# mosure/bevy_gaussian_splatting

Hardware: AMD Instinct MI355X
Metric: frames/sec @1080p, 1M-splat 3DGS (sort + rasterize every frame) (higher is better)
Workload: dtype f32; 1 GPU; 1000000-splat 3DGS f32 planar cloud (seed 2, reference random_gaussians_3d distributions), 1920x1080, SH degree 3, CloudSettings::default(), examples/headless.rs camera incl. its Msaa (Bevy's default Sample4: 4 samples per pixel, resolved frame); one camera per GPU; sample_count=4, parallelism=views1, sort=radix32, frames_in_flight=8, lanes=8, streams=4

## Files before the change

### bevy_gaussian_splatting_amd/_native.py

```python
from __future__ import annotations

import ctypes
import os
from ctypes import POINTER, c_char_p, c_float, c_int
from typing import Optional

from . import _build_id, _loader
from .camera import BgsView
from .settings import BgsSettings

SPEC = _build_id.LIBBGS
LIB_PATH = SPEC.path

BGS_OK = 0
BGS_EINVAL = -1
BGS_ENOMEM = -2
BGS_EHIP = -3
BGS_ECAPACITY = -4
BGS_EINTERNAL = -5

STAGE_NAMES = ("keygen", "depth_sort", "project", "tile_sort", "ranges", "raster")

COMM_ID_BYTES = 128
ABI_VERSION = (0 << 16) | 4


class BgsSortEntry(ctypes.Structure):
    _fields_ = [("key", ctypes.c_uint32), ("index", ctypes.c_uint32)]


class BgsStats(ctypes.Structure):
    _fields_ = [
        ("stage_ms", ctypes.c_float * 6),
        ("total_ms", ctypes.c_float),
        ("splat_count", ctypes.c_uint32),
        ("visible_count", ctypes.c_uint32),
        ("draw_count", ctypes.c_uint32),
        ("sort_path", ctypes.c_uint32),
        ("instance_count", ctypes.c_uint64),
        ("instance_capacity", ctypes.c_uint64),
        ("tiles_x", ctypes.c_uint32),
        ("tiles_y", ctypes.c_uint32),
        ("depth_passes", ctypes.c_uint32),
        ("tile_passes", ctypes.c_uint32),
        ("algorithmic_bytes", ctypes.c_uint64),
        ("regrow_count", ctypes.c_uint32),
        ("binning_mode", ctypes.c_uint32),
        ("frames_averaged", ctypes.c_uint32),
        ("list_capacity", ctypes.c_uint32),
        ("list_entries_allocated", ctypes.c_uint64),
        ("strip_tiles", ctypes.c_uint32),
        ("tile_saturation", ctypes.c_uint32),
    ]


class BgsFrameRecordsInfo(ctypes.Structure):

    _fields_ = [("draw_count", ctypes.c_uint32), ("record_stride", ctypes.c_uint32), ("has_rects", ctypes.c_uint32),
                ("visible_count", ctypes.c_uint32), ("color_max_bits", ctypes.c_uint32)]


vp, u32, u64 = ctypes.c_void_p, ctypes.c_uint32, ctypes.c_uint64
fp, up, u64p, vpp = POINTER(c_float), POINTER(u32), POINTER(u64), POINTER(vp)
view_p, settings_p, entry_p = POINTER(BgsView), POINTER(BgsSettings), POINTER(BgsSortEntry)

PROTOTYPES = (
    ("bgs_create", c_int, (c_int, vpp)),
    ("bgs_destroy", None, (vp,)),
    ("bgs_last_error", c_char_p, (vp,)),
    ("bgs_version", u32, ()),
    ("bgs_abi_check", c_int, (u32, u32, u32, u32)),
    ("bgs_build_id", c_char_p, ()),
    ("bgs_settings_default", None, (settings_p,)),
    ("bgs_view_perspective", None, (fp, c_float, c_float, u32, u32, view_p)),
    ("bgs_cloud_upload_f32", c_int, (vp, u32, fp, fp, fp, fp, vpp)),
    ("bgs_cloud_upload_f16", c_int, (vp, u32, fp, up, up, vpp)),
    ("bgs_cloud_upload_cov3d_f32", c_int, (vp, u32, fp, fp, fp, vpp)),
    ("bgs_cloud_free", None, (vp, vp)),
    ("bgs_cloud_len", u32, (vp,)),
    ("bgs_cloud_apply_particle_behaviors", c_int, (vp, vp, vp, u32, c_float)),
    ("bgs_sort", c_int, (vp, vp, view_p, settings_p, entry_p)),
    ("bgs_render", c_int, (vp, vp, view_p, settings_p, fp)),
    ("bgs_framebuffer_device_ptr", c_int, (vp, vpp, u64p)),
    ("bgs_set_output_srgb8", c_int, (vp, c_int)),
    ("bgs_framebuffer_srgb8_device_ptr", c_int, (vp, vpp, u64p)),
    ("bgs_set_output_rgba16f", c_int, (vp, c_int)),
    ("bgs_framebuffer_rgba16f_device_ptr", c_int, (vp, vpp, u64p)),
    ("bgs_set_packed_only", c_int, (vp, c_int)),
    ("bgs_set_srgb8_target", c_int, (vp, vp)),
    ("bgs_download", c_int, (vp, vp, vp, u64)),
    ("bgs_device_alloc", c_int, (vp, u64, vpp)),
    ("bgs_device_free", c_int, (vp, vp)),
    ("bgs_upload", c_int, (vp, vp, vp, u64)),
    ("bgs_set_pipeline_depth", c_int, (vp, u32)),
    ("bgs_pipeline_pop", c_int, (vp, vpp, vpp)),
    ("bgs_frames_in_flight", c_int, (vp, up)),
    ("bgs_sorted_entries_device_ptr", c_int, (vp, vpp, up)),
    ("bgs_synchronize", c_int, (vp,)),
    ("bgs_set_async", c_int, (vp, c_int)),
    ("bgs_stream", c_int, (vp, vpp)),
    ("bgs_set_binning", c_int, (vp, u32)),
    ("bgs_reset_adaptive_state", c_int, (vp,)),
    ("bgs_set_profiling", c_int, (vp, c_int)),
    ("bgs_set_profiling_stride", c_int, (vp, u32)),
    ("bgs_get_stats", c_int, (vp, POINTER(BgsStats))),
    ("bgs_set_pipeline_streams", c_int, (vp, u32)),
    ("bgs_set_graphs", c_int, (vp, c_int)),
    ("bgs_comm_unique_id", c_int, (c_char_p,)),
    ("bgs_comm_create", c_int, (vp, c_char_p, u32, u32, vpp)),
    ("bgs_comm_gather", c_int, (vp, vp, u32, vp, u64, vp, u64p)),
    ("bgs_comm_gather_after", c_int, (vp, vp, u32, vp, u64, vp, vp, u64p)),
    ("bgs_comm_wait", c_int, (vp, vp, u64)),
    ("bgs_comm_stream", c_int, (vp, vp, vpp)),
    ("bgs_comm_destroy", None, (vp, vp)),
    ("bgs_set_debug_flags", c_int, (vp, u32)),
    ("bgs_adaptive_counters", c_int, (vp, u64p)),
    ("bgs_learning_counters", c_int, (vp, u64p, u64p)),
    ("bgs_radix_sort_pairs", c_int, (vp, entry_p, u32, u32)),
    ("bgs_hbm_probe", c_int, (vp, u64, u32, fp, fp)),
    ("bgs_selftest_ln_f32", c_int, (vp, u32, u32, fp, u64p)),
    ("bgs_set_queue_holders", c_int, (c_int,)),
    ("bgs_set_tile_trace", c_int, (vp, vp)),
    ("bgs_graph_counters", c_int, (vp, u64p, u64p)),
    ("bgs_tile_order_counters", c_int, (vp, u64p, u64p, u64p)),
    ("bgs_selftest_tile_order", c_int, (vp, vp, u32, u32, vp, vp)),
    ("bgs_selftest_pack", c_int, (vp, u32, vp, u32, vp)),
    ("bgs_debug_frame_records", c_int, (vp, vp, u64, up, u32, POINTER(BgsFrameRecordsInfo))),
)
EXPORTED_SYMBOLS = tuple(name for name, _, _ in PROTOTYPES)


class BgsError(RuntimeError):
    def __init__(self, status: int, message: str):
        super().__init__(f"libbgs error {status}: {message}")
        self.status = status


_lib: Optional[ctypes.CDLL] = None


def ensure_current() -> str:
    return _loader.ensure_current(SPEC, LIB_PATH)


def build_id() -> str:
    return load().bgs_build_id().decode()


def load() -> ctypes.CDLL:
    global _lib
    if _lib is not None:
        return _lib
    override = os.environ.get("BGS_LIB_OVERRIDE")
    if override:
        import sys
        print(f"bevy_gaussian_splatting_amd: BGS_LIB_OVERRIDE={override} — NOT the library of this tree "
              f"(build id {_build_id.library_build_id(override)})", file=sys.stderr)
        lib = ctypes.CDLL(override, mode=SPEC.dlopen_mode)
        _loader.declare(lib, PROTOTYPES)
    else:
        want = ensure_current()
        lib = ctypes.CDLL(LIB_PATH, mode=SPEC.dlopen_mode)
        _loader.declare(lib, PROTOTYPES)
        if lib.bgs_build_id().decode() != want:
            raise ImportError(f"{LIB_PATH}: bgs_build_id() disagrees with the id in the file's bytes")
    rc = lib.bgs_abi_check(ABI_VERSION, ctypes.sizeof(BgsView), ctypes.sizeof(BgsSettings), ctypes.sizeof(BgsStats))
    if rc != BGS_OK:
        raise ImportError("libbgs.so refuses this binding: " + (lib.bgs_last_error(None) or b"").decode("utf-8", "replace"))
    _lib = lib
    return lib


def check(lib: ctypes.CDLL, ctx, status: int) -> None:
    if status != BGS_OK:
        msg = lib.bgs_last_error(ctx)
        raise BgsError(status, msg.decode("utf-8", "replace") if msg else "")
```

### bevy_gaussian_splatting_amd/csrc/bgs_api.hip

```cpp
#include "bgs_context.h"
#include "build_id.inc"

static const char g_build_id[] = "BGS_BUILD_ID=" BGS_BUILD_ID;

namespace {
void mat4_mul(const float* a, const float* b, float* out) {
    for (int c = 0; c < 4; ++c)
        for (int r = 0; r < 4; ++r) {
            float acc = 0.0f;
            for (int k = 0; k < 4; ++k) acc += a[4 * k + r] * b[4 * c + k];
            out[4 * c + r] = acc;
        }
}

bool mat4_inverse(const float* m, float* out) {
    double a[4][8];
    for (int r = 0; r < 4; ++r)
        for (int c = 0; c < 4; ++c) {
            a[r][c] = m[4 * c + r];
            a[r][4 + c] = r == c ? 1.0 : 0.0;
        }
    for (int i = 0; i < 4; ++i) {
        int piv = i;
        for (int r = i + 1; r < 4; ++r)
            if (std::fabs(a[r][i]) > std::fabs(a[piv][i])) piv = r;
        if (a[piv][i] == 0.0) return false;
        if (piv != i)
            for (int c = 0; c < 8; ++c) std::swap(a[i][c], a[piv][c]);
        const double d = a[i][i];
        for (int c = 0; c < 8; ++c) a[i][c] /= d;
        for (int r = 0; r < 4; ++r)
            if (r != i) {
                const double f = a[r][i];
                for (int c = 0; c < 8; ++c) a[r][c] -= f * a[i][c];
            }
    }
    for (int r = 0; r < 4; ++r)
        for (int c = 0; c < 4; ++c) out[4 * c + r] = (float)a[r][4 + c];
    return true;
}

}


extern "C" {

uint32_t bgs_version(void) { return (BGS_VERSION_MAJOR << 16) | BGS_VERSION_MINOR; }

const char* bgs_build_id(void) { return g_build_id + 13; }

const char* bgs_last_error(const bgs_ctx* ctx) { return ctx ? ctx->error.c_str() : g_error.c_str(); }

int bgs_create(int hip_device, bgs_ctx** out) {
    if (!out) return fail(nullptr, BGS_EINVAL, "out is NULL");
    *out = nullptr;
    int count = 0;
    hipError_t e = hipGetDeviceCount(&count);
    if (e != hipSuccess || count <= 0)
        return fail(nullptr, BGS_EHIP, std::string("no usable HIP device (there is no CPU fallback): ") +
                                           hipGetErrorString(e));
    if (hip_device < 0 || hip_device >= count) return fail(nullptr, BGS_EINVAL, "hip_device out of range");
    bgs_ctx* ctx = new (std::nothrow) bgs_ctx();
    if (!ctx) return fail(nullptr, BGS_ENOMEM, "out of host memory");
    ctx->device = hip_device;
    auto bail = [&](const std::string& msg) {
        bgs_destroy(ctx);
        return fail(nullptr, BGS_EHIP, msg);
    };
    if ((e = hipSetDevice(hip_device)) != hipSuccess) return bail(std::string("hipSetDevice: ") + hipGetErrorString(e));
    hipDeviceProp_t prop;
    if ((e = hipGetDeviceProperties(&prop, hip_device)) != hipSuccess)
        return bail(std::string("hipGetDeviceProperties: ") + hipGetErrorString(e));
    ctx->num_cus = prop.multiProcessorCount > 0 ? prop.multiProcessorCount : 256;
    if (lane_create(ctx, ctx->lanes[0]) != BGS_OK) return bail(ctx->error);
    *out = ctx;
    return BGS_OK;
}

void bgs_destroy(bgs_ctx* ctx) {
    if (!ctx) return;
    (void)hipSetDevice(ctx->device);
    for (auto& L : ctx->lanes) lane_destroy(L);
    for (auto st : ctx->streams) if (st) (void)hipStreamDestroy(st);
    if (ctx->step_done) (void)hipEventDestroy(ctx->step_done);
    delete ctx;
}

void bgs_settings_default(bgs_settings* out) {
    if (!out) return;
    std::memset(out, 0, sizeof *out);
    for (int i = 0; i < 4; ++i) out->transform[5 * i] = 1.0f;
    out->global_opacity = 1.0f;
    out->global_scale = 1.0f;
    out->gaussian_mode = BGS_GAUSSIAN_3D;
    out->aabb = 0;
    out->opacity_adaptive_radius = 1;
    out->color_space = BGS_COLOR_SRGB;
    out->radix_depth_bits = 32;
    out->sh_degree = 3;
    out->sort_mode = BGS_SORT_RADIX;
    out->rasterize_mode = BGS_RASTERIZE_COLOR;
    out->num_classes = 1;
    for (int i = 0; i < 3; ++i) out->position_max[i] = 1.0f;
    out->position_min[3] = out->position_max[3] = 1.0f;
}

void bgs_view_perspective(const float world_from_view[16], float fov_y_radians, float near_plane,
                          uint32_t width, uint32_t height, bgs_view* out) {
    if (!out || !world_from_view) return;
    std::memset(out, 0, sizeof *out);
    std::memcpy(out->world_from_view, world_from_view, 16 * sizeof(float));
    if (!mat4_inverse(world_from_view, out->view_from_world))
        for (int i = 0; i < 4; ++i) out->view_from_world[5 * i] = 1.0f;
    const float f = 1.0f / std::tan(0.5f * fov_y_radians);
    const float aspect = (float)width / (float)height;
    out->clip_from_view[0] = f / aspect;
    out->clip_from_view[5] = f;
    out->clip_from_view[11] = -1.0f;
    out->clip_from_view[14] = near_plane;
    mat4_mul(out->clip_from_view, out->view_from_world, out->clip_from_world);
    out->viewport[0] = 0.0f;
    out->viewport[1] = 0.0f;
    out->viewport[2] = (float)width;
    out->viewport[3] = (float)height;
    out->clear_color[3] = 1.0f;
    out->sample_count = 4;
    std::memcpy(out->previous_clip_from_world, out->clip_from_world, sizeof out->clip_from_world);
    out->delta_time = 1.0f / 60.0f;
}

static int upload_plane(bgs_ctx* ctx, const void* host, size_t bytes, DeviceBuffer<uint8_t>& dev) {
    if (!dev.reserve(bytes, 16)) return fail(ctx, BGS_ENOMEM, "hipMalloc(cloud plane) failed");
    if (bytes && hipMemcpy(dev.ptr, host, bytes, hipMemcpyHostToDevice) != hipSuccess)
        return fail(ctx, BGS_EHIP, "hipMemcpy(cloud plane) failed");
    return BGS_OK;
}

static int upload_and_pack(bgs_ctx* ctx, uint32_t format, uint32_t n, const void* pv, const void* const planes[3],
                           const uint32_t v4[3], uint32_t stride_v4, bgs_cloud** out) {
    if (!ctx) return fail(nullptr, BGS_EINVAL, "ctx is NULL");
    if (!out) return fail(ctx, BGS_EINVAL, "out is NULL");
    *out = nullptr;
    if (n > MAX_SPLATS) return fail(ctx, BGS_EINVAL, "too many splats");
    bool missing = !pv;
    for (int k = 0; k < 3; ++k) missing = missing || (v4[k] && !planes[k]);
    if (n && missing) return fail(ctx, BGS_EINVAL, "NULL plane pointer");
    if (hipSetDevice(ctx->device) != hipSuccess) return fail(ctx, BGS_EHIP, "hipSetDevice failed");
    bgs_cloud* c = new (std::nothrow) bgs_cloud();
    if (!c) return fail(ctx, BGS_ENOMEM, "out of host memory");
    DeviceBuffer<uint8_t> tmp[3];
    int rc = upload_plane(ctx, pv, (size_t)n * 16, c->positions);
    for (int k = 0; rc == BGS_OK && k < 3; ++k)
        if (v4[k]) rc = upload_plane(ctx, planes[k], (size_t)n * 16 * v4[k], tmp[k]);
    if (rc == BGS_OK && !c->packed.reserve((size_t)n * 16 * stride_v4, 256))
        rc = fail(ctx, BGS_ENOMEM, "hipMalloc(packed cloud records) failed");
    if (rc == BGS_OK) {
        hipStream_t st = ctx->lanes[0].stream;
        launch_pack_cloud(st, (const uint4*)c->positions.ptr, (const uint4*)tmp[0].ptr, v4[0], (const uint4*)tmp[1].ptr, v4[1],
                          (const uint4*)tmp[2].ptr, v4[2], (uint4*)c->packed.ptr, stride_v4, n);
        if (hipGetLastError() != hipSuccess || hipStreamSynchronize(st) != hipSuccess) {
            (void)hipGetLastError();
            rc = fail(ctx, BGS_EHIP, "packing the cloud on the device failed");
        }
    }
    if (rc != BGS_OK) { bgs_cloud_free(ctx, c); return rc; }
    c->bytes = (size_t)n * 16 + (size_t)n * 16 * stride_v4;
    c->ptrs.position_visibility = (const float4*)c->positions.ptr;
    c->ptrs.packed = (const uint4*)c->packed.ptr;
    c->ptrs.packed_v4 = stride_v4;
    c->ptrs.n = n;
    c->ptrs.format = format;
    *out = c;
    return BGS_OK;
}

int bgs_cloud_upload_f32(bgs_ctx* ctx, uint32_t n, const float* pv, const float* sh, const float* rot,
                         const float* so, bgs_cloud** out) {
    const void* const planes[3] = {rot, so, sh};
    const uint32_t v4[3] = {1u, 1u, 12u};
    return upload_and_pack(ctx, CLOUD_F32, n, pv, planes, v4, 16u, out);
}

int bgs_cloud_upload_f16(bgs_ctx* ctx, uint32_t n, const float* pv, const uint32_t* sh_h2,
                         const uint32_t* rso, bgs_cloud** out) {
    const void* const planes[3] = {rso, sh_h2, nullptr};
    const uint32_t v4[3] = {1u, 6u, 0u};
    return upload_and_pack(ctx, CLOUD_F16, n, pv, planes, v4, 8u, out);
}

int bgs_cloud_upload_cov3d_f32(bgs_ctx* ctx, uint32_t n, const float* pv, const float* sh, const float* cov3d_opacity,
                               bgs_cloud** out) {
    const void* const planes[3] = {cov3d_opacity, nullptr, sh};
    const uint32_t v4[3] = {2u, 0u, 12u};
    return upload_and_pack(ctx, CLOUD_COV3D, n, pv, planes, v4, 16u, out);
}

void bgs_cloud_free(bgs_ctx* ctx, bgs_cloud* cloud) {
    if (!cloud) return;
    if (ctx) {
        (void)hipSetDevice(ctx->device);
        (void)finish_all(ctx);
        for (auto& L : ctx->lanes) {
            if (L.stream) (void)hipStreamSynchronize(L.stream);
            if (L.in.cloud == cloud) L.in.cloud = nullptr;
        }
        for (auto& sl : ctx->split_slots)
            if (sl.cloud == cloud) sl.epoch = 0;
    }
    delete cloud;
}

uint32_t bgs_cloud_len(const bgs_cloud* cloud) { return cloud ? cloud->ptrs.n : 0; }

int bgs_cloud_apply_particle_behaviors(bgs_ctx* ctx, bgs_cloud* cloud, void* behaviors_device_ptr, uint32_t count, float delta_time) {
    if (!ctx) return fail(nullptr, BGS_EINVAL, "ctx is NULL");
    if (!cloud) return fail(ctx, BGS_EINVAL, "cloud is NULL");
    if (!std::isfinite(delta_time)) return fail(ctx, BGS_EINVAL, "delta_time is not finite");
    if (count == 0) return BGS_OK;
    if (!behaviors_device_ptr) return fail(ctx, BGS_EINVAL, "behaviors_device_ptr is NULL with count > 0");
    if ((uintptr_t)behaviors_device_ptr % 16u) return fail(ctx, BGS_EINVAL, "behaviors_device_ptr is not 16-byte aligned");
    return apply_particle_step(ctx, cloud, behaviors_device_ptr, count, delta_time);
}

int bgs_sort(bgs_ctx* ctx, const bgs_cloud* cloud, const bgs_view* view, const bgs_settings* settings,
             bgs_sort_entry* host_out) {
    int rc = run(ctx, cloud, view, settings, false);
    if (rc != BGS_OK) return rc;
    Lane& L = ctx->lanes[0];
    if (host_out && L.last_sorted_n)
        HIP_TRY(ctx, hipMemcpy(host_out, L.last_sorted, (size_t)L.last_sorted_n * sizeof(uint2), hipMemcpyDeviceToHost));
    return BGS_OK;
}

int bgs_render(bgs_ctx* ctx, const bgs_cloud* cloud, const bgs_view* view, const bgs_settings* settings,
               float* rgba_host_out) {
    int rc = run(ctx, cloud, view, settings, true);
    if (rc != BGS_OK) return rc;
    if (rgba_host_out) {
        Lane& L = ctx->lanes[ctx->recent];
        if (L.pending && (rc = finish_lane(ctx, L)) != BGS_OK) return rc;
        if (!L.fb_valid) return fail(ctx, BGS_EINVAL, "the frame wrote its packed image only (bgs_set_packed_only): no f32 target to copy");
        HIP_TRY(ctx, hipMemcpy(rgba_host_out, L.fb.ptr, (size_t)L.fb_w * L.fb_h * sizeof(float4), hipMemcpyDeviceToHost));
    }
    return BGS_OK;
}

int bgs_framebuffer_device_ptr(bgs_ctx* ctx, void** dptr, uint64_t* bytes) {
    if (!ctx || !dptr) return fail(ctx, BGS_EINVAL, "NULL argument");
    Lane& L = ctx->lanes[ctx->recent];
    if (L.pending) {
        int rc = finish_lane(ctx, L);
        if (rc != BGS_OK) return rc;
    }
    if (!L.fb.ptr) return fail(ctx, BGS_EINVAL, "no frame has been rendered yet");
    if (!L.fb_valid) return fail(ctx, BGS_EINVAL, "the last frame wrote its packed image only (bgs_set_packed_only)");
    *dptr = L.fb.ptr;
    if (bytes) *bytes = (uint64_t)L.fb_w * L.fb_h * sizeof(float4);
    return BGS_OK;
}

int bgs_framebuffer_srgb8_device_ptr(bgs_ctx* ctx, void** dptr, uint64_t* bytes) {
    if (!ctx || !dptr) return fail(ctx, BGS_EINVAL, "NULL argument");
    Lane& L = ctx->lanes[ctx->recent];
    if (L.pending) {
        int rc = finish_lane(ctx, L);
        if (rc != BGS_OK) return rc;
    }
    if (!L.fb8_out || !L.fb8_valid || L.fb8_is_f16)
        return fail(ctx, BGS_EINVAL, "no Rgba8UnormSrgb frame: call bgs_set_output_srgb8(ctx, 1) before rendering");
    *dptr = L.fb8_out;
    if (bytes) *bytes = (uint64_t)L.fb_w * L.fb_h * 4u;
    return BGS_OK;
}

int bgs_pipeline_pop(bgs_ctx* ctx, void** rgba_f32, void** rgba8) {
    if (!ctx) return fail(nullptr, BGS_EINVAL, "ctx is NULL");
    if (hipSetDevice(ctx->device) != hipSuccess) return fail(ctx, BGS_EHIP, "hipSetDevice failed");
    int best = -1;
    for (int i = 0; i < MAX_LANES; ++i)
        if ((ctx->lanes[i].pending || ctx->lanes[i].ready) && (best < 0 || ctx->lanes[i].seq < ctx->lanes[best].seq)) best = i;
    if (best < 0) return fail(ctx, BGS_EINVAL, "no frame in flight");
    Lane& L = ctx->lanes[best];
    int rc = finish_lane(ctx, L);
    if (rc != BGS_OK) return rc;
    if (rgba_f32) *rgba_f32 = L.fb_valid ? L.fb.ptr : nullptr;
    if (rgba8) *rgba8 = L.fb8_valid ? L.fb8_out : nullptr;
    return BGS_OK;
}

int bgs_frames_in_flight(bgs_ctx* ctx, uint32_t* count) {
    if (!ctx || !count) return fail(ctx, BGS_EINVAL, "NULL argument");
    uint32_t c = 0;
    for (auto& L : ctx->lanes) c += (L.pending || L.ready) ? 1u : 0u;
    *count = c;
    return BGS_OK;
}

int bgs_sorted_entries_device_ptr(bgs_ctx* ctx, void** dptr, uint32_t* n) {
    if (!ctx || !dptr) return fail(ctx, BGS_EINVAL, "NULL argument");
    Lane& L = ctx->lanes[ctx->recent];
    if (L.pending) {
        int rc = finish_lane(ctx, L);
        if (rc != BGS_OK) return rc;
    }
    if (!L.last_sorted) return fail(ctx, BGS_EINVAL, "no sort has been run yet");
    *dptr = (void*)L.last_sorted;
    if (n) *n = L.last_sorted_n;
    return BGS_OK;
}

int bgs_synchronize(bgs_ctx* ctx) {
    if (!ctx) return fail(nullptr, BGS_EINVAL, "ctx is NULL");
    if (hipSetDevice(ctx->device) != hipSuccess) return fail(ctx, BGS_EHIP, "hipSetDevice failed");
    int rc = finish_all(ctx);
    if (rc != BGS_OK) return rc;
    for (auto& L : ctx->lanes)
        if (L.stream) HIP_TRY(ctx, hipStreamSynchronize(L.stream));
    return BGS_OK;
}

int bgs_set_async(bgs_ctx* ctx, int enabled) {
    if (!ctx) return fail(nullptr, BGS_EINVAL, "ctx is NULL");
    if (!enabled) {
        int rc = finish_all(ctx);
        if (rc != BGS_OK) return rc;
    }
    ctx->async_frames = enabled != 0;
    return BGS_OK;
}

int bgs_set_pipeline_depth(bgs_ctx* ctx, uint32_t lanes) {
    if (!ctx) return fail(nullptr, BGS_EINVAL, "ctx is NULL");
    if (lanes < 1 || lanes > (uint32_t)MAX_LANES) return fail(ctx, BGS_EINVAL, "pipeline depth must be 1..8");
    if (hipSetDevice(ctx->device) != hipSuccess) return fail(ctx, BGS_EHIP, "hipSetDevice failed");
    int rc = finish_all(ctx);
    if (rc != BGS_OK) return rc;
    ctx->depth = (int)lanes;
    ctx->next = 0;
    ctx->recent = 0;
    for (uint32_t i = 0; i < lanes; ++i)
        if ((rc = lane_create(ctx, ctx->lanes[i])) != BGS_OK) return rc;
    return assign_streams(ctx);
}

int bgs_set_pipeline_streams(bgs_ctx* ctx, uint32_t streams) {
    if (!ctx) return fail(nullptr, BGS_EINVAL, "ctx is NULL");
    if (streams > (uint32_t)MAX_LANES) return fail(ctx, BGS_EINVAL, "pipeline streams must be 0..8");
    if (hipSetDevice(ctx->device) != hipSuccess) return fail(ctx, BGS_EHIP, "hipSetDevice failed");
    int rc = finish_all(ctx);
    if (rc != BGS_OK) return rc;
    for (auto st : ctx->streams)
        if (st) HIP_TRY(ctx, hipStreamSynchronize(st));
    ctx->num_streams = (int)streams;
    return assign_streams(ctx);
}

int bgs_set_srgb8_target(bgs_ctx* ctx, void* device_ptr) {
    if (!ctx) return fail(nullptr, BGS_EINVAL, "ctx is NULL");
    ctx->next_srgb8_target = (uint32_t*)device_ptr;
    return BGS_OK;
}

int bgs_download(bgs_ctx* ctx, const void* device_ptr, void* host_out, uint64_t bytes) {
    if (!ctx || !device_ptr || !host_out) return fail(ctx, BGS_EINVAL, "NULL argument");
    if (hipSetDevice(ctx->device) != hipSuccess) return fail(ctx, BGS_EHIP, "hipSetDevice failed");
    if (bytes) HIP_TRY(ctx, hipMemcpy(host_out, device_ptr, (size_t)bytes, hipMemcpyDeviceToHost));
    return BGS_OK;
}

int bgs_device_alloc(bgs_ctx* ctx, uint64_t bytes, void** device_ptr_out) {
    if (!ctx || !device_ptr_out) return fail(ctx, BGS_EINVAL, "NULL argument");
    *device_ptr_out = nullptr;
    if (hipSetDevice(ctx->device) != hipSuccess) return fail(ctx, BGS_EHIP, "hipSetDevice failed");
    DeviceBuffer<uint8_t> buf;
    if (!buf.reserve((size_t)bytes, 16)) return fail(ctx, BGS_ENOMEM, "hipMalloc(" + std::to_string(bytes) + " bytes) failed");
    *device_ptr_out = buf.release();
    return BGS_OK;
}

int bgs_device_free(bgs_ctx* ctx, void* device_ptr) {
    if (!ctx) return fail(nullptr, BGS_EINVAL, "ctx is NULL");
    if (!device_ptr) return BGS_OK;
    if (hipSetDevice(ctx->device) != hipSuccess) return fail(ctx, BGS_EHIP, "hipSetDevice failed");
    int rc = finish_all(ctx);
    if (rc != BGS_OK) return rc;
    HIP_TRY(ctx, hipFree(device_ptr));
    return BGS_OK;
}

int bgs_upload(bgs_ctx* ctx, void* device_ptr, const void* host_in, uint64_t bytes) {
    if (!ctx || !device_ptr || !host_in) return fail(ctx, BGS_EINVAL, "NULL argument");
    if (hipSetDevice(ctx->device) != hipSuccess) return fail(ctx, BGS_EHIP, "hipSetDevice failed");
    if (bytes) HIP_TRY(ctx, hipMemcpy(device_ptr, host_in, (size_t)bytes, hipMemcpyHostToDevice));
    return BGS_OK;
}

int bgs_set_output_srgb8(bgs_ctx* ctx, int enabled) {
    if (!ctx) return fail(nullptr, BGS_EINVAL, "ctx is NULL");
    ctx->output_srgb8 = enabled != 0;
    if (enabled) ctx->output_rgba16f = false;
    return BGS_OK;
}

int bgs_set_output_rgba16f(bgs_ctx* ctx, int enabled) {
    if (!ctx) return fail(nullptr, BGS_EINVAL, "ctx is NULL");
    ctx->output_rgba16f = enabled != 0;
    if (enabled) ctx->output_srgb8 = false;
    return BGS_OK;
}

int bgs_set_packed_only(bgs_ctx* ctx, int enabled) {
    if (!ctx) return fail(nullptr, BGS_EINVAL, "ctx is NULL");
    ctx->packed_only = enabled != 0;
    return BGS_OK;
}

int bgs_framebuffer_rgba16f_device_ptr(bgs_ctx* ctx, void** dptr, uint64_t* bytes) {
    if (!ctx || !dptr) return fail(ctx, BGS_EINVAL, "NULL argument");
    Lane& L = ctx->lanes[ctx->recent];
    if (L.pending) {
        int rc = finish_lane(ctx, L);
        if (rc != BGS_OK) return rc;
    }
    if (!L.fb8_out || !L.fb8_valid || !L.fb8_is_f16)
        return fail(ctx, BGS_EINVAL, "no Rgba16Float frame: call bgs_set_output_rgba16f(ctx, 1) before rendering");
    *dptr = L.fb8_out;
    if (bytes) *bytes = (uint64_t)L.fb_w * L.fb_h * 8u;
    return BGS_OK;
}

int bgs_stream(bgs_ctx* ctx, void** hip_stream) {
    if (!ctx || !hip_stream) return fail(ctx, BGS_EINVAL, "NULL argument");
    *hip_stream = (void*)ctx->lanes[ctx->recent].stream;
    return BGS_OK;
}

int bgs_set_profiling(bgs_ctx* ctx, int enabled) {
    if (!ctx) return fail(nullptr, BGS_EINVAL, "ctx is NULL");
    if (enabled < 0 || enabled > 2) return fail(ctx, BGS_EINVAL, "profiling level must be 0, 1 or 2");
    ctx->profiling = enabled;
    return BGS_OK;
}

int bgs_set_profiling_stride(bgs_ctx* ctx, uint32_t every_nth_frame) {
    if (!ctx) return fail(nullptr, BGS_EINVAL, "ctx is NULL");
    if (every_nth_frame == 0) return fail(ctx, BGS_EINVAL, "stride must be >= 1");
    ctx->profiling_stride = every_nth_frame;
    ctx->frame_counter = 0;
    return BGS_OK;
}

int bgs_set_binning(bgs_ctx* ctx, uint32_t mode) {
    if (!ctx) return fail(nullptr, BGS_EINVAL, "ctx is NULL");
    if (mode > BINNING_SORT) return fail(ctx, BGS_EINVAL, "binning mode must be 0 (scan) or 1 (sort)");
    int rc = finish_all(ctx);
    if (rc != BGS_OK) return rc;
    ctx->binning = mode;
    return BGS_OK;
}

int bgs_set_debug_flags(bgs_ctx* ctx, uint32_t flags) {
    if (!ctx) return fail(nullptr, BGS_EINVAL, "ctx is NULL");
    ctx->debug_flags = flags;
    return BGS_OK;
}

int bgs_adaptive_counters(bgs_ctx* ctx, uint64_t out[8]) {
    if (!ctx || !out) return fail(ctx, BGS_EINVAL, "NULL argument");
    out[0] = ctx->bucket_frames;
    out[1] = ctx->onesweep_frames;
    out[2] = ctx->reruns_sort;
    out[3] = ctx->reruns_lists;
    out[4] = ctx->reruns_instances;
    out[5] = ctx->level_changes;
// ... 88 lines not shown
```

### bevy_gaussian_splatting_amd/csrc/bgs_context.h

```cpp
#pragma once
#include <hip/hip_runtime.h>

#include <dlfcn.h>

#include <algorithm>
#include <chrono>
#include <cmath>
#include <cstdio>
#include <cstdlib>
#include <cstring>
#include <mutex>
#include <new>
#include <string>
#include <unordered_map>
#include <vector>

#include "../../include/bgs.h"
#include "../../include/bgs_diag.h"
#include "bgs_device.h"
#include "device_buffer.h"
#include "frame_params.h"
#include "kernels.h"

using namespace bgs;

namespace bgs_host {

struct DeviceMem {
    static void* alloc(size_t bytes) {
        void* p = nullptr;
        if (hipMalloc(&p, bytes) == hipSuccess) return p;
        (void)hipGetLastError();
        return nullptr;
    }
    static void free(void* p) { (void)hipFree(p); }
};
struct PinnedMem {
    static void* alloc(size_t bytes) {
        void* p = nullptr;
        if (hipHostMalloc(&p, bytes, hipHostMallocDefault) == hipSuccess) return p;
        (void)hipGetLastError();
        return nullptr;
    }
    static void free(void* p) { (void)hipHostFree(p); }
};
template <class T> using DeviceBuffer = Buffer<T, DeviceMem>;
template <class T> using PinnedBuffer = Buffer<T, PinnedMem>;

}

struct bgs_cloud {
    CloudPtrs ptrs{};
    bgs_host::DeviceBuffer<uint8_t> positions, packed;
    uint64_t bytes = 0;
};

namespace bgs_host {

extern thread_local std::string g_error;

constexpr uint64_t MIN_INSTANCE_CAPACITY = 1ull << 22;
constexpr uint64_t MAX_INSTANCE_CAPACITY = 1ull << 30;
constexpr uint32_t MAX_SPLATS = (1u << 30) - 1u;
constexpr int EV_COUNT = BGS_STAGE_COUNT + 1;
constexpr int EV_RING = 64;
constexpr int MAX_LANES = 8;

struct GraphKey {
    const void* cloud[6];
    const void* bufs[11];
    uint32_t n, format, places, sort_mode, gaussian_mode, aabb, any_mode, srgb8, debug_flags;
    int32_t width, height;
    int32_t sort_blocks, bin_blocks, keygen_blocks;
    uint32_t sup_edge;
    ScratchLayout scratch;
    uint32_t coarse_cap, sort_path;
    const void* keygen_func;
    uint32_t keygen_threads;
    uint32_t wide_bin;
    uint32_t raster_variant;
    uint32_t split_sub;
};
struct FrameGraph {
    hipGraph_t graph = nullptr;
    hipGraphExec_t exec = nullptr;
    hipGraphNode_t keygen_node = nullptr;
    GraphKey key{};
};

struct FrameInputs {
    const bgs_cloud* cloud = nullptr;
    bgs_view view{};
    bgs_settings settings{};
    bool render = false, allow_graph = false;
    uint32_t* srgb8_target = nullptr;
    bool output_srgb8 = false, output_rgba16f = false, packed_only = false;
    uint32_t debug_flags = 0;
    uint64_t kind = 0;
    bool force_passes = false;
};

struct FramePlan {
    FrameParams fp{};
    bool render = false, scan = false, surfel = false, culled_tail = true;
    uint32_t n = 0, places = 0, rec_bytes = 0, cloud_format = 0;
    bool bucket = false, wide = false, kept = false;
    uint32_t bucket_sub = 1, split_sub_out = 1;
    int split_slot = -1;
    uint64_t split_epoch = 0;
    uint32_t edges[4] = {6, 8, 16, 32}, level = 1, sup_edge = 8, num_st = 0;
    bool large = false, wide_bin = false, want_srgb8 = false;
    int sort_blocks = 0, bin_blocks = 0, binning_blocks = 0;
    uint32_t out_format = 0, ntiles = 0;
    bool raster_cleans = false;
    RasterInst raster{};
    bool heavy = false, cost = false, ordered = false, refresh = false, graph_ok = false;
    uint64_t sat_kind = 0;
};

struct Lane {
    hipStream_t stream = nullptr;
    hipEvent_t done = nullptr;
    DeviceBuffer<FrameParams> d_fp;
    FrameGraph graph[2];

    DeviceBuffer<uint8_t> scratch;
    ScratchLayout layout;
    uint32_t ctl_parity = 0;
    bool scratch_clean = false;

    DeviceBuffer<uint2> entries[2], culled;
    DeviceBuffer<uint8_t> records;
    DeviceBuffer<uint32_t> rects;
    DeviceBuffer<uint2> inst[2];
    DeviceBuffer<uint32_t> coarse;
    DeviceBuffer<uint2> bucket_slots;
    DeviceBuffer<uint32_t> d_split_keys;
    PinnedBuffer<uint32_t> h_split_keys;
    DeviceBuffer<uint8_t> heavy[2];
    uint32_t heavy_parity = 0;
    const uint8_t* heavy_done = nullptr;
    uint32_t heavy_done_grid = 0;
    bool ready = false;
    DeviceBuffer<uint16_t> cost[2], order;
    uint32_t cost_parity = 0;
    const uint16_t* cost_done = nullptr;
    uint32_t cost_done_grid = 0;
    uint32_t order_grid = 0xFFFFFFFFu, order_age = 0;
    DeviceBuffer<float4> fb;
    DeviceBuffer<uint32_t> fb8;
    uint32_t* fb8_out = nullptr;
    uint32_t fb_w = 0, fb_h = 0;
    bool fb8_valid = false, fb8_is_f16 = false;
    bool fb_valid = true;

    PinnedBuffer<Control> h_ctl;
    Control* h_ctl_dev = nullptr;
    hipEvent_t ev_ring[EV_RING][EV_COUNT] = {};
    uint8_t ev_kind[EV_RING] = {};
    uint32_t ev_head = 0;
    uint32_t frames_timed = 0;

    bool pending = false;
    FrameInputs in;
    FramePlan plan;
    uint32_t pending_coarse_cap = 0;
    uint64_t cost_done_kind = 0;
    uint64_t order_kind = 0;
    uint64_t seq = 0;

    const uint2* last_sorted = nullptr;
    uint32_t last_sorted_n = 0;
    const Control* last_ctl = nullptr;

    bgs_stats result{};
    bool has_result = false;
    uint8_t result_kind = 0;
};

}
using namespace bgs_host;

struct bgs_ctx {
    int device = 0;
    int num_cus = 256;
    std::string error;

    Lane lanes[MAX_LANES];
    hipStream_t streams[MAX_LANES] = {};
    int num_streams = 4;
    int depth = 1;
    int next = 0;
    int recent = 0;
    uint64_t seq = 0;
    hipEvent_t step_done = nullptr;

    uint32_t binning = BINNING_SCAN;
    uint32_t debug_flags = 0;
    int profiling = 2;
    uint32_t profiling_stride = 1;
    uint32_t frame_counter = 0;
    bool async_frames = false;
    bool output_srgb8 = false;
    bool output_rgba16f = false;
    bool packed_only = false;
    uint32_t* next_srgb8_target = nullptr;

    uint32_t draw_hint = 0;
    bool draw_hint_valid = false;
    uint32_t draw_shrink_votes = 0;
    uint32_t sup_level = 1;
    struct SplitterSlot {
        SplitterKeys table{};
        const bgs_cloud* cloud = nullptr;
        uint32_t n = 0;
        uint32_t sort_mode = 0;
        float transform[16] = {};
        float pos[3] = {}, fwd[3] = {};
        float clip_from_view[16] = {};
        float viewport_wh[2] = {};
        float reach = 0.0f;
        uint64_t epoch = 0;
        uint64_t last_used = 0;
    };
    static constexpr int SPLITTER_SLOTS = 16;
    SplitterSlot split_slots[SPLITTER_SLOTS];
    uint64_t split_epoch = 0;
    uint64_t split_failed_epoch = 0;
    uint32_t bucket_block = 0;
    uint32_t bucket_fail_streak = 0;
    uint32_t list_shrink_votes = 0;
    uint64_t bucket_frames = 0, onesweep_frames = 0;
    uint64_t reruns_sort = 0, reruns_lists = 0, reruns_instances = 0, level_changes = 0;
    uint32_t coarse_cap_hint = 0;
    struct KindState { uint32_t sup_level = 1; bool midround = false; };
    std::unordered_map<uint64_t, KindState> kinds;
    static constexpr uint32_t LEARN_MAX = 3;
    static constexpr double MIDROUND_ON = 0.30, MIDROUND_OFF = 0.15;
    uint64_t cur_kind = 0;
    std::unordered_map<uint64_t, uint32_t> learning;
    uint64_t early_frames = 0;
    uint4* tile_trace = nullptr;
    bool use_graphs = false;
    uint64_t graph_captures = 0, graph_replays = 0;
    uint64_t cost_frames = 0, ordered_frames = 0, order_refreshes = 0;

    bool have_stats = false;
    bgs_stats stats{};
    uint32_t regrow_count = 0;
};

namespace bgs_host {
int fail(bgs_ctx* ctx, int status, const std::string& msg);
int assign_streams(bgs_ctx* ctx);
int lane_create(bgs_ctx* ctx, Lane& L);
void lane_destroy(Lane& L);
int finish_lane(bgs_ctx* ctx, Lane& L);
int finish_all(bgs_ctx* ctx);
int collect_stats(bgs_ctx* ctx);
int ensure_scratch(bgs_ctx* ctx, Lane& L, uint32_t n, uint64_t inst_cap);
int enqueue_frame(bgs_ctx* ctx, Lane& L, const FrameInputs& in);
int ensure_entries(bgs_ctx* ctx, Lane& L, uint32_t n);
int run(bgs_ctx* ctx, const bgs_cloud* cloud, const bgs_view* view, const bgs_settings* s, bool render);
int apply_particle_step(bgs_ctx* ctx, bgs_cloud* cloud, void* behaviors, uint32_t count, float dt);
extern int g_queue_holders_mode;
extern std::mutex g_queue_holders_mutex;
}

#define HIP_TRY(ctx, expr)                                                                  \
    do {                                                                                    \
        hipError_t e_ = (expr);                                                             \
        if (e_ != hipSuccess)                                                               \
            return fail(ctx, BGS_EHIP, std::string(#expr) + ": " + hipGetErrorString(e_));  \
    } while (0)
```

### bevy_gaussian_splatting_amd/csrc/bgs_frame.hip

```cpp
#include "bgs_context.h"

thread_local std::string bgs_host::g_error;

namespace bgs_host {


constexpr int MAX_DEVICES = 64;
hipStream_t g_queue_holders[MAX_DEVICES][3] = {};
int g_queue_holders_mode = -1;
std::mutex g_queue_holders_mutex;

int fail(bgs_ctx* ctx, int status, const std::string& msg) {
    if (ctx) ctx->error = msg;
    g_error = msg;
    return status;
}


int assign_streams(bgs_ctx* ctx) {
    const int S = ctx->num_streams > 0 ? std::min(ctx->num_streams, ctx->depth) : ctx->depth;
    for (int i = 0; i < MAX_LANES; ++i) {
        Lane& L = ctx->lanes[i];
        if (!L.done) continue;
        const int si = i < ctx->depth ? i % S : i;
// ... 114 lines not shown

bool cost_holds(const Lane& L, uint32_t tiles) { return L.cost[0].holds(tile_cost_bytes(tiles) / 2u); }

int ensure_cost(bgs_ctx* ctx, Lane& L, uint32_t tiles) {
    if (cost_holds(L, tiles)) return BGS_OK;
    L.cost_done = nullptr;
    L.order_grid = 0xFFFFFFFFu;
    L.order.reset();
    bool ok = reserve_group(tile_cost_bytes(tiles) / 2u, L.cost[0], L.cost[1]) < 0;
    for (auto& c : L.cost)
        if (ok && hipMemset(c.ptr, 0, tile_cost_bytes(tiles)) != hipSuccess) { (void)hipGetLastError(); ok = false; }
    if (!ok) {
        for (auto& c : L.cost) c.reset();
        return fail(ctx, BGS_ENOMEM, "hipMalloc(tile cost feedback) failed");
    }
    if (!L.order.reserve(tile_order_bytes(tiles) / 2u)) {
        for (auto& c : L.cost) c.reset();
        return fail(ctx, BGS_ENOMEM, "hipMalloc(tile order) failed");
    }
    return BGS_OK;
}

int ensure_framebuffer(bgs_ctx* ctx, Lane& L, uint32_t w, uint32_t h, bool want8) {
    const size_t px = (size_t)w * h;
    if (!L.fb.reserve(px)) return fail(ctx, BGS_ENOMEM, "hipMalloc(framebuffer) failed");
    if (want8 && !L.fb8.reserve(2 * px)) return fail(ctx, BGS_ENOMEM, "hipMalloc(srgb8 framebuffer) failed");
    L.fb_w = w;
    L.fb_h = h;
    return BGS_OK;
}

int validate(bgs_ctx* ctx, const bgs_cloud* cloud, const bgs_view* view, const bgs_settings* s, bool render) {
    if (!ctx) return fail(nullptr, BGS_EINVAL, "ctx is NULL");
    if (!cloud || !view || !s) return fail(ctx, BGS_EINVAL, "cloud, view and settings must be non-NULL");
    if (s->radix_depth_bits != 16 && s->radix_depth_bits != 24 && s->radix_depth_bits != 32)
        return fail(ctx, BGS_EINVAL, "radix_depth_bits must be 16, 24 or 32");
    if (s->gaussian_mode > BGS_GAUSSIAN_3D) return fail(ctx, BGS_EINVAL, "gaussian_mode must be 2D or 3D");
    if (s->sh_degree > 3) return fail(ctx, BGS_EINVAL, "sh_degree must be 0..3");
    if (s->sort_mode > BGS_SORT_STD) return fail(ctx, BGS_EINVAL, "unknown sort_mode");
    if (s->color_space > BGS_COLOR_LINEAR) return fail(ctx, BGS_EINVAL, "unknown color_space");
    if (s->rasterize_mode == BGS_RASTERIZE_VELOCITY)
        return fail(ctx, BGS_EINVAL, "rasterize_mode Velocity is outside the path (4D clouds only)");
    if (s->rasterize_mode == BGS_RASTERIZE_OPTICAL_FLOW && !(view->delta_time > 0.0f))
        return fail(ctx, BGS_EINVAL, "rasterize_mode OpticalFlow needs bgs_view.delta_time > 0");
    if (s->rasterize_mode > BGS_RASTERIZE_VELOCITY) return fail(ctx, BGS_EINVAL, "unknown rasterize_mode");
    if (s->draw_mode > BGS_DRAW_HIGHLIGHT_SELECTED) return fail(ctx, BGS_EINVAL, "unknown draw_mode");
    if (s->rasterize_mode == BGS_RASTERIZE_CLASSIFICATION && s->num_classes == 0)
        return fail(ctx, BGS_EINVAL, "num_classes must be >= 1");
    if (view->entries_device_ptr) {
        if (view->entries_device_ptr % sizeof(bgs_sort_entry) != 0u)
            return fail(ctx, BGS_EINVAL, "bgs_view.entries_device_ptr must be aligned to 8 bytes (one bgs_sort_entry)");
        if (view->entry_count != cloud->ptrs.n)
            return fail(ctx, BGS_EINVAL, "bgs_view.entry_count must equal bgs_cloud_len(cloud) when entries_device_ptr is set; got " +
                                             std::to_string(view->entry_count) + " for a cloud of " + std::to_string(cloud->ptrs.n));
    } else if (view->entry_count != 0u) {
        return fail(ctx, BGS_EINVAL, "bgs_view.entry_count is " + std::to_string(view->entry_count) + " but bgs_view.entries_device_ptr is 0");
    }
    if (render && cloud->ptrs.format == CLOUD_COV3D &&
        (s->gaussian_mode != BGS_GAUSSIAN_3D || s->rasterize_mode == BGS_RASTERIZE_NORMAL))
        return fail(ctx, BGS_EINVAL, "a precomputed-covariance cloud has no rotation / scale: 3D gaussian mode only, no Normal raster mode");
    if (render) {
        const uint32_t samples = view->sample_count ? view->sample_count : 4u;
        if (samples != 1u && samples != 2u && samples != 4u && samples != 8u)
            return fail(ctx, BGS_EINVAL, "bgs_view.sample_count must be 1 (Msaa::Off), 2, 4 (Msaa::Sample4, Bevy's default), 8 or 0 (= 4); got " +
                                             std::to_string(view->sample_count));
        if (ctx->tile_trace && (view->depth_device_ptr || s->visualize_bounding_box || samples == 2u || samples == 8u))
            return fail(ctx, BGS_EINVAL, "the per-tile trace (bgs_set_tile_trace) has no instantiation with a depth buffer, the bounding-box "
                                         "overlay or 2 / 8 samples per pixel: a frame would leave the trace buffer untouched");
        if (view->depth_device_ptr % (4u * samples) != 0u)
            return fail(ctx, BGS_EINVAL, "bgs_view.depth_device_ptr must be aligned to one pixel's samples (4 * sample_count bytes)");
        const float w = view->viewport[2], h = view->viewport[3];
        if (!(w >= 1.0f) || !(h >= 1.0f) || w > 4096.0f || h > 4096.0f || w != std::floor(w) || h != std::floor(h))
            return fail(ctx, BGS_EINVAL, "viewport width/height must be integers in [1, 4096]");
    }
    return BGS_OK;
}

void view_pose(const bgs_view* v, float pos[3], float fwd[3]) {
    for (int k = 0; k < 3; ++k) { pos[k] = v->world_from_view[12 + k]; fwd[k] = -v->world_from_view[8 + k]; }
    const float len = std::sqrt(fwd[0] * fwd[0] + fwd[1] * fwd[1] + fwd[2] * fwd[2]);
    if (len > 0.0f) for (int k = 0; k < 3; ++k) fwd[k] /= len;
}

int find_splitter_slot(const bgs_ctx* ctx, const bgs_cloud* cloud, const bgs_view* view, const bgs_settings* s) {
    float pos[3], fwd[3];
    view_pose(view, pos, fwd);
    int best = -1;
    float best_d = 0.0f;
    for (int i = 0; i < bgs_ctx::SPLITTER_SLOTS; ++i) {
        const auto& sl = ctx->split_slots[i];
        if (!sl.epoch || sl.cloud != cloud || sl.n != cloud->ptrs.n || sl.sort_mode != s->sort_mode) continue;
        if (std::memcmp(sl.transform, s->transform, sizeof sl.transform) != 0) continue;
        if (s->sort_mode == BGS_SORT_RADIX &&
            (std::memcmp(sl.clip_from_view, view->clip_from_view, sizeof sl.clip_from_view) != 0 ||
             sl.viewport_wh[0] != view->viewport[2] || sl.viewport_wh[1] != view->viewport[3]))
            continue;
        const float dx = pos[0] - sl.pos[0], dy = pos[1] - sl.pos[1], dz = pos[2] - sl.pos[2];
        const float d = std::sqrt(dx * dx + dy * dy + dz * dz);
        const float c = fwd[0] * sl.fwd[0] + fwd[1] * sl.fwd[1] + fwd[2] * sl.fwd[2];
        if (!(d <= 0.05f * sl.reach) || !(c >= 0.9848f)) continue;
        const float score = d / std::max(sl.reach, 1e-30f) + (1.0f - c);
        if (best < 0 || score < best_d) { best = i; best_d = score; }
    }
    return best;
}

uint64_t frame_kind(const bgs_cloud* cloud, const bgs_view* view, const bgs_settings* s) {
    int32_t scale_step = INT32_MIN;
    if (s->global_scale > 0.0f && std::isfinite(s->global_scale)) scale_step = (int32_t)std::lround(2.0 * std::log2((double)s->global_scale));
    const uint64_t words[6] = {((uint64_t)cloud->ptrs.n << 32) | cloud->ptrs.format, ((uint64_t)s->gaussian_mode << 32) | s->aabb,
                               ((uint64_t)(uint32_t)scale_step << 32) | s->opacity_adaptive_radius,
                               ((uint64_t)(uint32_t)view->viewport[2] << 32) | (uint32_t)view->viewport[3],
                               ((uint64_t)(view->sample_count ? view->sample_count : 4u) << 32) | (view->depth_device_ptr ? 1u : 0u),
                               ((uint64_t)s->rasterize_mode << 32) | (s->draw_mode << 1) | (s->visualize_bounding_box ? 1u : 0u)};
    uint64_t hsh = 0xcbf29ce484222325ull;
    for (uint64_t w : words)
        for (int b = 0; b < 8; ++b) { hsh ^= (w >> (8 * b)) & 0xFFu; hsh *= 0x100000001b3ull; }
    return hsh ? hsh : 1ull;
}

void switch_kind(bgs_ctx* ctx, uint64_t kind) {
    if (kind == ctx->cur_kind) return;
    const auto it = ctx->kinds.find(kind);
    if (it != ctx->kinds.end()) ctx->sup_level = it->second.sup_level;
    ctx->cur_kind = kind;
}

struct FrameTotals { uint64_t instances = 0; uint32_t longest = 0; };

FrameTotals frame_totals(const FramePlan& p, const Control& h) {
    FrameTotals t;
    t.instances = (uint64_t)h.instance_total_lo | ((uint64_t)h.instance_total_hi << 32);
    if (p.render && p.scan) {
        t.instances = 0;
        for (uint32_t i = 0; i < p.num_st; ++i) {
            t.instances += h.coarse_total[i];
            t.longest = std::max(t.longest, h.coarse_total[i]);
        }
    }
    return t;
}

int check_watchdog(bgs_ctx* ctx, Lane& L) {
    const Control& h = *L.h_ctl.ptr;
    if (!h.error) return BGS_OK;
    L.scratch_clean = false;
    ctx->draw_hint_valid = false;
    for (auto& sl : ctx->split_slots) sl.epoch = 0;
    return fail(ctx, BGS_EINTERNAL, "device watchdog tripped (look-back spin bound), code " + std::to_string(h.error));
}

int check_capacities(bgs_ctx* ctx, Lane& L, const FrameTotals& t, int attempt, bool* rerun) {
    const FramePlan& p = L.plan;
    const Control& h = *L.h_ctl.ptr;
    *rerun = false;
    if (p.bucket && h.sort_overflow) {
        if (p.split_slot >= 0 && ctx->split_slots[p.split_slot].epoch == p.split_epoch)
            ctx->split_slots[p.split_slot].epoch = 0;
        if (h.sort_overflow & 2u) {
            ctx->bucket_block = 256u;
        } else if (p.split_epoch > ctx->split_failed_epoch) {
            ctx->bucket_fail_streak = std::min(ctx->bucket_fail_streak + 1u, 8u);
            if (ctx->bucket_fail_streak >= 3u) ctx->bucket_block = (1u << ctx->bucket_fail_streak) - 1u;
        }
        ctx->split_failed_epoch = std::max(ctx->split_failed_epoch, p.split_epoch);
        ctx->reruns_sort += 1;
        L.in.force_passes = true;
        *rerun = true;
    } else if (p.bucket) {
        ctx->bucket_fail_streak = 0;
    }
    if (p.render && p.scan) {
        const uint32_t want = std::max<uint32_t>(pow2_ceil_u32((uint64_t)t.longest + t.longest / 4), 4096u);
        if (p.level == ctx->sup_level) {
            if (want > ctx->coarse_cap_hint) {
                ctx->coarse_cap_hint = want;
                ctx->list_shrink_votes = 0;
            } else if ((uint64_t)want * 8u <= ctx->coarse_cap_hint) {
                if (++ctx->list_shrink_votes >= 64u) { ctx->coarse_cap_hint = want * 2u; ctx->list_shrink_votes = 0; }
            } else {
                ctx->list_shrink_votes = 0;
            }
        }
        if (t.longest > L.pending_coarse_cap) {
            if (want > ctx->coarse_cap_hint) ctx->coarse_cap_hint = want;
            *rerun = true;
            ctx->reruns_lists += 1;
        }
    }
    if (p.render && !p.scan && h.overflow) {
        if (t.instances > MAX_INSTANCE_CAPACITY)
            return fail(ctx, BGS_ECAPACITY,
                        "frame needs " + std::to_string(t.instances) + " tile instances, above the 2^30 limit");
        uint64_t cap = MIN_INSTANCE_CAPACITY;
        while (cap < t.instances + t.instances / 4) cap <<= 1;
        cap = std::min(cap, MAX_INSTANCE_CAPACITY);
        int rc = ensure_instances(ctx, L, cap);
        if (rc != BGS_OK) return rc;
        ctx->reruns_instances += 1;
        *rerun = true;
    }
    if ((L.in.debug_flags & BGS_DEBUG_RERUN_EVERY_FRAME) && attempt == 0 && p.render && p.scan) *rerun = true;
    return BGS_OK;
}

void learn_feedback(bgs_ctx* ctx, Lane& L) {
    const FramePlan& p = L.plan;
    const Control& h = *L.h_ctl.ptr;
    const uint32_t grid = (uint32_t)p.fp.tiles_x | ((uint32_t)p.fp.tiles_y << 16);
    L.heavy_done = p.heavy ? L.heavy[L.heavy_parity].ptr : nullptr;
    L.heavy_done_grid = grid;
    if (p.heavy) L.heavy_parity ^= 1u;
    L.cost_done = p.cost ? L.cost[L.cost_parity].ptr : nullptr;
    L.cost_done_kind = L.in.kind;
    L.cost_done_grid = grid;
    if (p.sat_kind && h.saturated_tiles_prev != 0xFFFFFFFFu) {
        const auto kit = ctx->kinds.find(p.sat_kind);
        if (kit != ctx->kinds.end()) {
            const double share = (double)h.saturated_tiles_prev / (double)0x7FFF;
            if (share >= bgs_ctx::MIDROUND_ON) kit->second.midround = true;
            else if (share <= bgs_ctx::MIDROUND_OFF) kit->second.midround = false;
        }
    }
    if (p.cost) L.cost_parity ^= 1u;
}

void learn_draw_hint(bgs_ctx* ctx, uint32_t draw_count) {
    if (!ctx->draw_hint_valid || draw_count > ctx->draw_hint) {
        ctx->draw_hint = (uint32_t)std::min<uint64_t>((uint64_t)draw_count + draw_count / 8 + 1024, 0xFFFFFFFFull);
        ctx->draw_hint_valid = true;
        ctx->draw_shrink_votes = 0;
    } else if ((uint64_t)draw_count * 4 < ctx->draw_hint) {
        if (++ctx->draw_shrink_votes >= 64u) {
            ctx->draw_hint = (uint32_t)std::min<uint64_t>((uint64_t)draw_count * 2 + 1024, 0xFFFFFFFFull);
            ctx->draw_shrink_votes = 0;
        }
    } else {
        ctx->draw_shrink_votes = 0;
    }
}

void learn_splitters(bgs_ctx* ctx, const Lane& L) {
    const FramePlan& p = L.plan;
    const Control& h = *L.h_ctl.ptr;
    const uint32_t nkeys = BUCKET_COUNT * p.split_sub_out - 1u;
    if (p.places != 4 || h.draw_count < BUCKET_COUNT || !splitters_ascending(h.splitters, nkeys) || !L.in.cloud) return;
    int slot = find_splitter_slot(ctx, L.in.cloud, &L.in.view, &L.in.settings);
    if (slot < 0) {
        slot = 0;
        for (int i = 0; i < bgs_ctx::SPLITTER_SLOTS; ++i) {
            if (!ctx->split_slots[i].epoch) { slot = i; break; }
            if (ctx->split_slots[i].last_used < ctx->split_slots[slot].last_used) slot = i;
        }
    }
    auto& sl = ctx->split_slots[slot];
    std::memcpy(sl.table.key, h.splitters, nkeys * sizeof(uint32_t));
    sl.table.sub = p.split_sub_out;
    sl.cloud = L.in.cloud;
    sl.n = p.n;
    sl.sort_mode = L.in.settings.sort_mode;
    std::memcpy(sl.transform, L.in.settings.transform, sizeof sl.transform);
    view_pose(&L.in.view, sl.pos, sl.fwd);
    std::memcpy(sl.clip_from_view, L.in.view.clip_from_view, sizeof sl.clip_from_view);
    sl.viewport_wh[0] = L.in.view.viewport[2];
    sl.viewport_wh[1] = L.in.view.viewport[3];
    const uint32_t mid_bits = 0xFFFFFFFFu - h.splitters[BUCKET_COUNT * p.split_sub_out / 2 - 1];
    float d2;
    std::memcpy(&d2, &mid_bits, 4);
    sl.reach = (d2 > 0.0f && d2 < 3.0e38f) ? std::sqrt(d2) : 1.0f;
    sl.epoch = ++ctx->split_epoch;
    sl.last_used = ctx->seq;
}

bool learn_level(bgs_ctx* ctx, const Lane& L, const FrameTotals& t) {
    const FramePlan& p = L.plan;
    const uint32_t lv = p.level;
    double longer = 1.0;
    const uint32_t target = canonical_supertile_level(
        next_supertile_level((double)t.instances / (double)L.h_ctl.ptr->visible_count, lv, p.edges, &longer), p.edges);
    const auto kit = ctx->kinds.find(L.in.kind);
    if (kit != ctx->kinds.end()) kit->second.sup_level = target;
    if (L.in.kind != ctx->cur_kind || target == lv) return target != lv;
    if (ctx->sup_level != target) {
        const double predicted = (double)t.longest * (target > lv ? longer : 1.0) * 1.25;
        ctx->coarse_cap_hint = std::max<uint32_t>(pow2_ceil_u32((uint64_t)std::min(predicted, 1.0e9)), 4096u);
        ctx->list_shrink_votes = 0;
        ctx->level_changes += 1;
        ctx->sup_level = target;
    }
    return true;
}

void fill_stats(const bgs_ctx* ctx, Lane& L, const FrameTotals& t) {
    const FramePlan& p = L.plan;
    const Control& h = *L.h_ctl.ptr;
    const bool render = p.render, scan = p.scan;
    bgs_stats& stt = L.result;
    std::memset(&stt, 0, sizeof stt);
    stt.regrow_count = ctx->regrow_count;
    stt.splat_count = p.n;
    stt.visible_count = render ? h.visible_count : h.draw_count;
    stt.draw_count = h.draw_count;
    stt.sort_path = p.kept ? 2u : (p.bucket ? 1u : 0u);
    stt.list_capacity = (render && scan) ? L.pending_coarse_cap : 0u;
    stt.instance_count = render ? t.instances : 0;
    stt.instance_capacity = L.inst[0].capacity;
    stt.list_entries_allocated = (render && scan) ? (uint64_t)(L.coarse.capacity / 2) : 0;
    stt.strip_tiles = (render && scan) ? h.strip_tiles : 0u;
    stt.tile_saturation = (render && scan && p.sat_kind && h.saturated_tiles_prev != 0xFFFFFFFFu)
                              ? (0x10000u | (h.saturated_tiles_prev & 0x7FFFu) | (p.raster.mode != 0 ? 0x80000000u : 0u)) : 0u;
    stt.tiles_x = render ? (uint32_t)p.fp.tiles_x : 0;
    stt.tiles_y = render ? (uint32_t)p.fp.tiles_y : 0;
    stt.depth_passes = p.places;
    stt.tile_passes = (render && !scan) ? 2 : 0;
    stt.binning_mode = scan ? BINNING_SCAN : BINNING_SORT;
    const uint64_t N = p.n, k = p.places, D = h.draw_count;
    uint64_t bytes = N * 16 + D * 8 + (p.culled_tail ? (N - D) * 8 : 0) + (p.bucket ? D * 24 : k * D * 16);
    if (p.kept) bytes = N * 8 + D * 8 + (p.culled_tail ? (N - D) * 8 : 0);
    if (render) {
        const uint64_t B = p.cloud_format == CLOUD_F16 ? 128 : 240, R = p.rec_bytes, V = h.visible_count, I = t.instances;
        const uint64_t P = (uint64_t)(uint32_t)p.fp.width * (uint32_t)p.fp.height;
        if (scan)
            bytes += V * (B - 16) + V * R + V * 8 + V * 8 + I * 8 + I * 8 + P * 16;
        else
            bytes += V * (B - 16) + V * R + I * 8 + 2 * I * 16 + I * (4 + R) + P * 16;
    }
    stt.algorithmic_bytes = bytes;
    L.has_result = true;
    L.result_kind = (uint8_t)(!render ? 1 : (scan ? 2 : 3) + (p.kept ? 2 : 0));
}

int finish_lane(bgs_ctx* ctx, Lane& L) {
    L.ready = false;
    for (int attempt = 0; L.pending; ++attempt) {
        HIP_TRY(ctx, hipEventSynchronize(L.done));
        L.pending = false;
        int rc = check_watchdog(ctx, L);
        if (rc != BGS_OK) return rc;
        const FramePlan& p = L.plan;
        const Control& h = *L.h_ctl.ptr;
        const FrameTotals t = frame_totals(p, h);
        bool rerun = false;
        if ((rc = check_capacities(ctx, L, t, attempt, &rerun)) != BGS_OK) return rc;
        if (rerun) {
            if (attempt >= 8) return fail(ctx, BGS_ECAPACITY, "frame kept overflowing its buffers");
            ctx->regrow_count += 1;
            if ((rc = enqueue_frame(ctx, L, L.in)) != BGS_OK) return rc;
            continue;
        }

        if (p.render && p.scan) learn_feedback(ctx, L);
        learn_draw_hint(ctx, h.draw_count);
        learn_splitters(ctx, L);
        const bool level_moved = p.render && p.scan && h.visible_count > 0 && learn_level(ctx, L, t);
        if (p.render && p.scan && attempt == 0 && !level_moved && L.in.kind) {
            if (ctx->kinds.size() >= (1u << 20)) ctx->kinds.clear();
            ctx->kinds[L.in.kind].sup_level = p.level;
        }

        L.last_sorted_n = p.render ? h.draw_count : p.n;
        const bool append_tail = !p.render && h.draw_count < p.n;
        const bool to_chunk = !p.render && L.in.view.entries_device_ptr && p.n > 0;
        if (append_tail) {
            HIP_TRY(ctx, hipMemcpyAsync(const_cast<uint2*>(L.last_sorted) + h.draw_count, L.culled.ptr,
                                        (size_t)(p.n - h.draw_count) * sizeof(uint2), hipMemcpyDeviceToDevice, L.stream));
        }
        if (to_chunk)
            HIP_TRY(ctx, hipMemcpyAsync(reinterpret_cast<void*>((uintptr_t)L.in.view.entries_device_ptr), L.last_sorted,
                                        (size_t)p.n * sizeof(uint2), hipMemcpyDeviceToDevice, L.stream));
        if (append_tail || to_chunk) HIP_TRY(ctx, hipStreamSynchronize(L.stream));
        fill_stats(ctx, L, t);
    }
    return BGS_OK;
}

int finish_all(bgs_ctx* ctx) {
    for (;;) {
        int best = -1;
        for (int i = 0; i < MAX_LANES; ++i)
            if (ctx->lanes[i].pending && (best < 0 || ctx->lanes[i].seq < ctx->lanes[best].seq)) best = i;
        if (best < 0) break;
        int rc = finish_lane(ctx, ctx->lanes[best]);
        if (rc != BGS_OK) return rc;
    }
    for (auto& L : ctx->lanes) L.ready = false;
    return BGS_OK;
}

int collect_stats(bgs_ctx* ctx) {
    Lane& R = ctx->lanes[ctx->recent];
    if (!R.has_result) return fail(ctx, BGS_EINVAL, "no frame has been run yet");
    ctx->stats = R.result;
    bgs_stats& stt = ctx->stats;
    if (ctx->profiling >= 1) {
        const uint8_t kind = R.result_kind;
        const bool render = kind != 1, scan = kind == 2 || kind == 4, kept = kind >= 4;
        const int last = render ? 6 : 2;
        uint32_t used = 0;
        float acc[BGS_STAGE_COUNT] = {0, 0, 0, 0, 0, 0}, acc_total = 0.0f;
        for (auto& L : ctx->lanes) {
            const uint32_t frames = std::min<uint32_t>(L.frames_timed, EV_RING);
            for (uint32_t f = 0; f < frames; ++f) {
                const uint32_t slot = (L.ev_head + EV_RING - f) % EV_RING;
                if (L.ev_kind[slot] != kind) continue;
                hipEvent_t* const ev = L.ev_ring[slot];
                auto ms = [&](int a, int b) { float t = 0; (void)hipEventElapsedTime(&t, ev[a], ev[b]); return t; };
                if (ctx->profiling >= 2) {
                    acc[BGS_STAGE_KEYGEN] += kept ? ms(0, 2) : ms(0, 1);
                    acc[BGS_STAGE_DEPTH_SORT] += kept ? 0.0f : ms(1, 2);
                    if (render && scan) {
                        acc[BGS_STAGE_PROJECT] += ms(2, 3);
                        acc[BGS_STAGE_RASTER] += ms(3, 6);
                    } else if (render) {
                        acc[BGS_STAGE_PROJECT] += ms(2, 3);
                        acc[BGS_STAGE_TILE_SORT] += ms(3, 4);
                        acc[BGS_STAGE_RANGES] += ms(4, 5);
                        acc[BGS_STAGE_RASTER] += ms(5, 6);
                    }
                }
                acc_total += ms(0, last);
                ++used;
            }
            L.frames_timed = 0;
        }
        if (used) {
            for (int i = 0; i < BGS_STAGE_COUNT; ++i) stt.stage_ms[i] = acc[i] / (float)used;
            stt.total_ms = acc_total / (float)used;
        }
        stt.frames_averaged = used;
    }
    ctx->have_stats = true;
    return BGS_OK;
}

FramePlan plan_frame(const bgs_ctx& ctx, const Lane& L, const FrameInputs& in) {
    FramePlan p;
    const uint32_t flags = in.debug_flags;
    const bgs_settings* s = &in.settings;
    FrameParams& fp = p.fp;
    fill_frame_params(in.cloud->ptrs.n, &in.view, s, fp);
    fp.debug = flags;
    fp.srgb8_target = (uint64_t)(uintptr_t)in.srgb8_target;
    const uint32_t n = p.n = fp.n;
    p.render = in.render;
    p.kept = in.render && in.view.entries_device_ptr != 0u && fp.n > 0u;
    p.places = p.kept ? 0u : depth_places(s);
    p.scan = ctx.binning == BINNING_SCAN;
    p.surfel = in.render && fp.gaussian_mode == 0u && fp.aabb != 0u;
    p.rec_bytes = p.surfel ? sizeof(RecordSurfel) : sizeof(Record);
    p.cloud_format = in.cloud->ptrs.format;
    p.culled_tail = !in.render || s->rasterize_mode == BGS_RASTERIZE_DEPTH;

    const bool hint = ctx.draw_hint_valid;
    const int slot = (p.places == 4 && n > 0) ? find_splitter_slot(&ctx, in.cloud, &in.view, s) : -1;
    const uint32_t narrow_max = BUCKET_COUNT * BUCKET_SUB_KERNARG * BUCKET_TARGET;
    p.wide = (hint && ctx.draw_hint > narrow_max && !(flags & BGS_DEBUG_BUCKETS_NARROW)) || (flags & BGS_DEBUG_BUCKETS_WIDE);
    const uint32_t cap_out = p.wide ? BUCKET_CAP_WIDE : BUCKET_CAP, target_out = p.wide ? BUCKET_TARGET_WIDE : BUCKET_TARGET;
    p.bucket = p.places == 4 && n > 0 && !(flags & BGS_DEBUG_NO_BUCKET_SORT) && ctx.bucket_block == 0 && !in.force_passes &&
               ((slot >= 0 && hint) || (flags & BGS_DEBUG_GUESSED_SPLITTERS)) &&
               (!hint || ctx.draw_hint <= BUCKET_MAX * (cap_out / 4u) * 3u);
    if (hint)
        p.split_sub_out = std::min<uint32_t>(std::max<uint32_t>((ctx.draw_hint + BUCKET_COUNT * target_out - 1u) / (BUCKET_COUNT * target_out), 1u), BUCKET_SUB_MAX);
    if (flags & BGS_DEBUG_SPLIT_SUB_3) p.split_sub_out = std::max<uint32_t>(p.split_sub_out, BUCKET_SUB_KERNARG);
    if (flags & BGS_DEBUG_SPLIT_SUB_5) p.split_sub_out = std::max<uint32_t>(p.split_sub_out, 5u);
    if (p.bucket && slot >= 0) {
        p.bucket_sub = std::min<uint32_t>(std::max<uint32_t>(ctx.split_slots[slot].table.sub, 1u), BUCKET_SUB_MAX);
        if (hint && ctx.draw_hint > BUCKET_COUNT * p.bucket_sub * (cap_out / 4u) * 3u) p.bucket = false;
    }
    if (p.bucket && slot >= 0) { p.split_slot = slot; p.split_epoch = ctx.split_slots[slot].epoch; }
    fp.sort_path = p.bucket ? 1u : 0u;
    if (p.kept) { fp.sort_mode = SORT_NONE; fp.key_shift = 0u; }

    supertile_edges((uint32_t)fp.tiles_x, (uint32_t)fp.tiles_y, p.edges);
    uint32_t level = ctx.sup_level;
    if (flags & BGS_DEBUG_LEVEL_0) level = 0;
    else if (flags & BGS_DEBUG_LEVEL_1) level = 1;
    else if (flags & BGS_DEBUG_LEVEL_2) level = 2;
    else if (flags & BGS_DEBUG_LEVEL_3) level = 3;
    p.level = canonical_supertile_level(level, p.edges);
    p.sup_edge = supertile_bins_fit((uint32_t)fp.tiles_x, (uint32_t)fp.tiles_y, p.edges[p.level]) ? p.edges[p.level] : p.edges[1];
    p.num_st = (((uint32_t)fp.tiles_x + p.sup_edge - 1) / p.sup_edge) * (((uint32_t)fp.tiles_y + p.sup_edge - 1) / p.sup_edge);

    p.large = n > (4u << 20);
    p.wide_bin = ctx.depth == 1;
    p.sort_blocks = ctx.num_cus * 4;
    p.bin_blocks = ctx.num_cus * 3;
    p.binning_blocks = ctx.num_cus * 4;
    if (hint && !(flags & BGS_DEBUG_NO_DRAW_HINT)) {
        const uint64_t want = (uint64_t)ctx.draw_hint / sort_tile_size(p.large) + 8;
        p.sort_blocks = (int)std::min<uint64_t>((uint64_t)p.sort_blocks, std::max<uint64_t>(want, 32));
        p.bin_blocks = (int)std::min<uint64_t>((uint64_t)p.bin_blocks, std::max<uint64_t>((uint64_t)ctx.draw_hint / 256 + 8, 32));
        p.binning_blocks = (int)std::min<uint64_t>((uint64_t)p.binning_blocks, std::max<uint64_t>((uint64_t)ctx.draw_hint / 1024 + 4, 16));
    }
    p.want_srgb8 = in.render && (in.output_srgb8 || in.output_rgba16f || in.srgb8_target);
    p.out_format = !p.want_srgb8 ? 0u : ((in.output_rgba16f ? OUT_RGBA16F : OUT_SRGB8) |
                                         ((in.packed_only && p.scan) ? OUT_SKIP_F32 : 0u));

    p.raster_cleans = in.render && p.scan && fp.tiles_x > 0 && fp.tiles_y > 0 && !(flags & BGS_DEBUG_NO_RASTER_CLEANUP);
    bool kind_midround = false;
    if (ctx.depth > 1) { const auto kit = ctx.kinds.find(in.kind); if (kit != ctx.kinds.end()) kind_midround = kit->second.midround; }
    p.raster = raster_instantiation(fp, p.level, kind_midround, ctx.depth, flags);
    p.ntiles = (uint32_t)(fp.tiles_x * fp.tiles_y);
    const bool feedback = p.raster_cleans && !(in.allow_graph && ctx.use_graphs) && p.ntiles <= 65535u;
    p.heavy = feedback && p.raster.mode == 1 && p.level >= 2u && !ctx.tile_trace &&
              (ctx.depth == 1 || (flags & BGS_DEBUG_STRIPS_ANY_DEPTH)) && !(flags & BGS_DEBUG_NO_STRIPS);
    p.cost = feedback && (ctx.depth == 1 || !(flags & BGS_DEBUG_NO_TILE_COST_PIPELINED)) && !(flags & BGS_DEBUG_NO_TILE_COST);
    if (p.cost && p.ntiles > (uint32_t)(ctx.num_cus * 4 * raster_scan_waves_per_simd(fp))) {
        const uint32_t grid = (uint32_t)fp.tiles_x | ((uint32_t)fp.tiles_y << 16);
        const bool kept = cost_holds(L, p.ntiles);
        const bool have_costs = kept && L.cost_done && L.cost_done != L.cost[L.cost_parity].ptr && L.cost_done_grid == grid;
        const bool have_order = kept && L.order_grid == grid;
        p.refresh = have_costs && (!have_order || L.order_age + 1u >= TILE_ORDER_REFRESH || (flags & BGS_DEBUG_ORDER_EVERY_FRAME));
        p.ordered = p.refresh || have_order;
    }
    p.sat_kind = !p.ordered ? 0 : (p.refresh ? L.cost_done_kind : L.order_kind);
    p.graph_ok = in.allow_graph && ctx.use_graphs && p.raster_cleans && p.bucket_sub <= BUCKET_SUB_KERNARG &&
                 !(flags & BGS_DEBUG_NO_GRAPHS) && !ctx.tile_trace && !p.kept;
    return p;
}

GraphKey graph_key(const FramePlan& p, const FrameInputs& in, const Lane& L, const KeygenLaunch& kg, uint32_t coarse_cap) {
    GraphKey key;
    std::memset(&key, 0, sizeof key);
    const FrameParams& fp = p.fp;
    const void* planes[6] = {in.cloud->ptrs.position_visibility, in.cloud->ptrs.packed, nullptr, nullptr, nullptr, nullptr};
    std::memcpy(key.cloud, planes, sizeof planes);
    const void* bufs[11] = {L.entries[0].ptr, L.entries[1].ptr, L.culled.ptr, L.records.ptr, L.coarse.ptr, L.fb.ptr, L.fb8.ptr,
                            L.scratch.ptr, L.d_fp.ptr, L.h_ctl_dev, L.bucket_slots.ptr};
    std::memcpy(key.bufs, bufs, sizeof bufs);
    key.n = p.n; key.format = p.cloud_format; key.places = p.places; key.sort_mode = in.settings.sort_mode;
    key.gaussian_mode = fp.gaussian_mode; key.aabb = fp.aabb;
    key.any_mode = (fp.rasterize_mode != RASTERIZE_COLOR || fp.draw_mode != 0u) ? 1u : 0u;
    key.srgb8 = p.out_format;
    key.debug_flags = in.debug_flags;
    key.width = fp.width; key.height = fp.height;
    key.sort_blocks = p.bucket ? 0 : p.sort_blocks;
    key.bin_blocks = p.bin_blocks * 4096 + p.binning_blocks;
    key.keygen_blocks = (int32_t)kg.blocks; key.keygen_func = kg.func; key.keygen_threads = kg.threads;
    key.wide_bin = p.wide_bin ? 1u : 0u;
    const RasterInst& r = p.raster;
    key.raster_variant = r.samples | (r.depth ? 0x100u : 0u) | (r.overlay ? 0x200u : 0u) | (r.mode == 1 ? 0x400u : r.mode == 2 ? 0x800u : 0u);
    key.split_sub = p.split_sub_out;
    key.sup_edge = p.sup_edge;
    key.scratch = L.layout;
    key.coarse_cap = coarse_cap;
    key.sort_path = p.bucket ? (p.bucket_sub | (p.wide ? 0x100u : 0u)) : 0u;
    return key;
}

template <class Issue>
int launch_graph(bgs_ctx* ctx, Lane& L, const GraphKey& key, KeygenLaunch& kg, Issue&& issue) {
    FrameGraph& G = L.graph[L.ctl_parity];
    if (G.exec && std::memcmp(&G.key, &key, sizeof key) == 0) {
        HIP_TRY(ctx, kg.update_node(G.exec, G.keygen_node));
        ctx->graph_replays += 1;
    } else {
        graph_destroy(G);
        HIP_TRY(ctx, hipStreamBeginCapture(L.stream, hipStreamCaptureModeThreadLocal));
        const hipError_t ie = issue();
        const hipError_t ce = hipStreamEndCapture(L.stream, &G.graph);
        size_t roots = 1;
        if (ie != hipSuccess || ce != hipSuccess || !G.graph ||
            hipGraphInstantiate(&G.exec, G.graph, nullptr, nullptr, 0) != hipSuccess ||
            hipGraphGetRootNodes(G.graph, &G.keygen_node, &roots) != hipSuccess || roots != 1) {
            graph_destroy(G);
            (void)hipGetLastError();
            return fail(ctx, BGS_EHIP, "capturing the frame into a hipGraph failed");
        }
        G.key = key;
        ctx->graph_captures += 1;
    }
    HIP_TRY(ctx, hipGraphLaunch(G.exec, L.stream));
    return BGS_OK;
}

int ensure_frame_buffers(bgs_ctx* ctx, Lane& L, const FramePlan& p, const FrameInputs& in, uint32_t* coarse_cap) {
    int rc;
    if ((rc = lane_create(ctx, L)) != BGS_OK) return rc;
    if ((rc = ensure_entries(ctx, L, p.n)) != BGS_OK) return rc;
    if (p.bucket && p.bucket_sub > BUCKET_SUB_KERNARG && (rc = ensure_split_keys(ctx, L)) != BGS_OK) return rc;
    if (p.bucket && (rc = ensure_bucket_slots(ctx, L, p.bucket_sub, p.wide)) != BGS_OK) return rc;
    if (p.render) {
        if (p.scan) {
            if ((rc = ensure_coarse(ctx, L, p.n, p.num_st, in.debug_flags, coarse_cap)) != BGS_OK) return rc;
            if ((rc = ensure_rects(ctx, L)) != BGS_OK) return rc;
        } else {
            if ((rc = ensure_instances(ctx, L, std::max<uint64_t>(L.inst[0].capacity, MIN_INSTANCE_CAPACITY))) != BGS_OK) return rc;
        }
        if ((rc = ensure_records(ctx, L, (size_t)p.n * p.rec_bytes)) != BGS_OK) return rc;
        if ((rc = ensure_framebuffer(ctx, L, (uint32_t)p.fp.width, (uint32_t)p.fp.height, in.output_srgb8 || in.output_rgba16f)) != BGS_OK) return rc;
    }
    if ((rc = ensure_scratch(ctx, L, p.n, L.inst[0].capacity)) != BGS_OK) return rc;
    if (p.heavy && (rc = ensure_heavy(ctx, L, p.ntiles)) != BGS_OK) return rc;
    if (p.cost && (rc = ensure_cost(ctx, L, p.ntiles)) != BGS_OK) return rc;
    return BGS_OK;
}

int enqueue_frame(bgs_ctx* ctx, Lane& L, const FrameInputs& in) {
    const FramePlan p = plan_frame(*ctx, L, in);
    const FrameParams& fp = p.fp;
    const uint32_t n = p.n, places = p.places, flags = in.debug_flags;
    const bool render = p.render, scan = p.scan, bucket = p.bucket;

    uint32_t coarse_cap = 1;
    int rc = ensure_frame_buffers(ctx, L, p, in, &coarse_cap);
    if (rc != BGS_OK) return rc;

    hipStream_t st = L.stream;
    const bool need_memset = !L.scratch_clean;
    if (need_memset) L.ctl_parity = 0;
    const ScratchLayout& lay = L.layout;
    uint8_t* const scratch = L.scratch.ptr;
    Control* ctl = (Control*)(scratch + (L.ctl_parity ? lay.off_ctl1 : 0));
    uint32_t* depth_status = (uint32_t*)(scratch + lay.off_depth_status);
    unsigned long long* scan_status = (unsigned long long*)(scratch + lay.off_scan_status);
    uint32_t* tile_status = (uint32_t*)(scratch + lay.off_tile_status);
    uint2* ranges = (uint2*)(scratch + lay.off_ranges);
    uint32_t* bin_status = (uint32_t*)(scratch + lay.off_bin_status);
    uint32_t* part_status = (uint32_t*)(scratch + lay.off_part_status);
    const uint32_t grid = (uint32_t)fp.tiles_x | ((uint32_t)fp.tiles_y << 16);
    uint8_t* const heavy_out = p.heavy ? L.heavy[L.heavy_parity].ptr : nullptr;
    const uint8_t* const heavy_in = (p.heavy && L.heavy_done && L.heavy_done != heavy_out && L.heavy_done_grid == grid) ? L.heavy_done : nullptr;
    uint16_t* const cost_out = p.cost ? L.cost[L.cost_parity].ptr : nullptr;
    const uint16_t* const cost_in = p.refresh ? L.cost_done : nullptr;
    uint16_t* const tile_order = p.ordered ? L.order.ptr : nullptr;
    uint2* const draw_list = L.entries[places & 1u].ptr;
    const uint32_t final_xor = (fp.sort_mode == BGS_SORT_RAYON || fp.sort_mode == BGS_SORT_STD) ? 0xFFFFFFFFu : 0u;

    KeygenLaunch kg{};
    kg.fp = fp;
    kg.pos = in.cloud->ptrs.position_visibility;
    kg.entries = L.entries[0].ptr;
    kg.culled = p.culled_tail ? L.culled.ptr : nullptr;
    kg.ctl = ctl;
    kg.part_status = part_status;
    kg.places = places;
    kg.ticket_slot = 7;
    kg.fp_out = L.d_fp.ptr;
    kg.zero_word = reinterpret_cast<uint32_t*>(heavy_out);
    kg.bucket_slots = L.bucket_slots.ptr;
    kg.bucket_status = depth_status;
    if (bucket) {
        if (p.split_slot >= 0) {
            const SplitterKeys& tk = ctx->split_slots[p.split_slot].table;
            const uint32_t nkeys = BUCKET_COUNT * p.bucket_sub - 1u;
            if (p.bucket_sub <= BUCKET_SUB_KERNARG) std::memcpy(kg.split.key, tk.key, nkeys * sizeof(uint32_t));
            else std::memcpy(L.h_split_keys.ptr, tk.key, nkeys * sizeof(uint32_t));
            kg.split.device_keys = L.d_split_keys.ptr;
        } else {
            for (uint32_t i = 0; i < BUCKET_COUNT; ++i) kg.split.key[i] = (i + 1u) << 24;
        }
        kg.split.sub = p.bucket_sub;
        kg.split.wide = p.wide ? 1u : 0u;
    }
    kg.wide = p.wide_bin;
    const bool have_keygen = !p.kept && kg.prepare(ctx->num_cus * 4);
    const uint2* const kept_entries = reinterpret_cast<const uint2*>((uintptr_t)in.view.entries_device_ptr);
    FrameCleanup cl{};
    if (p.raster_cleans) {
        cl.part_status = part_status;
        cl.depth_status = depth_status;
        cl.bin_status = bin_status;
        cl.other_ctl = (Control*)(scratch + (L.ctl_parity ? 0 : lay.off_ctl1));
        cl.host_ctl = L.h_ctl_dev;
        cl.pass_stride = lay.pass_stride;
        cl.places = bucket ? 0u : places;
        cl.depth_tile = sort_tile_size(p.large);
        cl.sorted = draw_list;
        cl.key_xor = final_xor;
        cl.split_sub = p.split_sub_out;
        if (tile_order) cl.order_stats = reinterpret_cast<const uint32_t*>(reinterpret_cast<const uint8_t*>(tile_order) + tile_order_stats_offset(p.ntiles));
    }

    if (ctx->bucket_block > 0 && places == 4) ctx->bucket_block -= 1;
    if (bucket) ctx->bucket_frames += 1;
    else if (places > 0) ctx->onesweep_frames += 1;
    if (bucket && p.split_slot >= 0) ctx->split_slots[p.split_slot].last_used = ctx->seq + 1;
    if (p.cost) ctx->cost_frames += 1;
    if (p.ordered) ctx->ordered_frames += 1;
    if (p.refresh) { ctx->order_refreshes += 1; L.order_kind = L.cost_done_kind; L.order_grid = grid; L.order_age = 0; }
    else if (p.ordered) L.order_age += 1u;
    const bool timed_frame = (ctx->frame_counter++ % ctx->profiling_stride) == 0;
    const int prof = timed_frame ? ctx->profiling : 0;
    const int last_mark = render ? 6 : 2;
    if (prof) {
        L.ev_head = (L.ev_head + 1) % EV_RING;
        L.ev_kind[L.ev_head] = (uint8_t)(!render ? 1 : (scan ? 2 : 3) + (p.kept ? 2 : 0));
        L.frames_timed += 1;
    }
    hipEvent_t* const ev = L.ev_ring[L.ev_head];
    auto mark = [&](int i) {
        if (prof >= 2 || (prof == 1 && (i == 0 || i == last_mark))) (void)hipEventRecord(ev[i], st);
    };

    auto issue = [&]() -> hipError_t {
        mark(0);
        if (cost_in) launch_tile_order(st, cost_in, tile_order, p.ntiles, fp, p.raster.mode != 0);
        if (have_keygen) {
            if (bucket && p.bucket_sub > BUCKET_SUB_KERNARG) {
                const hipError_t ce = hipMemcpyAsync(L.d_split_keys.ptr, L.h_split_keys.ptr, (BUCKET_COUNT * p.bucket_sub - 1u) * sizeof(uint32_t),
                                                     hipMemcpyHostToDevice, st);
                if (ce != hipSuccess) return ce;
            }
            hipError_t e = kg.launch(st);
            if (e != hipSuccess) return e;
        }
        if (p.kept) {
            const hipError_t e = launch_entries_compact(st, fp, kept_entries, draw_list, kg.culled, ctl, part_status, kg.ticket_slot,
                                                        L.d_fp.ptr, kg.zero_word);
            if (e != hipSuccess) return e;
        }
        mark(1);
        int cur = 0;
        if (bucket) {
            const hipError_t e = launch_bucket_sort(st, L.bucket_slots.ptr, draw_list, ctl, final_xor, BUCKET_COUNT * p.bucket_sub, p.wide);
            if (e != hipSuccess) return e;
        }
        for (uint32_t q = 0; q < (bucket ? 0u : places); ++q) {
            launch_onesweep_pass(st, L.entries[cur].ptr, L.entries[cur ^ 1].ptr, &ctl->draw_count, n, ctl->hist_depth[q],
                                 depth_status + (size_t)q * lay.pass_stride, &ctl->ticket[q][0], &ctl->error,
                                 q * RADIX_BITS, q + 1 == places ? final_xor : 0u, p.large, p.sort_blocks);
            cur ^= 1;
        }
        mark(2);
        if (render && scan) {
            launch_project_bin(st, fp, L.d_fp.ptr, in.cloud->ptrs, draw_list, L.culled.ptr, ctl, bin_status, L.records.ptr, L.rects.ptr, L.coarse.ptr,
                               coarse_cap, p.sup_edge, 4, p.bin_blocks, p.binning_blocks, p.wide_bin);
            mark(3);
            launch_raster_scan(st, fp, L.d_fp.ptr, L.records.ptr, L.coarse.ptr, coarse_cap, p.sup_edge, ctl, L.fb.ptr, L.fb8.ptr,
                               (flags & BGS_DEBUG_SEPARATE_ENCODE) ? 0u : p.out_format, cl, ctx->tile_trace,
                               p.raster.mode, heavy_in, heavy_out, tile_order, cost_out);
            mark(6);
        } else if (render) {
            const uint32_t capacity = (uint32_t)std::min<uint64_t>(L.inst[0].capacity, MAX_INSTANCE_CAPACITY);
            launch_project_emit(st, fp, in.cloud->ptrs, draw_list, L.culled.ptr, ctl, scan_status, L.records.ptr, L.inst[0].ptr, capacity,
                                4, ctx->num_cus * 3);
            mark(3);
            for (uint32_t q = 0; q < 2; ++q)
                launch_onesweep_pass(st, L.inst[q].ptr, L.inst[q ^ 1].ptr, &ctl->instance_count, capacity, ctl->hist_tile[q],
                                     tile_status + (size_t)q * lay.inst_tiles * RADIX_BASE, &ctl->ticket[5 + q][0],
                                     &ctl->error, q * RADIX_BITS, 0u, true, ctx->num_cus * 4);
            mark(4);
            launch_tile_ranges(st, L.inst[0].ptr, ctl, ranges);
            mark(5);
            launch_raster(st, fp, L.records.ptr, L.inst[0].ptr, ranges, L.fb.ptr, in.view.clear_color, ctl);
            mark(6);
        }
        if (p.want_srgb8 && !(render && scan && !(flags & BGS_DEBUG_SEPARATE_ENCODE)))
            launch_encode_srgb8(st, L.fb.ptr, L.fb8.ptr, (uint32_t)fp.width * (uint32_t)fp.height, L.d_fp.ptr, p.out_format);
        return hipGetLastError();
    };
    if (p.graph_ok && !need_memset && prof == 0 && have_keygen) {
        if ((rc = launch_graph(ctx, L, graph_key(p, in, L, kg, coarse_cap), kg, issue)) != BGS_OK) return rc;
    } else {
        if (need_memset) HIP_TRY(ctx, hipMemsetAsync(scratch, 0, lay.bytes, st));
        if (!have_keygen && !p.kept) HIP_TRY(ctx, hipMemcpyAsync(L.d_fp.ptr, &fp, sizeof fp, hipMemcpyHostToDevice, st));
        HIP_TRY(ctx, issue());
    }
    L.scratch_clean = p.raster_cleans;
    if (p.raster_cleans) {
        L.ctl_parity ^= 1u;
    } else {
        if (places == 4 && n > 0) launch_splitters(st, draw_list, ctl, final_xor, p.split_sub_out);
        HIP_TRY(ctx, hipMemcpyAsync(L.h_ctl.ptr, ctl, sizeof(Control), hipMemcpyDeviceToHost, st));
    }
    HIP_TRY(ctx, hipEventRecord(L.done, st));

    L.last_sorted = draw_list;
    L.last_sorted_n = n;
    L.last_ctl = render ? ctl : nullptr;
    L.fb_valid = !(p.out_format & OUT_SKIP_F32) || (flags & BGS_DEBUG_SEPARATE_ENCODE);
    L.fb8_is_f16 = (p.out_format & OUT_RGBA16F) != 0u;
    L.fb8_valid = p.want_srgb8;
    if (p.want_srgb8) L.fb8_out = in.srgb8_target ? in.srgb8_target : L.fb8.ptr;
    L.pending = true;
    L.pending_coarse_cap = coarse_cap;
    L.in = in;
    L.plan = p;
    L.seq = ++ctx->seq;
    return BGS_OK;
}

int run(bgs_ctx* ctx, const bgs_cloud* cloud, const bgs_view* view, const bgs_settings* s, bool render) {
    int rc = validate(ctx, cloud, view, s, render);
    if (rc != BGS_OK) return rc;
    if (hipSetDevice(ctx->device) != hipSuccess) return fail(ctx, BGS_EHIP, "hipSetDevice failed");
    const bool async = ctx->async_frames && render && ctx->binning == BINNING_SCAN;
    Lane& L = ctx->lanes[async ? ctx->next : 0];
    if (!async && (rc = finish_all(ctx)) != BGS_OK) return rc;
    if (async && L.pending && (rc = finish_lane(ctx, L)) != BGS_OK) return rc;
    const FrameInputs in{cloud, *view, *s, render, async, render ? ctx->next_srgb8_target : nullptr,
                         ctx->output_srgb8, ctx->output_rgba16f, ctx->packed_only, ctx->debug_flags,
                         render ? frame_kind(cloud, view, s) : 0ull, false};
    if (!async) {
        ctx->recent = 0;
        ctx->regrow_count = 0;
        if (render) switch_kind(ctx, in.kind);
        if ((rc = enqueue_frame(ctx, L, in)) != BGS_OK) return rc;
        ctx->next_srgb8_target = nullptr;
        return finish_lane(ctx, L);
    }
    L.ready = false;
    const bool learn = ctx->kinds.find(in.kind) == ctx->kinds.end();
    switch_kind(ctx, in.kind);
    if ((rc = enqueue_frame(ctx, L, in)) != BGS_OK) return rc;
    ctx->next_srgb8_target = nullptr;
    ctx->recent = ctx->next;
    ctx->next = (ctx->next + 1) % ctx->depth;
    if (learn) {
        if ((rc = finish_lane(ctx, L)) != BGS_OK) return rc;
        L.ready = true;
        ctx->early_frames += 1;
        if (ctx->kinds.find(in.kind) != ctx->kinds.end()) {
            ctx->learning.erase(in.kind);
        } else if (++ctx->learning[in.kind] >= bgs_ctx::LEARN_MAX) {
            ctx->kinds[in.kind].sup_level = ctx->sup_level;
            ctx->learning.erase(in.kind);
        }
        if (ctx->learning.size() >= (1u << 16)) ctx->learning.clear();
    }
    return BGS_OK;
}

int apply_particle_step(bgs_ctx* ctx, bgs_cloud* cloud, void* behaviors, uint32_t count, float dt) {
    if (hipSetDevice(ctx->device) != hipSuccess) return fail(ctx, BGS_EHIP, "hipSetDevice failed");
    for (;;) {
        int best = -1;
        for (int i = 0; i < MAX_LANES; ++i)
            if (ctx->lanes[i].pending && (best < 0 || ctx->lanes[i].seq < ctx->lanes[best].seq)) best = i;
        if (best < 0) break;
        int rc = finish_lane(ctx, ctx->lanes[best]);
        if (rc != BGS_OK) return rc;
        ctx->lanes[best].ready = true;
    }
    if (!ctx->step_done) HIP_TRY(ctx, hipEventCreateWithFlags(&ctx->step_done, hipEventDisableTiming));
    hipStream_t st = ctx->lanes[0].stream;
    launch_particle_step(st, behaviors, count, cloud->ptrs, dt);
    HIP_TRY(ctx, hipGetLastError());
    HIP_TRY(ctx, hipEventRecord(ctx->step_done, st));
    for (hipStream_t other : ctx->streams)
        if (other && other != st) HIP_TRY(ctx, hipStreamWaitEvent(other, ctx->step_done, 0));
    return BGS_OK;
}

}
```

### bevy_gaussian_splatting_amd/csrc/kernels.h

```cpp
#pragma once
#include <hip/hip_runtime.h>
#include <stdint.h>

#include "bgs_device.h"

namespace bgs {

struct CloudPtrs {
    const float4* position_visibility;
    const uint4* packed;
    uint32_t packed_v4;
    uint32_t n;
    uint32_t format;
};
constexpr uint32_t PACK_ROT = 1u, PACK_SCALE_OPACITY = 2u, PACK_SH_F32 = 3u;
constexpr uint32_t PACK_COV3D = 1u;
constexpr uint32_t PACK_RSO_F16 = 1u, PACK_SH_F16 = 2u;
constexpr uint32_t CLOUD_F32 = 0, CLOUD_F16 = 1, CLOUD_COV3D = 2;

struct FrameCleanup {
    uint32_t* part_status;
    uint32_t* depth_status;
    uint32_t* bin_status;
    Control* other_ctl;
    Control* host_ctl;
    uint32_t pass_stride;
    uint32_t places;
    uint32_t depth_tile;
    const uint2* sorted;
    uint32_t key_xor;
    uint32_t split_sub;
    const uint32_t* order_stats;
};


struct KeygenLaunch {
    FrameParams fp;
    const float4* pos;
    uint2* entries;
    uint2* culled;
    Control* ctl;
    uint32_t* part_status;
    uint32_t places;
    uint32_t ticket_slot;
    FrameParams* fp_out;
    uint2* bucket_slots;
    uint32_t* bucket_status;
    SplitterTable split;
    uint32_t* zero_word;
    bool wide = false;
    const void* func;
    uint32_t blocks, threads;
    void* argv[13];
    uint32_t lds_bytes;
    bool prepare(int max_blocks);
    hipError_t launch(hipStream_t stream);
    hipError_t update_node(hipGraphExec_t exec, hipGraphNode_t node);
};
#ifndef BGS_KEYGEN_WIDE_THREADS
#define BGS_KEYGEN_WIDE_THREADS 256
#endif
#ifndef BGS_KEYGEN_HUGE_LOG2
#define BGS_KEYGEN_HUGE_LOG2 (BGS_KEYGEN_WIDE_THREADS == 256 ? 31 : 22)
#endif
inline uint32_t keygen_tile_splats(uint32_t n) { return n >= (1u << BGS_KEYGEN_HUGE_LOG2) ? 8192u : (n >= (1u << 19) ? 4096u : 2048u); }

hipError_t launch_entries_compact(hipStream_t stream, const FrameParams& fp, const uint2* entries, uint2* draw_list, uint2* tail,
                                  Control* ctl, uint32_t* part_status, uint32_t ticket_slot, FrameParams* fp_out, uint32_t* zero_word);

void launch_histogram(hipStream_t stream, const uint2* pairs, uint32_t n, uint32_t* hist ,
                      uint32_t passes);

void launch_onesweep_pass(hipStream_t stream, const uint2* in, uint2* out, const uint32_t* n_ptr,
                          uint32_t max_n, const uint32_t* hist, uint32_t* status, uint32_t* ticket,
                          uint32_t* error_flag, uint32_t shift, uint32_t key_xor, bool large_tiles,
                          int max_blocks);

hipError_t launch_bucket_sort(hipStream_t stream, const uint2* bucket_slots, uint2* out, Control* ctl, uint32_t key_xor,
                              uint32_t buckets = BUCKET_COUNT , bool wide = false);
void launch_splitters(hipStream_t stream, const uint2* sorted, Control* ctl, uint32_t key_xor, uint32_t sub = 1u);

void launch_project_emit(hipStream_t stream, const FrameParams& fp, const CloudPtrs& cloud,
                         const uint2* draw_list, const uint2* culled, Control* ctl, unsigned long long* scan_status,
                         void* records, uint2* instances, uint32_t capacity, uint32_t ticket_slot,
                         int max_blocks);

void launch_project_bin(hipStream_t stream, const FrameParams& fp, const FrameParams* d_fp, const CloudPtrs& cloud,
                        const uint2* draw_list, const uint2* culled, Control* ctl, uint32_t* bin_status, void* records,
                        uint32_t* rects, uint32_t* coarse, uint32_t coarse_cap, uint32_t sup_edge,
                        uint32_t ticket_slot, int project_blocks, int bin_blocks, bool wide_bin);

void launch_raster_scan(hipStream_t stream, const FrameParams& fp, const FrameParams* d_fp, const void* records,
                        const uint32_t* coarse, uint32_t coarse_cap,
                        uint32_t sup_edge, Control* ctl, float4* framebuffer, uint32_t* srgb8_default,
                        uint32_t out_format, const FrameCleanup& cleanup, uint4* tile_trace = nullptr,
                        int mode = 0 ,
                        const uint8_t* heavy_in = nullptr, uint8_t* heavy_out = nullptr,
                        const uint16_t* order = nullptr, uint16_t* cost_out = nullptr);
constexpr uint32_t TILE_ORDER_REFRESH = 8u;
inline size_t tile_cost_bytes(uint32_t tiles) { return ((size_t)tiles + 4u) * 2u; }
__host__ __device__ inline size_t tile_order_stats_offset(uint32_t tiles) { return (((((size_t)tiles + 3u) / 4u + 8u) * 2u + 63u) / 64u) * 64u; }
inline size_t tile_order_bytes(uint32_t tiles) { return tile_order_stats_offset(tiles) + 16u * sizeof(uint32_t); }
void launch_tile_order(hipStream_t stream, const uint16_t* cost, uint16_t* order, uint32_t ntiles, const FrameParams& fp,
                       bool midround_exit);
void launch_tile_order_runs(hipStream_t stream, const uint16_t* cost, uint16_t* order, uint32_t ntiles, uint32_t runs);
int raster_scan_waves_per_simd(const FrameParams& fp);
constexpr uint32_t HEAVY_CAP = 256u, HEAVY_LIST_OFFSET = 128u, HEAVY_FLAGS_OFFSET = HEAVY_LIST_OFFSET + 2u * HEAVY_CAP;
inline size_t heavy_feedback_bytes(uint32_t tiles) { return (size_t)HEAVY_FLAGS_OFFSET + tiles; }
constexpr uint32_t OUT_SRGB8 = 1u;
constexpr uint32_t OUT_RGBA16F = 2u;
constexpr uint32_t OUT_SKIP_F32 = 4u;

void launch_tile_ranges(hipStream_t stream, const uint2* instances, const Control* ctl, uint2* ranges);

void launch_raster(hipStream_t stream, const FrameParams& fp, const void* records,
                   const uint2* instances, const uint2* ranges, float4* framebuffer,
                   const float clear_color[4], const Control* ctl);

void launch_encode_srgb8(hipStream_t stream, const float4* framebuffer, uint32_t* default_out, uint32_t pixels,
                         const FrameParams* d_fp, uint32_t out_format = 1u);

void launch_pack_cloud(hipStream_t stream, const uint4* pos, const uint4* a, uint32_t v4_a, const uint4* b, uint32_t v4_b,
                       const uint4* c, uint32_t v4_c, uint4* out, uint32_t stride_v4, uint32_t n);

void launch_particle_step(hipStream_t stream, void* behaviors, uint32_t count, const CloudPtrs& cloud, float dt);

void launch_triad(hipStream_t stream, float4* a, const float4* b, const float4* c, float s, size_t n4,
                  int blocks);

void launch_selftest_ln(hipStream_t stream, uint32_t first_bits, uint32_t count, float* out, unsigned long long* sum,
                        int blocks);

}
```

### bevy_gaussian_splatting_amd/csrc/sort_kernels.hip

```cpp
#include <hip/hip_runtime.h>
#include <type_traits>

#include "kernels.h"
#include "lookback.h"
#include "splat_math.h"

namespace bgs {

namespace {

__device__ __forceinline__ uint32_t ld_agent(const uint32_t* p) {
    return __hip_atomic_load(p, __ATOMIC_RELAXED, __HIP_MEMORY_SCOPE_AGENT);
}
__device__ __forceinline__ void st_agent(uint32_t* p, uint32_t v) {
    __hip_atomic_store(p, v, __ATOMIC_RELAXED, __HIP_MEMORY_SCOPE_AGENT);
}

__device__ __forceinline__ uint32_t wave_inclusive_scan(uint32_t v, int lane) {
#pragma unroll
    for (int off = 1; off < 64; off <<= 1) {
        uint32_t t = __shfl_up(v, off, 64);
        if (lane >= off) v += t;
    }
    return v;
}

__device__ __forceinline__ uint32_t block_exclusive_scan_256(uint32_t v, uint32_t* s_tot,
                                                             uint32_t& total) {
    const int lane = threadIdx.x & 63, wave = threadIdx.x >> 6;
    const uint32_t inc = wave_inclusive_scan(v, lane);
    if (lane == 63) s_tot[wave] = inc;
    __syncthreads();
    const uint32_t w0 = s_tot[0], w1 = s_tot[1], w2 = s_tot[2], w3 = s_tot[3];
    const uint32_t woff = wave == 0 ? 0u : (wave == 1 ? w0 : (wave == 2 ? w0 + w1 : w0 + w1 + w2));
    total = w0 + w1 + w2 + w3;
    __syncthreads();
    return woff + inc - v;
}


}

#ifndef BGS_KG_GROUP
#define BGS_KG_GROUP 2
#endif
template <int KG_ITEMS, bool BUCKET, int THREADS, bool ORDERED = true>
__global__ __launch_bounds__(THREADS, (THREADS == 1024 && ORDERED) ? 8 : 1) void keygen_kernel(FrameParams fp, const float4* __restrict__ pos,
                                                         uint2* __restrict__ entries,
                                                         uint2* __restrict__ culled, Control* ctl,
                                                         uint32_t* part_status, uint32_t places,
                                                         uint32_t ticket_slot, FrameParams* fp_out,
                                                         uint2* __restrict__ bucket_slots, uint32_t* bucket_status,
                                                         SplitterTable split, uint32_t* zero_word) {
    constexpr int WAVES = THREADS / 64;
    constexpr int ROWS = KG_ITEMS * WAVES;
    static_assert((THREADS == 256 || THREADS == 512 || THREADS == 1024) && ROWS <= 128, "tile geometry");
    __shared__ uint32_t s_hist[BUCKET ? 1 : 4][RADIX_BASE];
    __shared__ uint32_t s_cnt[ROWS];
    __shared__ uint32_t s_off[ROWS];
    __shared__ uint32_t s_keys[THREADS * KG_ITEMS];
    __shared__ uint32_t s_idx[BUCKET ? THREADS * KG_ITEMS : 1];
    extern __shared__ uint32_t s_dyn[];
    uint32_t* const s_bcnt = s_dyn;
    uint32_t* const s_bexcl = s_dyn;
    uint32_t* const s_split = s_dyn + (BUCKET ? BUCKET_COUNT * split.sub : 0u);
    __shared__ uint16_t s_at[BUCKET ? THREADS * KG_ITEMS : 1];
    __shared__ uint16_t s_bk[BUCKET ? THREADS * KG_ITEMS : 1];
    __shared__ uint32_t s_total;
    __shared__ uint32_t s_base;
    __shared__ uint32_t s_tile;
    const int tid = threadIdx.x, lane = tid & 63, wave = tid >> 6;
    if (fp_out && blockIdx.x == 0 && (uint32_t)tid < (uint32_t)(sizeof(FrameParams) / 4u))
        reinterpret_cast<uint32_t*>(fp_out)[tid] = reinterpret_cast<const uint32_t*>(&fp)[tid];
    if (zero_word && blockIdx.x == 0 && tid == 0) *zero_word = 0u;
    const uint32_t nsub = BUCKET ? split.sub : 1u, nb = BUCKET_COUNT * nsub;
    const uint32_t bucket_cap = (BUCKET && split.wide != 0u) ? BUCKET_CAP_WIDE : BUCKET_CAP;
    uint32_t p2 = 256u;
    while (p2 < nb) p2 <<= 1;
    if constexpr (BUCKET) {
        const uint32_t* __restrict__ keys = nsub <= BUCKET_SUB_KERNARG ? split.key : split.device_keys;
        for (uint32_t t = (uint32_t)tid; t < p2; t += (uint32_t)THREADS)
            s_split[t] = t < nb - 1u ? keys[t] : 0xFFFFFFFFu;
    } else if (tid < 256) {
#pragma unroll
        for (int p = 0; p < 4; ++p) s_hist[p][tid] = 0u;
    }
    const uint32_t sentinel = KEY_CULLED >> fp.key_shift;
    constexpr uint32_t per_tile = (uint32_t)(THREADS * KG_ITEMS);
    const uint32_t num_tiles = (fp.n + per_tile - 1u) / per_tile;
    const unsigned long long lanes_below = (1ull << lane) - 1ull;
    const bool single_shot = gridDim.x >= num_tiles;

    auto bucket_of = [&](const uint32_t kk) -> uint32_t {
        uint32_t lo = 0u;
        if (nsub == 1u) {
#pragma unroll
            for (uint32_t step = 128u; step > 0u; step >>= 1)
                if (s_split[lo + step - 1u] <= kk) lo += step;
        } else if (p2 == 512u) {
#pragma unroll
            for (uint32_t step = 256u; step > 0u; step >>= 1)
                if (s_split[lo + step - 1u] <= kk) lo += step;
        } else if (p2 == 1024u) {
#pragma unroll
            for (uint32_t step = 512u; step > 0u; step >>= 1)
                if (s_split[lo + step - 1u] <= kk) lo += step;
        } else {
            for (uint32_t step = p2 >> 1; step > 0u; step >>= 1)
                if (s_split[lo + step - 1u] <= kk) lo += step;
        }
        return min(lo, nb - 1u);
    };
    auto claim_bucket_slots = [&]() {
        if (nb <= (uint32_t)THREADS) {
            if ((uint32_t)tid < nb) {
                const uint32_t mine = s_bcnt[tid];
                s_bexcl[tid] = mine ? atomicAdd(&ctl->bucket_count[tid], mine) : 0u;
            }
            return;
        }
        for (uint32_t f0 = (uint32_t)tid; f0 < nb; f0 += 8u * (uint32_t)THREADS) {
            uint32_t ex[8];
#pragma unroll
            for (uint32_t k = 0; k < 8u; ++k) {
                const uint32_t f = f0 + k * (uint32_t)THREADS;
                const uint32_t mine = f < nb ? s_bcnt[f] : 0u;
                ex[k] = mine ? atomicAdd(&ctl->bucket_count[f], mine) : 0u;
            }
#pragma unroll
            for (uint32_t k = 0; k < 8u; ++k) {
                const uint32_t f = f0 + k * (uint32_t)THREADS;
                if (f < nb) s_bexcl[f] = ex[k];
            }
        }
    };
    if constexpr (BUCKET && !ORDERED) {
        if (blockIdx.x == 0 && tid == 0) ctl->splat_count = fp.n;
        for (uint32_t tile = blockIdx.x; tile < num_tiles; tile += gridDim.x) {
            for (uint32_t f = (uint32_t)tid; f < nb; f += (uint32_t)THREADS) s_bcnt[f] = 0u;
            if (tid == 0) s_total = 0u;
            __syncthreads();
            const uint32_t base = tile * per_tile;
            float4 pin[KG_ITEMS];
#pragma unroll
            for (int k = 0; k < KG_ITEMS; ++k) {
                const uint32_t i = base + (uint32_t)(k * THREADS) + (uint32_t)tid;
                pin[k] = i < fp.n ? pos[i] : make_float4(0.0f, 0.0f, 0.0f, 0.0f);
            }
            uint32_t key[KG_ITEMS], below[KG_ITEMS], rowoff[KG_ITEMS];
            const bool all_draw = fp.sort_mode != SORT_RADIX;
#define BGS_KG_KEYS(KIND)                                                                      \
    _Pragma("unroll") for (int k0 = 0; k0 < KG_ITEMS; k0 += BGS_KG_GROUP) {                    \
         \
        uint32_t unsure_mask = 0u;                                                             \
        _Pragma("unroll") for (int k = k0; k < k0 + BGS_KG_GROUP; ++k) {                       \
            const uint32_t i = base + (uint32_t)(k * THREADS) + (uint32_t)tid;                 \
            const float4 p = pin[k];                                                           \
            bool unsure;                                                                       \
            const uint32_t kf = sort_key_fast<KIND>(fp, V3{p.x, p.y, p.z}, unsure);            \
            key[k] = i < fp.n ? kf : sentinel;                                                 \
            unsure_mask |= (unsure && i < fp.n) ? (1u << (k - k0)) : 0u;                       \
        }                                                                                      \
        if (unsure_mask) {                                                                     \
            _Pragma("unroll") for (int k = k0; k < k0 + BGS_KG_GROUP; ++k)                     \
                if ((unsure_mask >> (k - k0)) & 1u) key[k] = sort_key_kind<KIND>(fp, V3{pin[k].x, pin[k].y, pin[k].z}); \
        }                                                                                      \
    }
            if (fp.sort_mode == SORT_RADIX) { BGS_KG_KEYS(1) }
            else if (fp.sort_mode == SORT_NONE) { BGS_KG_KEYS(0) }
            else { BGS_KG_KEYS(2) }
#undef BGS_KG_KEYS
#define BGS_KG_DRAWN(k) (all_draw ? (base + (uint32_t)((k) * THREADS) + (uint32_t)tid < fp.n) : (key[k] != sentinel))
            uint32_t run = 0u;
#pragma unroll
            for (int k = 0; k < KG_ITEMS; ++k) {
                const unsigned long long b = __ballot(BGS_KG_DRAWN(k));
                below[k] = (uint32_t)__popcll(b & lanes_below);
                rowoff[k] = run;
                run += (uint32_t)__popcll(b);
            }
            uint32_t wbase = 0u;
            if (lane == 0 && run) wbase = atomicAdd(&s_total, run);
            wbase = (uint32_t)__shfl((int)wbase, 0, 64);
#pragma unroll
            for (int k = 0; k < KG_ITEMS; ++k)
                if (BGS_KG_DRAWN(k)) {
                    const uint32_t j = wbase + rowoff[k] + below[k];
                    s_keys[j] = key[k];
                    s_idx[j] = base + (uint32_t)(k * THREADS) + (uint32_t)tid;
                }
#undef BGS_KG_DRAWN
            __syncthreads();
            const uint32_t total = s_total;
#pragma unroll
            for (int r = 0; r < KG_ITEMS; ++r) {
                const uint32_t j = (uint32_t)(r * THREADS) + (uint32_t)tid;
                if (j < total) {
                    const uint32_t bkt = bucket_of(s_keys[j]);
                    s_bk[j] = (uint16_t)bkt;
                    s_at[j] = (uint16_t)min(atomicAdd(&s_bcnt[bkt], 1u), 0xFFFFu);
                }
            }
            __syncthreads();
            claim_bucket_slots();
            __syncthreads();
#pragma unroll
            for (int r = 0; r < KG_ITEMS; ++r) {
                const uint32_t j = (uint32_t)(r * THREADS) + (uint32_t)tid;
                if (j < total) {
                    const uint32_t bkt = s_bk[j];
                    const uint32_t slot = s_bexcl[bkt] + (uint32_t)s_at[j];
                    if (slot < bucket_cap)
                        bucket_slots[(size_t)bkt * bucket_cap + slot] = make_uint2(s_keys[j], s_idx[j]);
                }
            }
        }
        return;
    }

    for (;;) {
        if (tid == 0) s_tile = atomicAdd(&ctl->ticket[ticket_slot][0], 1u);
        if constexpr (BUCKET) { for (uint32_t f = (uint32_t)tid; f < nb; f += (uint32_t)THREADS) s_bcnt[f] = 0u; }
        __syncthreads();
        const uint32_t tile = s_tile;
        if (tile >= num_tiles) break;
        const uint32_t base = tile * per_tile;
        uint32_t key[KG_ITEMS], below[KG_ITEMS];
        const bool all_draw = fp.sort_mode != SORT_RADIX;
#define BGS_KG_DRAWN(k) (all_draw ? (base + (uint32_t)((k) * THREADS) + (uint32_t)tid < fp.n) : (key[k] != sentinel))
        float4 pin[KG_ITEMS];
#pragma unroll
        for (int k = 0; k < KG_ITEMS; ++k) {
            const uint32_t i = base + (uint32_t)(k * THREADS) + (uint32_t)tid;
            pin[k] = i < fp.n ? pos[i] : make_float4(0.0f, 0.0f, 0.0f, 0.0f);
        }
#define BGS_KG_KEYS(KIND)                                                                      \
    _Pragma("unroll") for (int k = 0; k < KG_ITEMS; ++k) {                                     \
         \
        const uint32_t i = base + (uint32_t)(k * THREADS) + (uint32_t)tid;                     \
        const float4 p = pin[k];                                                               \
        key[k] = i < fp.n ? sort_key_kind<KIND>(fp, V3{p.x, p.y, p.z}) : sentinel;             \
    }
        if (fp.sort_mode == SORT_RADIX) { BGS_KG_KEYS(1) }
        else if (fp.sort_mode == SORT_NONE) { BGS_KG_KEYS(0) }
        else { BGS_KG_KEYS(2) }
#undef BGS_KG_KEYS
        if constexpr (BUCKET && KG_ITEMS <= 8) {
            if (all_draw && base + per_tile <= fp.n) {
                uint32_t bkat[KG_ITEMS];
#pragma unroll
                for (int k = 0; k < KG_ITEMS; ++k) {
                    const uint32_t bkt = bucket_of(key[k]);
                    bkat[k] = bkt | (atomicAdd(&s_bcnt[bkt], 1u) << 16);
                }
                if (tid == 0 && tile == num_tiles - 1u) { ctl->draw_count = fp.n; ctl->splat_count = fp.n; }
                __syncthreads();
                claim_bucket_slots();
                __syncthreads();
#pragma unroll
                for (int k = 0; k < KG_ITEMS; ++k) {
                    const uint32_t bkt = bkat[k] & 0xFFFFu, slot = s_bexcl[bkt] + (bkat[k] >> 16);
                    if (slot < bucket_cap)
                        bucket_slots[(size_t)bkt * bucket_cap + slot] = make_uint2(key[k], base + (uint32_t)(k * THREADS) + (uint32_t)tid);
                }
                if (single_shot) break;
                __syncthreads();
                continue;
            }
        }
#pragma unroll
        for (int k = 0; k < KG_ITEMS; ++k) {
            const unsigned long long b = __ballot(BGS_KG_DRAWN(k));
            below[k] = (uint32_t)__popcll(b & lanes_below);
            if (lane == 0) s_cnt[k * WAVES + wave] = (uint32_t)__popcll(b);
        }
        __syncthreads();
        if (wave == 0) {
            const uint32_t c0 = lane < ROWS ? s_cnt[lane] : 0u;
            const uint32_t c1 = ROWS > 64 && lane + 64 < ROWS ? s_cnt[lane + 64] : 0u;
            const uint32_t i0 = wave_inclusive_scan(c0, lane);
            const uint32_t t0 = (uint32_t)__shfl((int)i0, 63, 64);
            if (lane < ROWS) s_off[lane] = i0 - c0;
            uint32_t t1 = 0u;
            if constexpr (ROWS > 64) {
                const uint32_t i1 = wave_inclusive_scan(c1, lane);
                t1 = (uint32_t)__shfl((int)i1, 63, 64);
                if (lane + 64 < ROWS) s_off[lane + 64] = t0 + i1 - c1;
            }
            if (lane == 0) s_total = t0 + t1;
        }
        __syncthreads();
        uint32_t off[KG_ITEMS];
#pragma unroll
        for (int k = 0; k < KG_ITEMS; ++k) off[k] = s_off[k * WAVES + wave];
        const uint32_t total = s_total;
#pragma unroll
        for (int k = 0; k < KG_ITEMS; ++k)
            if (BGS_KG_DRAWN(k)) {
                s_keys[off[k] + below[k]] = key[k];
                if constexpr (BUCKET) s_idx[off[k] + below[k]] = base + (uint32_t)(k * THREADS) + (uint32_t)tid;
            }
        {
            if (wave == 0) {
                uint32_t* const my_status = part_status + tile;
                uint32_t excl = 0u;
                if (tile > 0u) {
                    if (lane == 0) st_agent(my_status, STATUS_AGGREGATE | total);
                    excl = all_draw ? tile * per_tile : lookback_wave(part_status, tile, lane, &ctl->error, 8u);
                }
                if (lane == 0) {
                    st_agent(my_status, STATUS_PREFIX | ((excl + total) & STATUS_VALUE_MASK));
                    s_base = excl;
                    if (tile == num_tiles - 1u) {
                        ctl->draw_count = excl + total;
                        ctl->splat_count = fp.n;
                    }
                }
            }
            __syncthreads();
            if constexpr (!BUCKET)
                for (uint32_t j = (uint32_t)tid; j < total; j += (uint32_t)THREADS) {
                    const uint32_t kk = s_keys[j];
                    for (uint32_t pl = 0; pl < places; ++pl)
                        atomicAdd(&s_hist[pl][(kk >> (RADIX_BITS * pl)) & (RADIX_BASE - 1u)], 1u);
                }
        }
        if constexpr (BUCKET) {
#pragma unroll
            for (int r = 0; r < KG_ITEMS; ++r) {
                const uint32_t j = (uint32_t)(r * THREADS) + (uint32_t)tid;
                if (j < total) {
                    const uint32_t bkt = bucket_of(s_keys[j]);
                    s_bk[j] = (uint16_t)bkt;
                    s_at[j] = (uint16_t)min(atomicAdd(&s_bcnt[bkt], 1u), 0xFFFFu);
                }
            }
            __syncthreads();
            claim_bucket_slots();
            __syncthreads();
#pragma unroll
            for (int r = 0; r < KG_ITEMS; ++r) {
                const uint32_t j = (uint32_t)(r * THREADS) + (uint32_t)tid;
                if (j < total) {
                    const uint32_t bkt = s_bk[j];
                    const uint32_t slot = s_bexcl[bkt] + (uint32_t)s_at[j];
                    if (slot < bucket_cap)
                        bucket_slots[(size_t)bkt * bucket_cap + slot] = make_uint2(s_keys[j], s_idx[j]);
                }
            }
        }
        {
        const uint32_t vis_base = s_base;
#pragma unroll
        for (int k = 0; k < KG_ITEMS; ++k) {
            const uint32_t i = base + (uint32_t)(k * THREADS) + (uint32_t)tid;
            if (i < fp.n) {
                const uint32_t before = vis_base + off[k] + below[k];
                if (BGS_KG_DRAWN(k)) { if constexpr (!BUCKET) entries[before] = make_uint2(key[k], i); }
                else if (culled) {
                    typedef uint32_t v2u __attribute__((ext_vector_type(2)));
                    __builtin_nontemporal_store((v2u){key[k], i}, reinterpret_cast<v2u*>(culled + (i - before)));
                }
            }
        }
        }
#undef BGS_KG_DRAWN
        if (single_shot) break;
        __syncthreads();
    }
    if constexpr (!BUCKET) {
        __syncthreads();
        if (tid < 256)
            for (uint32_t pl = 0; pl < places; ++pl) {
                const uint32_t v = s_hist[pl][tid];
                if (v) atomicAdd(&ctl->hist_depth[pl][tid], v);
            }
    }
}

bool KeygenLaunch::prepare(int max_blocks) {
    if (fp.n == 0) return false;
    const bool bucket = fp.sort_path == 1u;
    const bool unordered = bucket && culled == nullptr;
#ifndef BGS_KG_UNORDERED_TILE
#define BGS_KG_UNORDERED_TILE 0
#endif
    const uint32_t per_block = (unordered && BGS_KG_UNORDERED_TILE) ? (uint32_t)BGS_KG_UNORDERED_TILE : keygen_tile_splats(fp.n);
#define BGS_KG_PICK(ITEMS, THR) \
    (bucket ? (unordered ? reinterpret_cast<const void*>(&keygen_kernel<ITEMS, true, THR, false>)                       \
                         : reinterpret_cast<const void*>(&keygen_kernel<ITEMS, true, THR, true>))                       \
            : reinterpret_cast<const void*>(&keygen_kernel<ITEMS, false, THR, true>))
#if BGS_KEYGEN_WIDE_THREADS == 256
    threads = 256u;
    func = per_block >= 4096u ? BGS_KG_PICK(16, 256) : BGS_KG_PICK(8, 256);
#else
    threads = per_block >= 4096u ? 1024u : 256u;
    func = per_block == 8192u ? BGS_KG_PICK(8, 1024) : (per_block == 4096u ? BGS_KG_PICK(4, 1024) : BGS_KG_PICK(8, 256));
#endif
    if (bucket && wide && per_block == 4096u) {
        threads = 1024u;
        func = unordered ? reinterpret_cast<const void*>(&keygen_kernel<4, true, 1024, false>)
                         : reinterpret_cast<const void*>(&keygen_kernel<4, true, 1024, true>);
    }
#undef BGS_KG_PICK
    blocks = (fp.n + per_block - 1) / per_block;
    if (!unordered && blocks > (uint32_t)max_blocks) blocks = (uint32_t)max_blocks;
    argv[0] = &fp; argv[1] = &pos; argv[2] = &entries; argv[3] = &culled; argv[4] = &ctl;
    argv[5] = &part_status; argv[6] = &places; argv[7] = &ticket_slot; argv[8] = &fp_out; argv[9] = &bucket_slots;
    argv[10] = &bucket_status; argv[11] = &split; argv[12] = &zero_word;
    if (split.sub < 1u || split.sub > BUCKET_SUB_MAX) split.sub = 1u;
    {
        uint32_t nbk = BUCKET_COUNT * split.sub, pad2 = 256u;
        while (pad2 < nbk) pad2 <<= 1;
        lds_bytes = bucket ? (nbk + pad2) * (uint32_t)sizeof(uint32_t) : 0u;
    }
    return true;
}

hipError_t KeygenLaunch::launch(hipStream_t stream) {
    if (lds_bytes > 12288u) {
        const hipError_t e = hipFuncSetAttribute(func, hipFuncAttributeMaxDynamicSharedMemorySize, (int)lds_bytes);
        if (e != hipSuccess) return e;
    }
    return hipLaunchKernel(func, dim3(blocks), dim3(threads), argv, lds_bytes, stream);
}

hipError_t KeygenLaunch::update_node(hipGraphExec_t exec, hipGraphNode_t node) {
    hipKernelNodeParams np{};
    np.func = const_cast<void*>(func);
    np.gridDim = dim3(blocks);
    np.blockDim = dim3(threads);
    np.sharedMemBytes = lds_bytes;
    np.kernelParams = argv;
    np.extra = nullptr;
    return hipGraphExecKernelNodeSetParams(exec, node, &np);
}

__global__ __launch_bounds__(256) void histogram_kernel(const uint2* __restrict__ pairs, uint32_t n,
                                                        uint32_t* hist, uint32_t passes) {
    __shared__ uint32_t s_hist[4][RADIX_BASE];
    const int tid = threadIdx.x;
#pragma unroll
    for (int p = 0; p < 4; ++p) s_hist[p][tid] = 0u;
    __syncthreads();
    for (uint32_t i = blockIdx.x * 256u + tid; i < n; i += gridDim.x * 256u) {
        const uint32_t key = pairs[i].x;
        for (uint32_t pl = 0; pl < passes; ++pl)
            atomicAdd(&s_hist[pl][(key >> (RADIX_BITS * pl)) & (RADIX_BASE - 1u)], 1u);
    }
    __syncthreads();
    for (uint32_t pl = 0; pl < passes; ++pl) {
        const uint32_t v = s_hist[pl][tid];
        if (v) atomicAdd(&hist[pl * RADIX_BASE + tid], v);
    }
}

void launch_histogram(hipStream_t stream, const uint2* pairs, uint32_t n, uint32_t* hist,
                      uint32_t passes) {
    if (n == 0) return;
    uint32_t blocks = (n + 256u * 16u - 1) / (256u * 16u);
    if (blocks > 1024u) blocks = 1024u;
    hipLaunchKernelGGL(histogram_kernel, dim3(blocks), dim3(256), 0, stream, pairs, n, hist, passes);
}

#ifndef BGS_ONESWEEP_WAVES
#define BGS_ONESWEEP_WAVES 0
#endif
template <int KPT>
#if BGS_ONESWEEP_WAVES
__global__ __launch_bounds__(256, BGS_ONESWEEP_WAVES) void onesweep_kernel(
#else
__global__ __launch_bounds__(256) void onesweep_kernel(
#endif
const uint2* __restrict__ in,
                                                       uint2* __restrict__ out,
                                                       const uint32_t* __restrict__ n_ptr,
                                                       const uint32_t* __restrict__ hist,
                                                       uint32_t* status, uint32_t* ticket,
                                                       uint32_t* error_flag, uint32_t shift,
                                                       uint32_t key_xor) {
    constexpr uint32_t TILE = 256u * KPT;
    __shared__ uint2 s_pairs[TILE];
    __shared__ uint32_t s_wave_hist[4][RADIX_BASE];
    __shared__ uint32_t s_global_base[RADIX_BASE];
    __shared__ uint32_t s_hist_excl[RADIX_BASE];
    __shared__ uint32_t s_tot[4];
    __shared__ uint32_t s_tile;

    const int tid = threadIdx.x, lane = tid & 63, wave = tid >> 6;
    const uint32_t h = hist[tid];
    const uint32_t n = *n_ptr;
    const uint32_t num_tiles = (n + TILE - 1u) / TILE;
    if (num_tiles == 0u) return;

    {
        uint32_t total;
        s_hist_excl[tid] = block_exclusive_scan_256(h, s_tot, total);
    }
    const bool single_shot = gridDim.x >= num_tiles;

    for (;;) {
        if (tid == 0) s_tile = atomicAdd(ticket, 1u);
#pragma unroll
        for (int w = 0; w < 4; ++w) s_wave_hist[w][tid] = 0u;
        __syncthreads();
        const uint32_t tile = s_tile;
        if (tile >= num_tiles) break;
        auto process = [&](auto full_c) {
            constexpr bool FULL = decltype(full_c)::value;
            const uint32_t tile_base = tile * TILE;
            const uint32_t row_base = tile_base + (uint32_t)wave * (uint32_t)(KPT * 64) + (uint32_t)lane;

            uint2 kv[KPT];
            uint32_t rank[KPT];
    #pragma unroll
            for (int k = 0; k < KPT; ++k) {
                const uint32_t idx = row_base + (uint32_t)k * 64u;
                kv[k] = (FULL || idx < n) ? in[idx] : make_uint2(0xFFFFFFFFu, 0xFFFFFFFFu);
            }
            uint32_t* const wh = s_wave_hist[wave];
    #pragma unroll
            for (int k = 0; k < KPT; ++k) {
                const uint32_t idx = row_base + (uint32_t)k * 64u;
                const bool valid = FULL || idx < n;
                const uint32_t d = (kv[k].x >> shift) & (RADIX_BASE - 1u);
                const unsigned long long mv = FULL ? ~0ull : __ballot(valid);
                uint32_t m_lo = (uint32_t)mv, m_hi = (uint32_t)(mv >> 32);
    #pragma unroll
                for (int b = 0; b < 8; ++b) {
                    const int32_t seli = __builtin_amdgcn_sbfe((int32_t)d, (uint32_t)b, 1u);
                    const uint32_t sel = (uint32_t)seli;
                    const unsigned long long bal = __builtin_amdgcn_ballot_w64(seli < 0);
                    m_lo &= ~((uint32_t)bal ^ sel);
                    m_hi &= ~((uint32_t)(bal >> 32) ^ sel);
                }
                const uint32_t below = __builtin_amdgcn_mbcnt_hi(m_hi, __builtin_amdgcn_mbcnt_lo(m_lo, 0u));
                const uint32_t prev = __atomic_load_n(&wh[d], __ATOMIC_RELAXED);
                __builtin_amdgcn_wave_barrier();
                if (valid && below == 0u) __atomic_store_n(&wh[d], prev + (uint32_t)__popc(m_lo) + (uint32_t)__popc(m_hi), __ATOMIC_RELAXED);
                __builtin_amdgcn_wave_barrier();
                rank[k] = prev + below;
            }
            __syncthreads();

            uint32_t total;
            {
                const uint32_t c0 = s_wave_hist[0][tid], c1 = s_wave_hist[1][tid];
                const uint32_t c2 = s_wave_hist[2][tid], c3 = s_wave_hist[3][tid];
                s_wave_hist[0][tid] = 0u;
                s_wave_hist[1][tid] = c0;
                s_wave_hist[2][tid] = c0 + c1;
                s_wave_hist[3][tid] = c0 + c1 + c2;
                total = c0 + c1 + c2 + c3;
            }
            uint32_t* const my_status = status + (size_t)tile * RADIX_BASE + tid;
            uint32_t excl = 0u;
            if (tile > 0u) {
                st_agent(my_status, STATUS_AGGREGATE | total);
                excl = num_tiles > 1024u ? lookback_u32<16>(status + tid, tile, RADIX_BASE, error_flag, 1u)
                                         : lookback_u32<4>(status + tid, tile, RADIX_BASE, error_flag, 1u);
            }
            st_agent(my_status, STATUS_PREFIX | ((excl + total) & STATUS_VALUE_MASK));

            uint32_t blk_total;
            const uint32_t bexcl = block_exclusive_scan_256(total, s_tot, blk_total);
            s_global_base[tid] = s_hist_excl[tid] + excl - bexcl;
    #pragma unroll
            for (int w = 0; w < 4; ++w) s_wave_hist[w][tid] += bexcl;
            __syncthreads();

    #pragma unroll
            for (int k = 0; k < KPT; ++k) {
                const uint32_t idx = row_base + (uint32_t)k * 64u;
                if (FULL || idx < n) {
                    const uint32_t d = (kv[k].x >> shift) & (RADIX_BASE - 1u);
                    const uint32_t slot = s_wave_hist[wave][d] + rank[k];
                    s_pairs[slot] = kv[k];
                }
            }
            __syncthreads();
            const uint32_t count = FULL ? TILE : min(TILE, n - tile_base);
    #pragma unroll
            for (int k = 0; k < KPT; ++k) {
                const uint32_t slot = (uint32_t)k * 256u + (uint32_t)tid;
                if (FULL || slot < count) {
                    uint2 e = s_pairs[slot];
                    const uint32_t d = (e.x >> shift) & (RADIX_BASE - 1u);
                    e.x ^= key_xor;
                    const uint32_t dst = s_global_base[d] + slot;
                    if (dst < n) out[dst] = e;
                }
            }
        };
        if ((tile + 1u) * TILE <= n) process(std::true_type{}); else process(std::false_type{});
        if (single_shot) break;
        __syncthreads();
    }
}

void launch_onesweep_pass(hipStream_t stream, const uint2* in, uint2* out, const uint32_t* n_ptr,
                          uint32_t max_n, const uint32_t* hist, uint32_t* status, uint32_t* ticket,
                          uint32_t* error_flag, uint32_t shift, uint32_t key_xor, bool large_tiles,
                          int max_blocks) {
    if (max_n == 0) return;
    const uint32_t tile = sort_tile_size(large_tiles);
    uint32_t blocks = (max_n + tile - 1u) / tile;
    if (blocks > (uint32_t)max_blocks) blocks = (uint32_t)max_blocks;
    if (large_tiles)
        hipLaunchKernelGGL(onesweep_kernel<SORT_KPT_LARGE>, dim3(blocks), dim3(256), 0, stream, in, out,
                           n_ptr, hist, status, ticket, error_flag, shift, key_xor);
    else
        hipLaunchKernelGGL(onesweep_kernel<SORT_KPT_SMALL>, dim3(blocks), dim3(256), 0, stream, in, out,
                           n_ptr, hist, status, ticket, error_flag, shift, key_xor);
}

#ifndef BGS_BUCKET_SORT_THREADS
#define BGS_BUCKET_SORT_THREADS 256
#endif
constexpr uint32_t BUCKET_SORT_THREADS = BGS_BUCKET_SORT_THREADS;
template <uint32_t THREADS, uint32_t CAP, uint32_t NF>
__global__ __launch_bounds__(THREADS) void bucket_sort_kernel(const uint2* __restrict__ slots,
                                                              uint2* __restrict__ out, Control* ctl,
                                                              uint32_t key_xor, uint32_t nb ) {
    constexpr uint32_t WAVES = THREADS / 64u;
    constexpr uint32_t EPT = CAP / THREADS;
    constexpr uint32_t FPT = NF / THREADS;
    constexpr bool PACK = NF > 4096u;
    constexpr uint32_t FWORDS = PACK ? NF / 2u + 1u : NF + 1u;
    static_assert((NF == 2048u || NF == 4096u || NF == 8192u) && BUCKET_COUNT == 256u && (THREADS == 256u || THREADS == 1024u) &&
                  EPT >= 1u && FPT >= 2u && FPT % 2u == 0u && CAP <= 65535u, "bucket geometry");
    extern __shared__ uint2 s_el[];
    __shared__ uint32_t s_f[FWORDS];
    __shared__ uint32_t s_tot[WAVES];
    __shared__ uint32_t s_red[WAVES][2];

    const int tid = threadIdx.x, lane = tid & 63, wave = tid >> 6;
    const uint32_t b = blockIdx.x;
    uint32_t before = 0u, mine = 0u, mx = 0u;
    for (uint32_t i = (uint32_t)tid; i < nb; i += THREADS) {
        const uint32_t cnt = ctl->bucket_count[i];
        before += i < b ? cnt : 0u;
        mine += i == b ? cnt : 0u;
        mx = max(mx, cnt);
    }
#pragma unroll
    for (int off = 32; off > 0; off >>= 1) {
        before += (uint32_t)__shfl_xor((int)before, off, 64);
        mine += (uint32_t)__shfl_xor((int)mine, off, 64);
        mx = max(mx, (uint32_t)__shfl_xor((int)mx, off, 64));
    }
    if (lane == 0) { s_red[wave][0] = before; s_red[wave][1] = mine; s_tot[wave] = mx; }
    for (uint32_t j = (uint32_t)tid; j < FWORDS; j += THREADS) s_f[j] = 0u;
    __syncthreads();
    uint32_t base = 0u, m = 0u;
    mx = 0u;
#pragma unroll
    for (uint32_t w = 0; w < WAVES; ++w) { base += s_red[w][0]; m += s_red[w][1]; mx = max(mx, s_tot[w]); }
    if (b == 0u && tid == 0) {
        ctl->bucket_max = mx;
        if (mx > CAP) {
            ctl->sort_overflow = 1u;
            ctl->draw_count = 0u;
        }
    }
    if (b == nb - 1u && tid == 0 && mx <= CAP) ctl->draw_count = base + m;
    if (m == 0u || mx > CAP) return;
    __syncthreads();

    const uint2* __restrict__ src = slots + (size_t)b * CAP;
    uint2 kv[EPT];
    uint32_t kmn = 0xFFFFFFFFu, kmx = 0u;
#pragma unroll
    for (uint32_t k = 0; k < EPT; ++k) {
        const uint32_t e = k * THREADS + (uint32_t)tid;
        kv[k] = make_uint2(0u, 0u);
        if (e < m) {
            kv[k] = src[e];
            kmn = min(kmn, kv[k].x);
            kmx = max(kmx, kv[k].x);
        }
    }
#pragma unroll
    for (int off = 32; off > 0; off >>= 1) {
        kmn = min(kmn, (uint32_t)__shfl_xor((int)kmn, off, 64));
        kmx = max(kmx, (uint32_t)__shfl_xor((int)kmx, off, 64));
    }
    if (lane == 0) { s_red[wave][0] = kmn; s_red[wave][1] = kmx; }
    __syncthreads();
    kmn = 0xFFFFFFFFu; kmx = 0u;
#pragma unroll
    for (uint32_t w = 0; w < WAVES; ++w) { kmn = min(kmn, s_red[w][0]); kmx = max(kmx, s_red[w][1]); }
    const uint32_t span = kmx - kmn;
    const bool direct = span < NF;
    const uint32_t scale = direct ? 0u : (uint32_t)(((unsigned long long)NF << 32) / ((unsigned long long)span + 1ull));
    auto fine_of = [&](const uint32_t key) -> uint32_t { const uint32_t d = key - kmn; return direct ? d : __umulhi(d, scale); };

    uint32_t slot[EPT];
#pragma unroll
    for (uint32_t k = 0; k < EPT; ++k) {
        const uint32_t e = k * THREADS + (uint32_t)tid;
        if (e < m) {
            const uint32_t fb = fine_of(kv[k].x);
            if constexpr (PACK) slot[k] = fb | (((atomicAdd(&s_f[fb >> 1], 1u << ((fb & 1u) << 4)) >> ((fb & 1u) << 4)) & 0xFFFFu) << 16);
            else slot[k] = fb | (atomicAdd(&s_f[fb], 1u) << 16);
        }
    }
    __syncthreads();
    uint32_t f[FPT], fsum = 0u, fmax = 0u;
#pragma unroll
    for (uint32_t j = 0; j < FPT; ++j) {
        if constexpr (PACK) f[j] = (s_f[((uint32_t)tid * FPT + j) >> 1] >> ((j & 1u) << 4)) & 0xFFFFu;
        else f[j] = s_f[(uint32_t)tid * FPT + j];
// ... 133 lines not shown
```

### bevy_gaussian_splatting_amd/plugin.py

```python
from __future__ import annotations

import ctypes
from dataclasses import dataclass
from typing import Optional, Union

import numpy as np

from . import _native
from .camera import View
from .gaussian import PlanarGaussian3d, PlanarGaussian3dF16, PlanarGaussian4d
from .particles import PARTICLE_BEHAVIOR_DTYPE, ParticleBehaviors, ParticleBehaviorsHandle
from .settings import CloudSettings
from .sparse_select import SparseSelect, selected_indices

SORT_ENTRY_DTYPE = np.dtype([("key", np.uint32), ("index", np.uint32)])


@dataclass
class SortedEntries:

    camera_count: int
    entry_count: int
    sorted: np.ndarray

# ... 354 lines not shown

    def sort(self, handle: PlanarGaussian3dHandle, view: View, settings: CloudSettings,
             download: bool = True, into: Optional[DeviceEntriesChunk] = None) -> Optional[np.ndarray]:
        v, s = _with_entries(view.to_native(), into), settings.to_native()
        if download:
            out = np.empty(handle.n, dtype=SORT_ENTRY_DTYPE)
            ptr = out.ctypes.data_as(ctypes.POINTER(_native.BgsSortEntry))
        else:
            out, ptr = None, None
        self._check(self._lib.bgs_sort(self._ctx, handle._ptr, ctypes.byref(v), ctypes.byref(s), ptr))
        return out

    def sort_cameras(self, handle: PlanarGaussian3dHandle, views, settings: CloudSettings,
                     sorted_entries: Optional[SortedEntries] = None, camera_indices=None) -> SortedEntries:
        views = list(views)
        idx = list(range(len(views))) if camera_indices is None else [int(i) for i in camera_indices]
        if len(idx) != len(views):
            raise ValueError("camera_indices must match views")
        count = (max(idx) + 1) if idx else 0
        if sorted_entries is None:
            sorted_entries = SortedEntries.for_cloud(count, handle.n)
        if count > sorted_entries.camera_count:
            raise ValueError("sorted_entries has fewer camera chunks than the camera indices need")
        for view, ci in zip(views, idx):
            chunk = sorted_entries.chunk(ci, handle.n)
            v, s = view.to_native(), settings.to_native()
            tmp = np.empty(handle.n, dtype=SORT_ENTRY_DTYPE)
            self._check(self._lib.bgs_sort(self._ctx, handle._ptr, ctypes.byref(v), ctypes.byref(s),
                                           tmp.ctypes.data_as(ctypes.POINTER(_native.BgsSortEntry))))
            chunk[:] = tmp
        return sorted_entries

    def prepare(self, view: View, settings: CloudSettings) -> "PreparedView":
        return PreparedView(view.to_native(), settings.to_native(), view.width, view.height)

    def render(self, handle: PlanarGaussian3dHandle, view, settings: Optional[CloudSettings] = None,
               download: bool = True, entries: Optional[DeviceEntriesChunk] = None) -> Optional[np.ndarray]:
        if isinstance(view, PreparedView):
            v, s = view.view, view.settings
        else:
            v, s = view.to_native(), settings.to_native()
        v = _with_entries(v, entries)
        if download:
            out = np.empty((view.height, view.width, 4), dtype=np.float32)
            ptr = _fptr(out)
        else:
            out, ptr = None, None
        self._check(self._lib.bgs_render(self._ctx, handle._ptr, ctypes.byref(v), ctypes.byref(s), ptr))
        return out

    def device_sorted_entries(self, camera_count: int, handle: PlanarGaussian3dHandle) -> DeviceSortedEntries:
        return DeviceSortedEntries(self, camera_count, handle.n)

    def render_with_trigger(self, handle: PlanarGaussian3dHandle, view: View, settings: CloudSettings, trigger,
                            chunk: DeviceEntriesChunk, download: bool = True) -> Optional[np.ndarray]:
        if trigger.needs_sort:
            self.sort(handle, view, settings, download=False, into=chunk)
            trigger.needs_sort = False
        return self.render(handle, view, settings, download=download, entries=chunk)

    def radix_sort_pairs(self, keys: np.ndarray, passes: int = 4) -> np.ndarray:
        keys = np.ascontiguousarray(keys, dtype=np.uint32)
        e = np.empty(keys.shape[0], dtype=SORT_ENTRY_DTYPE)
        e["key"] = keys
        e["index"] = np.arange(keys.shape[0], dtype=np.uint32)
        self._check(
            self._lib.bgs_radix_sort_pairs(
                self._ctx, e.ctypes.data_as(ctypes.POINTER(_native.BgsSortEntry)),
                keys.shape[0], int(passes)))
        return e

    def hbm_probe(self, nbytes: int = 1 << 29, iters: int = 20):
        c, t = ctypes.c_float(), ctypes.c_float()
        self._check(self._lib.bgs_hbm_probe(self._ctx, int(nbytes), int(iters), ctypes.byref(c), ctypes.byref(t)))
        return float(c.value), float(t.value)

    def selftest_ln(self, first_bits: int, count: int, download: Optional[bool] = None):
        if download is None:
            download = count <= (1 << 24)
        out = np.empty(count, np.float32) if download else None
        chk = ctypes.c_uint64()
        self._check(self._lib.bgs_selftest_ln_f32(
            self._ctx, int(first_bits), int(count),
            out.ctypes.data_as(ctypes.POINTER(ctypes.c_float)) if download else None, ctypes.byref(chk)))
        return out, int(chk.value)

    def selftest_pack(self, fmt: str, device_in: int, pixels: int, device_out: int) -> None:
        code = fmt if isinstance(fmt, int) else {"srgb8": 1, "rgba16f": 2}[fmt]
        self._check(self._lib.bgs_selftest_pack(self._ctx, code, device_in or None, int(pixels), device_out or None))

    def debug_frame_records(self) -> dict:
        info = _native.BgsFrameRecordsInfo()
        self._check(self._lib.bgs_debug_frame_records(self._ctx, None, 0, None, 0, ctypes.byref(info)))
        count, words = int(info.draw_count), int(info.record_stride) // 4
        records = np.zeros((count, words), np.uint32)
        rects = np.zeros(count, np.uint32)
        self._check(self._lib.bgs_debug_frame_records(self._ctx, records.ctypes.data_as(ctypes.c_void_p), records.nbytes,
                                                      _uptr(rects), count, ctypes.byref(info)))
        if int(info.draw_count) != count:
            raise RuntimeError("the frame changed between the two calls of bgs_debug_frame_records")
        return {"draw_count": count, "record_stride": int(info.record_stride), "records": records,
                "rects": rects if info.has_rects else None, "visible_count": int(info.visible_count),
                "color_max_bits": int(info.color_max_bits)}

    def set_pipeline_streams(self, streams: int) -> None:
        self._check(self._lib.bgs_set_pipeline_streams(self._ctx, int(streams)))

    def set_graphs(self, enabled: bool) -> None:
        self._check(self._lib.bgs_set_graphs(self._ctx, 1 if enabled else 0))

    def graph_counters(self) -> tuple:
        c, r = ctypes.c_uint64(), ctypes.c_uint64()
        self._check(self._lib.bgs_graph_counters(self._ctx, ctypes.byref(c), ctypes.byref(r)))
        return int(c.value), int(r.value)

    def tile_order_counters(self) -> tuple:
        c, r, n = ctypes.c_uint64(), ctypes.c_uint64(), ctypes.c_uint64()
        self._check(self._lib.bgs_tile_order_counters(self._ctx, ctypes.byref(c), ctypes.byref(r), ctypes.byref(n)))
        return int(c.value), int(r.value), int(n.value)

    def selftest_tile_order(self, cost: np.ndarray, runs: int = 1, sums: bool = False):
        c = np.ascontiguousarray(cost, dtype=np.uint16)
        out = np.empty((c.size + 3) // 4, np.uint16)
        two = np.zeros(2, np.uint32)
        self._check(self._lib.bgs_selftest_tile_order(self._ctx, c.ctypes.data_as(ctypes.c_void_p), c.size, runs,
                                                      out.ctypes.data_as(ctypes.c_void_p), two.ctypes.data_as(ctypes.c_void_p)))
        return (out, (int(two[0]), int(two[1]))) if sums else out

    def synchronize(self) -> None:
        self._check(self._lib.bgs_synchronize(self._ctx))

    def set_profiling(self, level: int) -> None:
        self._check(self._lib.bgs_set_profiling(self._ctx, int(level)))

    def set_profiling_stride(self, every_nth_frame: int) -> None:
        self._check(self._lib.bgs_set_profiling_stride(self._ctx, int(every_nth_frame)))

    def set_pipeline_depth(self, lanes: int) -> None:
        self._check(self._lib.bgs_set_pipeline_depth(self._ctx, int(lanes)))

    def set_output_srgb8(self, enabled: bool) -> None:
        self._check(self._lib.bgs_set_output_srgb8(self._ctx, 1 if enabled else 0))

    def set_srgb8_target(self, device_ptr: Optional[int]) -> None:
        self._check(self._lib.bgs_set_srgb8_target(self._ctx, ctypes.c_void_p(device_ptr or 0)))

    def set_output_rgba16f(self, enabled: bool) -> None:
        self._check(self._lib.bgs_set_output_rgba16f(self._ctx, 1 if enabled else 0))

    def set_packed_only(self, enabled: bool) -> None:
        self._check(self._lib.bgs_set_packed_only(self._ctx, 1 if enabled else 0))

    def framebuffer_rgba16f_device_ptr(self):
        p = ctypes.c_void_p()
        nbytes = ctypes.c_uint64()
        self._check(self._lib.bgs_framebuffer_rgba16f_device_ptr(self._ctx, ctypes.byref(p), ctypes.byref(nbytes)))
        return p.value, nbytes.value

    def framebuffer_srgb8_device_ptr(self):
        p = ctypes.c_void_p()
        nbytes = ctypes.c_uint64()
        self._check(self._lib.bgs_framebuffer_srgb8_device_ptr(self._ctx, ctypes.byref(p), ctypes.byref(nbytes)))
        return p.value, nbytes.value

    def pipeline_pop(self):
        a, b = ctypes.c_void_p(), ctypes.c_void_p()
        self._check(self._lib.bgs_pipeline_pop(self._ctx, ctypes.byref(a), ctypes.byref(b)))
        return a.value, b.value

    def frames_in_flight(self) -> int:
        c = ctypes.c_uint32()
        self._check(self._lib.bgs_frames_in_flight(self._ctx, ctypes.byref(c)))
        return int(c.value)

    def set_async(self, enabled: bool) -> None:
        self._check(self._lib.bgs_set_async(self._ctx, 1 if enabled else 0))

    def set_binning(self, mode: str) -> None:
        self._check(self._lib.bgs_set_binning(self._ctx, {"scan": 0, "sort": 1}[mode]))

    def set_debug_flags(self, flags: int) -> None:
        self._check(self._lib.bgs_set_debug_flags(self._ctx, int(flags)))

    def draw_list(self) -> np.ndarray:
        p, n = ctypes.c_void_p(), ctypes.c_uint32()
        self._check(self._lib.bgs_sorted_entries_device_ptr(self._ctx, ctypes.byref(p), ctypes.byref(n)))
        out = np.empty(n.value, dtype=np.dtype([("key", np.uint32), ("index", np.uint32)]))
        if n.value:
            self._check(self._lib.bgs_download(self._ctx, p, out.ctypes.data_as(ctypes.c_void_p), out.nbytes))
        return out

    def device_alloc(self, nbytes: int) -> int:
        p = ctypes.c_void_p()
        self._check(self._lib.bgs_device_alloc(self._ctx, int(nbytes), ctypes.byref(p)))
        return int(p.value or 0)

    def device_free(self, device_ptr: int) -> None:
        self._check(self._lib.bgs_device_free(self._ctx, ctypes.c_void_p(device_ptr)))

    def upload_bytes(self, device_ptr: int, host: np.ndarray) -> None:
        a = np.ascontiguousarray(host)
        self._check(self._lib.bgs_upload(self._ctx, ctypes.c_void_p(device_ptr), a.ctypes.data_as(ctypes.c_void_p), a.nbytes))

    def download(self, device_ptr: int, host_out: np.ndarray) -> np.ndarray:
        if not host_out.flags["C_CONTIGUOUS"] or not host_out.flags["WRITEABLE"]:
            raise ValueError("host_out must be a writeable C-contiguous array")
        self._check(self._lib.bgs_download(self._ctx, ctypes.c_void_p(device_ptr), host_out.ctypes.data_as(ctypes.c_void_p),
                                           host_out.nbytes))
        return host_out

    def upload_depth(self, depth: np.ndarray) -> int:
        d = np.ascontiguousarray(depth, dtype=np.float32)
        if d.ndim != 3 or d.shape[2] not in (1, 2, 4, 8):
            raise ValueError("depth must be [height, width, samples] with 1, 2, 4 or 8 samples")
        p = self.device_alloc(d.nbytes)
        self.upload_bytes(p, d)
        return p

    def set_tile_trace(self, device_ptr: Optional[int]) -> None:
        self._check(self._lib.bgs_set_tile_trace(self._ctx, ctypes.c_void_p(device_ptr or 0)))

    def build_id(self) -> str:
        return self._lib.bgs_build_id().decode()

    def adaptive_counters(self) -> dict:
        out = (ctypes.c_uint64 * 8)()
        self._check(self._lib.bgs_adaptive_counters(self._ctx, out))
        names = ("bucket_frames", "onesweep_frames", "reruns_sort", "reruns_lists", "reruns_instances",
                 "level_changes", "supertile_level", "list_capacity_hint")
        return {k: int(v) for k, v in zip(names, out)}

    def learning_counters(self) -> dict:
        a, b = ctypes.c_uint64(), ctypes.c_uint64()
        self._check(self._lib.bgs_learning_counters(self._ctx, ctypes.byref(a), ctypes.byref(b)))
        return {"early_frames": a.value, "kinds_settled": b.value}

    @staticmethod
    def comm_unique_id() -> bytes:
        buf = ctypes.create_string_buffer(_native.COMM_ID_BYTES)
        lib = _native.load()
        _native.check(lib, None, lib.bgs_comm_unique_id(buf))
        return buf.raw

    def comm_create(self, unique_id: bytes, world_size: int, rank: int) -> int:
        if len(unique_id) != _native.COMM_ID_BYTES:
            raise ValueError("unique_id must be the 128 bytes of comm_unique_id()")
        out = ctypes.c_void_p()
        self._check(self._lib.bgs_comm_create(self._ctx, unique_id, int(world_size), int(rank), ctypes.byref(out)))
        return out.value

    def comm_gather(self, comm: int, root: int, send_ptr: int, nbytes: int, recv_ptr: Optional[int]) -> int:
        ticket = ctypes.c_uint64()
        self._check(self._lib.bgs_comm_gather(self._ctx, comm, int(root), ctypes.c_void_p(send_ptr), int(nbytes),
                                              ctypes.c_void_p(recv_ptr or 0), ctypes.byref(ticket)))
        return ticket.value

    def comm_gather_after(self, comm: int, root: int, send_ptr: int, nbytes: int, recv_ptr: Optional[int],
                          hip_stream: Optional[int] = None) -> int:
        t = ctypes.c_uint64(0)
        self._check(self._lib.bgs_comm_gather_after(self._ctx, comm, int(root), ctypes.c_void_p(send_ptr), int(nbytes),
                                                    ctypes.c_void_p(recv_ptr or 0), ctypes.c_void_p(hip_stream or 0), ctypes.byref(t)))
        return int(t.value)

    def comm_wait(self, comm: int, ticket: int = 0) -> None:
        self._check(self._lib.bgs_comm_wait(self._ctx, comm, int(ticket)))

    def comm_destroy(self, comm: int) -> None:
        self._lib.bgs_comm_destroy(self._ctx, comm)

    def reset_adaptive_state(self) -> None:
        self._check(self._lib.bgs_reset_adaptive_state(self._ctx))

    def framebuffer_device_ptr(self):
        p = ctypes.c_void_p()
        nbytes = ctypes.c_uint64()
        self._check(self._lib.bgs_framebuffer_device_ptr(self._ctx, ctypes.byref(p), ctypes.byref(nbytes)))
        return p.value, nbytes.value

    def stream_handle(self) -> int:
        p = ctypes.c_void_p()
        self._check(self._lib.bgs_stream(self._ctx, ctypes.byref(p)))
        return p.value or 0

    def stats(self) -> dict:
        st = _native.BgsStats()
        self._check(self._lib.bgs_get_stats(self._ctx, ctypes.byref(st)))
        d = {
            "total_ms": float(st.total_ms),
            "splat_count": int(st.splat_count),
            "visible_count": int(st.visible_count),
            "draw_count": int(st.draw_count),
            "instance_count": int(st.instance_count),
            "instance_capacity": int(st.instance_capacity),
            "list_entries_allocated": int(st.list_entries_allocated),
            "strip_tiles": int(st.strip_tiles),
            "tile_saturation": {"known": bool((int(st.tile_saturation) >> 16) & 1), "work_share": (int(st.tile_saturation) & 0x7FFF) / 0x7FFF,
                                "midround_exit": bool(int(st.tile_saturation) >> 31)},
            "tiles": (int(st.tiles_x), int(st.tiles_y)),
            "depth_passes": int(st.depth_passes),
            "tile_passes": int(st.tile_passes),
            "algorithmic_bytes": int(st.algorithmic_bytes),
            "regrow_count": int(st.regrow_count),
            "sort_path": ("onesweep", "bucket", "kept")[int(st.sort_path)],
            "list_capacity": int(st.list_capacity),
            "binning": "sort" if st.binning_mode else "scan",
            "frames_averaged": int(st.frames_averaged),
            "stage_ms": {n: float(st.stage_ms[i]) for i, n in enumerate(_native.STAGE_NAMES)},
        }
        return d
```

### include/bgs.h

```cpp
#ifndef BGS_H
#define BGS_H

#include <stdint.h>

#ifdef __cplusplus
extern "C" {
#endif

#define BGS_VERSION_MAJOR 0
#define BGS_VERSION_MINOR 4

typedef enum bgs_status {
    BGS_OK = 0,
    BGS_EINVAL = -1,
    BGS_ENOMEM = -2,
    BGS_EHIP = -3,
    BGS_ECAPACITY = -4,
    BGS_EINTERNAL = -5
} bgs_status;

typedef struct bgs_ctx bgs_ctx;
typedef struct bgs_cloud bgs_cloud;

typedef struct bgs_view {
    float world_from_view[16];
    float view_from_world[16];
    float clip_from_view[16];
    float clip_from_world[16];
    float viewport[4];
    float clear_color[4];
    float previous_clip_from_world[16];
    float delta_time;
    uint32_t sample_count;
    uint32_t entry_count;
    uint32_t reserved[1];
    uint64_t depth_device_ptr;
    uint64_t entries_device_ptr;
} bgs_view;

#define BGS_GAUSSIAN_2D 0u
#define BGS_GAUSSIAN_3D 1u
#define BGS_COLOR_SRGB 0u
#define BGS_COLOR_LINEAR 1u
#define BGS_SORT_NONE 0u
#define BGS_SORT_RADIX 1u
#define BGS_SORT_RAYON 2u
#define BGS_SORT_STD 3u

#define BGS_RASTERIZE_CLASSIFICATION 0u
#define BGS_RASTERIZE_COLOR 1u
#define BGS_RASTERIZE_DEPTH 2u
#define BGS_RASTERIZE_NORMAL 3u
#define BGS_RASTERIZE_OPTICAL_FLOW 4u
#define BGS_RASTERIZE_POSITION 5u
#define BGS_RASTERIZE_VELOCITY 6u

#define BGS_DRAW_ALL 0u
#define BGS_DRAW_SELECTED 1u
#define BGS_DRAW_HIGHLIGHT_SELECTED 2u

typedef struct bgs_settings {
    float transform[16];
    float global_opacity;
    float global_scale;
    uint32_t gaussian_mode;
    uint32_t aabb;
    uint32_t opacity_adaptive_radius;
    uint32_t color_space;
    uint32_t radix_depth_bits;
    uint32_t sh_degree;
    uint32_t sort_mode;
    uint32_t rasterize_mode;
    uint32_t num_classes;
    uint32_t draw_mode;
    uint32_t visualize_bounding_box;
    uint32_t reserved[1];
    float position_min[4];
    float position_max[4];
} bgs_settings;

typedef struct bgs_sort_entry {
    uint32_t key;
    uint32_t index;
} bgs_sort_entry;

#define BGS_STAGE_KEYGEN 0
#define BGS_STAGE_DEPTH_SORT 1
#define BGS_STAGE_PROJECT 2
#define BGS_STAGE_TILE_SORT 3
#define BGS_STAGE_RANGES 4
#define BGS_STAGE_RASTER 5
#define BGS_STAGE_COUNT 6

typedef struct bgs_stats {
    float stage_ms[BGS_STAGE_COUNT];
    float total_ms;
    uint32_t splat_count;
    uint32_t visible_count;
    uint32_t draw_count;
    uint32_t sort_path;
    uint64_t instance_count;
    uint64_t instance_capacity;
    uint32_t tiles_x, tiles_y;
    uint32_t depth_passes;
    uint32_t tile_passes;
    uint64_t algorithmic_bytes;
    uint32_t regrow_count;
    uint32_t binning_mode;
    uint32_t frames_averaged;
    uint32_t list_capacity;
    uint64_t list_entries_allocated;
    uint32_t strip_tiles;
    uint32_t tile_saturation;
} bgs_stats;

int bgs_create(int hip_device, bgs_ctx** out);
void bgs_destroy(bgs_ctx* ctx);
const char* bgs_last_error(const bgs_ctx* ctx);
uint32_t bgs_version(void);
#define BGS_ABI_VERSION ((BGS_VERSION_MAJOR << 16) | BGS_VERSION_MINOR)
int bgs_abi_check(uint32_t version, uint32_t sizeof_view, uint32_t sizeof_settings, uint32_t sizeof_stats);
const char* bgs_build_id(void);

void bgs_settings_default(bgs_settings* out);

void bgs_view_perspective(const float world_from_view[16], float fov_y_radians,
                          float near_plane, uint32_t width, uint32_t height,
                          bgs_view* out);

int bgs_cloud_upload_f32(bgs_ctx* ctx, uint32_t n, const float* position_visibility,
                         const float* spherical_harmonic, const float* rotation,
                         const float* scale_opacity, bgs_cloud** out);
int bgs_cloud_upload_f16(bgs_ctx* ctx, uint32_t n, const float* position_visibility,
                         const uint32_t* spherical_harmonic_h2,
                         const uint32_t* rotation_scale_opacity, bgs_cloud** out);
int bgs_cloud_upload_cov3d_f32(bgs_ctx* ctx, uint32_t n, const float* position_visibility,
                               const float* spherical_harmonic, const float* covariance_3d_opacity,
                               bgs_cloud** out);
void bgs_cloud_free(bgs_ctx* ctx, bgs_cloud* cloud);
uint32_t bgs_cloud_len(const bgs_cloud* cloud);

typedef struct bgs_particle_behavior {
    uint32_t indicies[4];
    float velocity[4];
    float acceleration[4];
    float jerk[4];
} bgs_particle_behavior;
int bgs_cloud_apply_particle_behaviors(bgs_ctx* ctx, bgs_cloud* cloud, void* behaviors_device_ptr, uint32_t count,
                                       float delta_time);

int bgs_sort(bgs_ctx* ctx, const bgs_cloud* cloud, const bgs_view* view,
             const bgs_settings* settings, bgs_sort_entry* host_out);

int bgs_render(bgs_ctx* ctx, const bgs_cloud* cloud, const bgs_view* view,
               const bgs_settings* settings, float* rgba_host_out);

int bgs_framebuffer_device_ptr(bgs_ctx* ctx, void** dptr, uint64_t* bytes);
int bgs_set_output_srgb8(bgs_ctx* ctx, int enabled);
int bgs_framebuffer_srgb8_device_ptr(bgs_ctx* ctx, void** dptr, uint64_t* bytes);
int bgs_set_output_rgba16f(bgs_ctx* ctx, int enabled);
int bgs_framebuffer_rgba16f_device_ptr(bgs_ctx* ctx, void** dptr, uint64_t* bytes);
int bgs_set_packed_only(bgs_ctx* ctx, int enabled);
int bgs_set_srgb8_target(bgs_ctx* ctx, void* device_ptr);
int bgs_download(bgs_ctx* ctx, const void* device_ptr, void* host_out, uint64_t bytes);
int bgs_device_alloc(bgs_ctx* ctx, uint64_t bytes, void** device_ptr_out);
int bgs_device_free(bgs_ctx* ctx, void* device_ptr);
int bgs_upload(bgs_ctx* ctx, void* device_ptr, const void* host_in, uint64_t bytes);

int bgs_set_pipeline_depth(bgs_ctx* ctx, uint32_t lanes );
int bgs_pipeline_pop(bgs_ctx* ctx, void** rgba_f32_dptr_or_null, void** rgba8_dptr_or_null);
int bgs_frames_in_flight(bgs_ctx* ctx, uint32_t* count);

int bgs_sorted_entries_device_ptr(bgs_ctx* ctx, void** dptr, uint32_t* n);

int bgs_synchronize(bgs_ctx* ctx);
int bgs_set_async(bgs_ctx* ctx, int enabled);
int bgs_stream(bgs_ctx* ctx, void** hip_stream);

#define BGS_BINNING_SCAN 0u
#define BGS_BINNING_SORT 1u
int bgs_set_binning(bgs_ctx* ctx, uint32_t mode);

int bgs_reset_adaptive_state(bgs_ctx* ctx);
int bgs_set_profiling(bgs_ctx* ctx, int enabled);
int bgs_set_profiling_stride(bgs_ctx* ctx, uint32_t every_nth_frame);
int bgs_get_stats(bgs_ctx* ctx, bgs_stats* out);

int bgs_set_pipeline_streams(bgs_ctx* ctx, uint32_t streams);
int bgs_set_graphs(bgs_ctx* ctx, int enabled);

#define BGS_COMM_ID_BYTES 128
typedef struct bgs_comm bgs_comm;
int bgs_comm_unique_id(uint8_t id_out[BGS_COMM_ID_BYTES]);
int bgs_comm_create(bgs_ctx* ctx, const uint8_t id[BGS_COMM_ID_BYTES], uint32_t world_size, uint32_t rank, bgs_comm** out);
int bgs_comm_gather(bgs_ctx* ctx, bgs_comm* comm, uint32_t root, const void* send_device_ptr, uint64_t bytes_per_rank,
                    void* recv_device_ptr_root_only, uint64_t* ticket_out_or_null);
int bgs_comm_gather_after(bgs_ctx* ctx, bgs_comm* comm, uint32_t root, const void* send_device_ptr, uint64_t bytes_per_rank,
                          void* recv_device_ptr_root_only, void* hip_stream_or_null, uint64_t* ticket_out_or_null);
int bgs_comm_wait(bgs_ctx* ctx, bgs_comm* comm, uint64_t ticket);
int bgs_comm_stream(bgs_ctx* ctx, bgs_comm* comm, void** hip_stream);
void bgs_comm_destroy(bgs_ctx* ctx, bgs_comm* comm);
#ifdef __cplusplus
}
#endif
#endif
```

### include/bgs_diag.h

```cpp
#ifndef BGS_DIAG_H
#define BGS_DIAG_H

#include "bgs.h"

#ifdef __cplusplus
extern "C" {
#endif

enum bgs_debug_flag {
    BGS_DEBUG_BUCKETS_NARROW = 0x100,
    BGS_DEBUG_SPLIT_SUB_3 = 0x200,
    BGS_DEBUG_SPLIT_SUB_5 = 0x400,
    BGS_DEBUG_BUCKETS_WIDE = 0x800,
    BGS_DEBUG_NO_RASTER_CLEANUP = 0x1000,
    BGS_DEBUG_NO_DRAW_HINT = 0x2000,
    BGS_DEBUG_NO_GRAPHS = 0x4000,
    BGS_DEBUG_LEVEL_1 = 0x8000,
    BGS_DEBUG_LEVEL_0 = 0x10000,
    BGS_DEBUG_MIDROUND_ALWAYS = 0x20000,
    BGS_DEBUG_SEPARATE_ENCODE = 0x40000,
    BGS_DEBUG_NO_BUCKET_SORT = 0x80000,
    BGS_DEBUG_SMALL_LISTS = 0x100000,
    BGS_DEBUG_GUESSED_SPLITTERS = 0x200000,
    BGS_DEBUG_LEVEL_2 = 0x400000,
    BGS_DEBUG_LEVEL_3 = 0x800000,
    BGS_DEBUG_NO_MIDROUND = 0x1000000,
    BGS_DEBUG_NO_STRIPS = 0x2000000,
    BGS_DEBUG_STRIPS_ANY_DEPTH = 0x4000000,
    BGS_DEBUG_RERUN_EVERY_FRAME = 0x8000000,
    BGS_DEBUG_NO_TILE_COST = 0x10000000,
    BGS_DEBUG_NO_TILE_COST_PIPELINED = 0x20000000,
    BGS_DEBUG_ORDER_EVERY_FRAME = 0x40000000
};
int bgs_set_debug_flags(bgs_ctx* ctx, uint32_t flags);

int bgs_adaptive_counters(bgs_ctx* ctx, uint64_t out[8]);

int bgs_learning_counters(bgs_ctx* ctx, uint64_t* early_frames, uint64_t* kinds_settled);

int bgs_radix_sort_pairs(bgs_ctx* ctx, bgs_sort_entry* entries_inout, uint32_t n,
                         uint32_t passes);

int bgs_hbm_probe(bgs_ctx* ctx, uint64_t bytes, uint32_t iters, float* copy_gbs, float* triad_gbs);

int bgs_selftest_ln_f32(bgs_ctx* ctx, uint32_t first_bits, uint32_t count, float* host_out, uint64_t* checksum_out);

int bgs_set_queue_holders(int enabled);

int bgs_set_tile_trace(bgs_ctx* ctx, void* device_ptr);

int bgs_graph_counters(bgs_ctx* ctx, uint64_t* captures, uint64_t* replays);

int bgs_tile_order_counters(bgs_ctx* ctx, uint64_t* cost_frames, uint64_t* ordered_frames, uint64_t* refreshes);

int bgs_selftest_tile_order(bgs_ctx* ctx, const uint16_t* host_cost, uint32_t ntiles, uint32_t runs, uint16_t* host_order,
                            uint32_t* host_sums);

enum bgs_pack_format { BGS_PACK_SRGB8 = 1, BGS_PACK_RGBA16F = 2 };
int bgs_selftest_pack(bgs_ctx* ctx, uint32_t format, const void* device_in_rgba_f32, uint32_t pixels, void* device_out);

typedef struct bgs_frame_records_info {
    uint32_t draw_count, record_stride, has_rects, visible_count, color_max_bits;
} bgs_frame_records_info;
int bgs_debug_frame_records(bgs_ctx* ctx, void* host_records, uint64_t records_capacity_bytes, uint32_t* host_rects,
                            uint32_t rects_capacity_words, bgs_frame_records_info* info_out);

#ifdef __cplusplus
}
#endif
#endif
```

Before: 22380 frames/s.

## Morton-reorder splats into blocks and cull whole blocks in bucket keygen

At cloud upload, a key plane is built: splats are sorted by a Morton code over their bounds and gathered into a reordered position buffer that carries the source index, plus per-256-splat AABBs. In the unordered bucket radix keygen path, each tile tests its blocks' AABBs against conservative frustum planes and skips loading and keying splats in blocks that are certainly culled. The cost is an upload-time sort, extra memory, a reordered read path that writes original indices, and a per-tile ballot test. The frame path keeps a 'rested' counter so the plane is built lazily when it is missing.

```diff
diff --git a/bevy_gaussian_splatting_amd/_native.py b/bevy_gaussian_splatting_amd/_native.py
--- a/bevy_gaussian_splatting_amd/_native.py
+++ b/bevy_gaussian_splatting_amd/_native.py
@@ -37,6 +37,7 @@
         ("visible_count", ctypes.c_uint32),
         ("draw_count", ctypes.c_uint32),
         ("sort_path", ctypes.c_uint32),
+        ("block_walk", ctypes.c_uint32),
         ("instance_count", ctypes.c_uint64),
         ("instance_capacity", ctypes.c_uint64),
         ("tiles_x", ctypes.c_uint32),
diff --git a/bevy_gaussian_splatting_amd/csrc/bgs_api.hip b/bevy_gaussian_splatting_amd/csrc/bgs_api.hip
--- a/bevy_gaussian_splatting_amd/csrc/bgs_api.hip
+++ b/bevy_gaussian_splatting_amd/csrc/bgs_api.hip
@@ -164,12 +164,13 @@
         }
     }
     if (rc != BGS_OK) { bgs_cloud_free(ctx, c); return rc; }
-    c->bytes = (size_t)n * 16 + (size_t)n * 16 * stride_v4;
     c->ptrs.position_visibility = (const float4*)c->positions.ptr;
     c->ptrs.packed = (const uint4*)c->packed.ptr;
     c->ptrs.packed_v4 = stride_v4;
     c->ptrs.n = n;
     c->ptrs.format = format;
+    if ((rc = build_key_plane(ctx, c, ctx->lanes[0].stream)) != BGS_OK) { bgs_cloud_free(ctx, c); return rc; }
+    c->bytes = (size_t)n * 16 + (size_t)n * 16 * stride_v4 + c->key_plane.ordered.capacity * sizeof(float4) + c->key_plane.bounds.capacity * sizeof(float);
     *out = c;
     return BGS_OK;
 }
diff --git a/bevy_gaussian_splatting_amd/csrc/bgs_context.h b/bevy_gaussian_splatting_amd/csrc/bgs_context.h
--- a/bevy_gaussian_splatting_amd/csrc/bgs_context.h
+++ b/bevy_gaussian_splatting_amd/csrc/bgs_context.h
@@ -49,9 +49,16 @@
 
 }
 
+struct KeyPlane {
+    bgs_host::DeviceBuffer<float4> ordered;
+    bgs_host::DeviceBuffer<float> bounds;
+    bool valid = false;
+    uint32_t rested = 0;
+};
 struct bgs_cloud {
     CloudPtrs ptrs{};
     bgs_host::DeviceBuffer<uint8_t> positions, packed;
+    mutable KeyPlane key_plane;
     uint64_t bytes = 0;
 };
 
@@ -105,6 +112,7 @@
     bool render = false, scan = false, surfel = false, culled_tail = true;
     uint32_t n = 0, places = 0, rec_bytes = 0, cloud_format = 0;
     bool bucket = false, wide = false, kept = false;
+    bool block_cull = false, block_walk = false;
     uint32_t bucket_sub = 1, split_sub_out = 1;
     int split_slot = -1;
     uint64_t split_epoch = 0;
@@ -244,6 +252,7 @@
     bool use_graphs = false;
     uint64_t graph_captures = 0, graph_replays = 0;
     uint64_t cost_frames = 0, ordered_frames = 0, order_refreshes = 0;
+    uint64_t block_walk_frames = 0, key_plane_builds = 0;
 
     bool have_stats = false;
     bgs_stats stats{};
@@ -263,6 +272,7 @@
 int ensure_entries(bgs_ctx* ctx, Lane& L, uint32_t n);
 int run(bgs_ctx* ctx, const bgs_cloud* cloud, const bgs_view* view, const bgs_settings* s, bool render);
 int apply_particle_step(bgs_ctx* ctx, bgs_cloud* cloud, void* behaviors, uint32_t count, float dt);
+int build_key_plane(bgs_ctx* ctx, const bgs_cloud* cloud, hipStream_t stream);
 extern int g_queue_holders_mode;
 extern std::mutex g_queue_holders_mutex;
 }
diff --git a/bevy_gaussian_splatting_amd/csrc/bgs_frame.hip b/bevy_gaussian_splatting_amd/csrc/bgs_frame.hip
--- a/bevy_gaussian_splatting_amd/csrc/bgs_frame.hip
+++ b/bevy_gaussian_splatting_amd/csrc/bgs_frame.hip
@@ -440,6 +440,7 @@
     stt.visible_count = render ? h.visible_count : h.draw_count;
     stt.draw_count = h.draw_count;
     stt.sort_path = p.kept ? 2u : (p.bucket ? 1u : 0u);
+    stt.block_walk = p.block_walk ? 1u : 0u;
     stt.list_capacity = (render && scan) ? L.pending_coarse_cap : 0u;
     stt.instance_count = render ? t.instances : 0;
     stt.instance_capacity = L.inst[0].capacity;
@@ -607,6 +608,7 @@
     }
     if (p.bucket && slot >= 0) { p.split_slot = slot; p.split_epoch = ctx.split_slots[slot].epoch; }
     fp.sort_path = p.bucket ? 1u : 0u;
+    p.block_cull = p.bucket && !p.culled_tail && fp.sort_mode == SORT_RADIX && !(flags & BGS_DEBUG_NO_BLOCK_CULL);
     if (p.kept) { fp.sort_mode = SORT_NONE; fp.key_shift = 0u; }
 
     supertile_edges((uint32_t)fp.tiles_x, (uint32_t)fp.tiles_y, p.edges);
@@ -661,7 +663,7 @@
     GraphKey key;
     std::memset(&key, 0, sizeof key);
     const FrameParams& fp = p.fp;
-    const void* planes[6] = {in.cloud->ptrs.position_visibility, in.cloud->ptrs.packed, nullptr, nullptr, nullptr, nullptr};
+    const void* planes[6] = {in.cloud->ptrs.position_visibility, in.cloud->ptrs.packed, kg.pos, kg.block_bounds, nullptr, nullptr};
     std::memcpy(key.cloud, planes, sizeof planes);
     const void* bufs[11] = {L.entries[0].ptr, L.entries[1].ptr, L.culled.ptr, L.records.ptr, L.coarse.ptr, L.fb.ptr, L.fb8.ptr,
                             L.scratch.ptr, L.d_fp.ptr, L.h_ctl_dev, L.bucket_slots.ptr};
@@ -712,6 +714,40 @@
     return BGS_OK;
 }
 
+int build_key_plane(bgs_ctx* ctx, const bgs_cloud* cloud, hipStream_t stream) {
+    KeyPlane& kp = cloud->key_plane;
+    const uint32_t n = cloud->ptrs.n;
+    kp.valid = false;
+    kp.rested = 0;
+    if (n == 0) return BGS_OK;
+    const uint32_t nblk = (n + KG_BLOCK - 1u) / KG_BLOCK;
+    DeviceBuffer<uint2> pairs;
+    DeviceBuffer<uint8_t> work;
+    if (!kp.ordered.reserve(n, 256) || !kp.bounds.reserve((size_t)nblk * KG_BOUNDS_FLOATS, 256) || !pairs.reserve((size_t)n * 2u, 256) ||
+        !work.reserve(key_plane_work_bytes(n), 256))
+        return BGS_OK;
+    uint32_t watchdog = 1u;
+    HIP_TRY(ctx, launch_key_plane_build(stream, cloud->ptrs.position_visibility, n, pairs.ptr, pairs.ptr + n, (uint32_t*)work.ptr,
+                                        kp.ordered.ptr, kp.bounds.ptr, ctx->num_cus * 4));
+    HIP_TRY(ctx, hipMemcpyAsync(&watchdog, (uint32_t*)work.ptr + KEY_PLANE_WATCHDOG_WORD, sizeof watchdog, hipMemcpyDeviceToHost, stream));
+    HIP_TRY(ctx, hipStreamSynchronize(stream));
+    kp.valid = watchdog == 0u;
+    ctx->key_plane_builds += 1;
+    return BGS_OK;
+}
+
+int ensure_key_plane(bgs_ctx* ctx, Lane& L, const bgs_cloud& cloud, bool wanted) {
+    KeyPlane& kp = cloud.key_plane;
+    if (kp.valid || cloud.ptrs.n == 0) return BGS_OK;
+    if (wanted && kp.rested >= 1u) {
+        int rc = lane_create(ctx, L);
+        if (rc != BGS_OK) return rc;
+        return build_key_plane(ctx, &cloud, L.stream);
+    }
+    kp.rested += 1u;
+    return BGS_OK;
+}
+
 int ensure_frame_buffers(bgs_ctx* ctx, Lane& L, const FramePlan& p, const FrameInputs& in, uint32_t* coarse_cap) {
     int rc;
     if ((rc = lane_create(ctx, L)) != BGS_OK) return rc;
@@ -735,7 +771,12 @@
 }
 
 int enqueue_frame(bgs_ctx* ctx, Lane& L, const FrameInputs& in) {
-    const FramePlan p = plan_frame(*ctx, L, in);
+    FramePlan p = plan_frame(*ctx, L, in);
+    {
+        int krc = ensure_key_plane(ctx, L, *in.cloud, p.block_cull);
+        if (krc != BGS_OK) return krc;
+        p.block_walk = p.block_cull && in.cloud->key_plane.valid;
+    }
     const FrameParams& fp = p.fp;
     const uint32_t n = p.n, places = p.places, flags = in.debug_flags;
     const bool render = p.render, scan = p.scan, bucket = p.bucket;
@@ -792,6 +833,11 @@
         kg.split.wide = p.wide ? 1u : 0u;
     }
     kg.wide = p.wide_bin;
+    if (p.block_walk) {
+        kg.pos = in.cloud->key_plane.ordered.ptr;
+        kg.block_bounds = in.cloud->key_plane.bounds.ptr;
+        block_cull_planes(fp, kg.planes);
+    }
     const bool have_keygen = !p.kept && kg.prepare(ctx->num_cus * 4);
     const uint2* const kept_entries = reinterpret_cast<const uint2*>((uintptr_t)in.view.entries_device_ptr);
     FrameCleanup cl{};
@@ -815,6 +861,7 @@
     else if (places > 0) ctx->onesweep_frames += 1;
     if (bucket && p.split_slot >= 0) ctx->split_slots[p.split_slot].last_used = ctx->seq + 1;
     if (p.cost) ctx->cost_frames += 1;
+    if (p.block_walk && have_keygen) ctx->block_walk_frames += 1;
     if (p.ordered) ctx->ordered_frames += 1;
     if (p.refresh) { ctx->order_refreshes += 1; L.order_kind = L.cost_done_kind; L.order_grid = grid; L.order_age = 0; }
     else if (p.ordered) L.order_age += 1u;
@@ -973,6 +1020,8 @@
     }
     if (!ctx->step_done) HIP_TRY(ctx, hipEventCreateWithFlags(&ctx->step_done, hipEventDisableTiming));
     hipStream_t st = ctx->lanes[0].stream;
+    cloud->key_plane.valid = false;
+    cloud->key_plane.rested = 0;
     launch_particle_step(st, behaviors, count, cloud->ptrs, dt);
     HIP_TRY(ctx, hipGetLastError());
     HIP_TRY(ctx, hipEventRecord(ctx->step_done, st));
diff --git a/bevy_gaussian_splatting_amd/csrc/block_cull.h b/bevy_gaussian_splatting_amd/csrc/block_cull.h
--- /dev/null
+++ b/bevy_gaussian_splatting_amd/csrc/block_cull.h
@@ -0,0 +1,88 @@
+#pragma once
+#include "splat_math.h"
+
+namespace bgs {
+
+constexpr uint32_t KG_BLOCK = 256;
+constexpr uint32_t KG_BOUNDS_FLOATS = 6;
+
+BGS_HD uint32_t morton_spread10(uint32_t v) {
+    v &= 0x3FFu;
+    v = (v | (v << 16)) & 0x030000FFu;
+    v = (v | (v << 8)) & 0x0300F00Fu;
+    v = (v | (v << 4)) & 0x030C30C3u;
+    v = (v | (v << 2)) & 0x09249249u;
+    return v;
+}
+BGS_HD bool finite3(V3 p) { return fabsf(p.x) <= 3.402823466e38f && fabsf(p.y) <= 3.402823466e38f && fabsf(p.z) <= 3.402823466e38f; }
+BGS_HD uint32_t morton_axis(float p, float lo, float scale) {
+    const float q = fminf(fmaxf((p - lo) * scale, 0.0f), 1023.0f);
+    return (uint32_t)q;
+}
+BGS_HD uint32_t morton_code(V3 p, const float lo[3], const float scale[3]) {
+    if (!finite3(p)) return 0xFFFFFFFFu;
+    return morton_spread10(morton_axis(p.x, lo[0], scale[0])) | (morton_spread10(morton_axis(p.y, lo[1], scale[1])) << 1) |
+           (morton_spread10(morton_axis(p.z, lo[2], scale[2])) << 2);
+}
+BGS_HD float morton_scale(float lo, float hi) {
+    const float d = hi - lo;
+    return (d > 0.0f && d <= 3.402823466e38f) ? 1023.0f / d : 0.0f;
+}
+
+struct BlockCullPlanes {
+    float a[7][4];
+    float b[7][4];
+};
+
+inline void block_cull_planes(const FrameParams& fp, BlockCullPlanes& P) {
+    const float* M = fp.transform;
+    const float* C = fp.clip_from_world;
+    double A[4][4], Aa[4][4];
+    for (int r = 0; r < 4; ++r)
+        for (int j = 0; j < 4; ++j) {
+            double s = j == 3 ? (double)C[12 + r] : 0.0, sa = j == 3 ? fabs((double)C[12 + r]) : 0.0;
+            for (int i = 0; i < 3; ++i) {
+                s += (double)C[4 * i + r] * (double)M[4 * j + i];
+                sa += fabs((double)C[4 * i + r]) * fabs((double)M[4 * j + i]);
+            }
+            A[r][j] = s; Aa[r][j] = sa;
+        }
+    const double K = (double)1.1f * (1.0 + 0x1p-16), KZ = 1.0 + 0x1p-16, U = 0x1p-18;
+    const int row[7] = {0, 0, 1, 1, 2, 2, 3};
+    const double sign[7] = {1.0, -1.0, 1.0, -1.0, -1.0, 1.0, 1.0};
+    const double kw[7] = {K, K, K, K, 0.0, KZ, 0.0};
+    for (int k = 0; k < 7; ++k)
+        for (int j = 0; j < 4; ++j) {
+            P.a[k][j] = (float)(sign[k] * A[row[k]][j] - kw[k] * A[3][j]);
+            P.b[k][j] = (float)(U * (Aa[row[k]][j] + 1.2 * Aa[3][j]));
+        }
+}
+
+BGS_HD bool block_certainly_culled(const BlockCullPlanes& P, const float lo[3], const float hi[3]) {
+    bool finite = true;
+    float c[3], e[3], pm[3];
+#pragma unroll
+    for (int j = 0; j < 3; ++j) {
+        finite = finite && fabsf(lo[j]) <= 3.402823466e38f && fabsf(hi[j]) <= 3.402823466e38f && lo[j] <= hi[j];
+        c[j] = 0.5f * lo[j] + 0.5f * hi[j];
+        e[j] = 0.5f * hi[j] - 0.5f * lo[j];
+        pm[j] = fmaxf(fabsf(lo[j]), fabsf(hi[j]));
+    }
+    float fmin[7], fmax[7], mar[7];
+#pragma unroll
+    for (int k = 0; k < 7; ++k) {
+        const float cen = ((P.a[k][0] * c[0] + P.a[k][1] * c[1]) + P.a[k][2] * c[2]) + P.a[k][3];
+        const float rad = (fabsf(P.a[k][0]) * e[0] + fabsf(P.a[k][1]) * e[1]) + fabsf(P.a[k][2]) * e[2];
+        mar[k] = (((P.b[k][0] * pm[0] + P.b[k][1] * pm[1]) + P.b[k][2] * pm[2]) + P.b[k][3]) + 1e-8f;
+        fmin[k] = cen - rad;
+        fmax[k] = cen + rad;
+    }
+    const bool front = fmin[6] >= mar[6], behind = fmax[6] <= -mar[6];
+    bool one_plane = false;
+#pragma unroll
+    for (int k = 0; k < 6; ++k) one_plane = one_plane | (fmin[k] >= mar[k]);
+    const bool z_positive = fmax[4] <= -mar[4];
+    return finite & ((front & one_plane) | (behind & z_positive));
+}
+
+}
diff --git a/bevy_gaussian_splatting_amd/csrc/kernels.h b/bevy_gaussian_splatting_amd/csrc/kernels.h
--- a/bevy_gaussian_splatting_amd/csrc/kernels.h
+++ b/bevy_gaussian_splatting_amd/csrc/kernels.h
@@ -3,6 +3,7 @@
 #include <stdint.h>
 
 #include "bgs_device.h"
+#include "block_cull.h"
 
 namespace bgs {
 
@@ -49,9 +50,11 @@
     SplitterTable split;
     uint32_t* zero_word;
     bool wide = false;
+    const float* block_bounds;
+    BlockCullPlanes planes;
     const void* func;
     uint32_t blocks, threads;
-    void* argv[13];
+    void* argv[15];
     uint32_t lds_bytes;
     bool prepare(int max_blocks);
     hipError_t launch(hipStream_t stream);
@@ -64,6 +67,11 @@
 #define BGS_KEYGEN_HUGE_LOG2 (BGS_KEYGEN_WIDE_THREADS == 256 ? 31 : 22)
 #endif
 inline uint32_t keygen_tile_splats(uint32_t n) { return n >= (1u << BGS_KEYGEN_HUGE_LOG2) ? 8192u : (n >= (1u << 19) ? 4096u : 2048u); }
+
+constexpr uint32_t KEY_PLANE_WORK_WORDS = 32u + 4u * RADIX_BASE + 4u * 32u, KEY_PLANE_WATCHDOG_WORD = 7u;
+size_t key_plane_work_bytes(uint32_t n);
+hipError_t launch_key_plane_build(hipStream_t stream, const float4* pos, uint32_t n, uint2* pairs0, uint2* pairs1, uint32_t* work,
+                                  float4* ordered, float* bounds, int max_blocks);
 
 hipError_t launch_entries_compact(hipStream_t stream, const FrameParams& fp, const uint2* entries, uint2* draw_list, uint2* tail,
                                   Control* ctl, uint32_t* part_status, uint32_t ticket_slot, FrameParams* fp_out, uint32_t* zero_word);
diff --git a/bevy_gaussian_splatting_amd/csrc/key_plane_kernels.hip b/bevy_gaussian_splatting_amd/csrc/key_plane_kernels.hip
--- /dev/null
+++ b/bevy_gaussian_splatting_amd/csrc/key_plane_kernels.hip
@@ -0,0 +1,125 @@
+#include <hip/hip_runtime.h>
+
+#include "block_cull.h"
+#include "kernels.h"
+
+namespace bgs {
+
+namespace {
+
+__device__ __forceinline__ uint32_t float_order(float f) {
+    const uint32_t u = __float_as_uint(f);
+    return (u & 0x80000000u) ? ~u : (u | 0x80000000u);
+}
+__device__ __forceinline__ float float_unorder(uint32_t o) {
+    return __uint_as_float((o & 0x80000000u) ? (o & 0x7FFFFFFFu) : ~o);
+}
+
+__device__ __forceinline__ float wave_min(float v) {
+#pragma unroll
+    for (int off = 32; off > 0; off >>= 1) v = fminf(v, __shfl_xor(v, off, 64));
+    return v;
+}
+__device__ __forceinline__ float wave_max(float v) {
+#pragma unroll
+    for (int off = 32; off > 0; off >>= 1) v = fmaxf(v, __shfl_xor(v, off, 64));
+    return v;
+}
+
+__global__ __launch_bounds__(256) void key_plane_bounds_kernel(const float4* __restrict__ pos, uint32_t n, uint32_t* work) {
+    float lo[3] = {INFINITY, INFINITY, INFINITY}, hi[3] = {-INFINITY, -INFINITY, -INFINITY};
+    for (uint32_t i = blockIdx.x * 256u + threadIdx.x; i < n; i += gridDim.x * 256u) {
+        const float4 p = pos[i];
+        if (finite3(V3{p.x, p.y, p.z})) {
+            lo[0] = fminf(lo[0], p.x); lo[1] = fminf(lo[1], p.y); lo[2] = fminf(lo[2], p.z);
+            hi[0] = fmaxf(hi[0], p.x); hi[1] = fmaxf(hi[1], p.y); hi[2] = fmaxf(hi[2], p.z);
+        }
+    }
+#pragma unroll
+    for (int a = 0; a < 3; ++a) {
+        const float l = wave_min(lo[a]), h = wave_max(hi[a]);
+        if ((threadIdx.x & 63u) == 0u && l <= h) {
+            atomicMin(&work[a], float_order(l));
+            atomicMax(&work[3 + a], float_order(h));
+        }
+    }
+}
+
+__global__ __launch_bounds__(256) void key_plane_codes_kernel(const float4* __restrict__ pos, uint32_t n, const uint32_t* __restrict__ work,
+                                                              uint2* __restrict__ pairs) {
+    const uint32_t i = blockIdx.x * 256u + threadIdx.x;
+    if (i >= n) return;
+    float lo[3], scale[3];
+#pragma unroll
+    for (int a = 0; a < 3; ++a) {
+        lo[a] = float_unorder(work[a]);
+        scale[a] = morton_scale(lo[a], float_unorder(work[3 + a]));
+    }
+    const float4 p = pos[i];
+    pairs[i] = make_uint2(morton_code(V3{p.x, p.y, p.z}, lo, scale), i);
+}
+
+__global__ __launch_bounds__(256) void key_plane_gather_kernel(const float4* __restrict__ pos, const uint2* __restrict__ sorted, uint32_t n,
+                                                               float4* __restrict__ ordered, float* __restrict__ bounds) {
+    static_assert(KG_BLOCK == 256u, "one thread per splat of a block");
+    __shared__ float s_red[4][6];
+    __shared__ uint32_t s_bad[4];
+    const uint32_t tid = threadIdx.x, wave = tid >> 6, i = blockIdx.x * KG_BLOCK + tid;
+    float lo[3] = {INFINITY, INFINITY, INFINITY}, hi[3] = {-INFINITY, -INFINITY, -INFINITY};
+    bool bad = false;
+    if (i < n) {
+        const uint32_t src = sorted[i].y;
+        const float4 p = src < n ? pos[src] : make_float4(NAN, NAN, NAN, 0.0f);
+        ordered[i] = make_float4(p.x, p.y, p.z, __uint_as_float(src));
+        if (finite3(V3{p.x, p.y, p.z})) {
+            lo[0] = hi[0] = p.x; lo[1] = hi[1] = p.y; lo[2] = hi[2] = p.z;
+        } else {
+            bad = true;
+        }
+    }
+#pragma unroll
+    for (int a = 0; a < 3; ++a) {
+        const float l = wave_min(lo[a]), h = wave_max(hi[a]);
+        if ((tid & 63u) == 0u) { s_red[wave][a] = l; s_red[wave][3 + a] = h; }
+    }
+    const unsigned long long any_bad = __ballot(bad);
+    if ((tid & 63u) == 0u) s_bad[wave] = any_bad != 0ull ? 1u : 0u;
+    __syncthreads();
+    if (tid < KG_BOUNDS_FLOATS) {
+        float v = s_red[0][tid];
+#pragma unroll
+        for (int w = 1; w < 4; ++w) v = tid < 3u ? fminf(v, s_red[w][tid]) : fmaxf(v, s_red[w][tid]);
+        if (tid == 0u && (s_bad[0] | s_bad[1] | s_bad[2] | s_bad[3])) v = NAN;
+        bounds[(size_t)blockIdx.x * KG_BOUNDS_FLOATS + tid] = v;
+    }
+}
+
+}
+
+size_t key_plane_work_bytes(uint32_t n) {
+    const size_t tiles = ((size_t)n + sort_tile_size(false) - 1u) / sort_tile_size(false);
+    return (KEY_PLANE_WORK_WORDS + 4u * tiles * RADIX_BASE) * sizeof(uint32_t);
+}
+
+hipError_t launch_key_plane_build(hipStream_t stream, const float4* pos, uint32_t n, uint2* pairs0, uint2* pairs1, uint32_t* work,
+                                  float4* ordered, float* bounds, int max_blocks) {
+    if (n == 0) return hipSuccess;
+    hipError_t e = hipMemsetAsync(work, 0, key_plane_work_bytes(n), stream);
+    if (e != hipSuccess) return e;
+    if ((e = hipMemsetAsync(work, 0xFF, 3u * sizeof(uint32_t), stream)) != hipSuccess) return e;
+    if ((e = hipMemsetD32Async((hipDeviceptr_t)(work + 6), (int)n, 1, stream)) != hipSuccess) return e;
+    const uint32_t blocks = (n + 255u) / 256u;
+    hipLaunchKernelGGL(key_plane_bounds_kernel, dim3(blocks < (uint32_t)max_blocks ? blocks : (uint32_t)max_blocks), dim3(256), 0, stream, pos, n, work);
+    hipLaunchKernelGGL(key_plane_codes_kernel, dim3(blocks), dim3(256), 0, stream, pos, n, work, pairs0);
+    uint32_t* const hist = work + 32, * const tickets = hist + 4u * RADIX_BASE, * const status = work + KEY_PLANE_WORK_WORDS;
+    const size_t pass_words = (((size_t)n + sort_tile_size(false) - 1u) / sort_tile_size(false)) * RADIX_BASE;
+    launch_histogram(stream, pairs0, n, hist, 4u);
+    uint2* io[2] = {pairs0, pairs1};
+    for (uint32_t q = 0; q < 4u; ++q)
+        launch_onesweep_pass(stream, io[q & 1u], io[(q & 1u) ^ 1u], work + 6, n, hist + q * RADIX_BASE, status + q * pass_words, tickets + q * 32u,
+                             work + 7, q * RADIX_BITS, 0u, false, max_blocks);
+    hipLaunchKernelGGL(key_plane_gather_kernel, dim3((n + KG_BLOCK - 1u) / KG_BLOCK), dim3(256), 0, stream, pos, pairs0, n, ordered, bounds);
+    return hipGetLastError();
+}
+
+}
diff --git a/bevy_gaussian_splatting_amd/csrc/sort_kernels.hip b/bevy_gaussian_splatting_amd/csrc/sort_kernels.hip
--- a/bevy_gaussian_splatting_amd/csrc/sort_kernels.hip
+++ b/bevy_gaussian_splatting_amd/csrc/sort_kernels.hip
@@ -1,6 +1,7 @@
 #include <hip/hip_runtime.h>
 #include <type_traits>
 
+#include "block_cull.h"
 #include "kernels.h"
 #include "lookback.h"
 #include "splat_math.h"
@@ -44,14 +45,17 @@
 #ifndef BGS_KG_GROUP
 #define BGS_KG_GROUP 2
 #endif
-template <int KG_ITEMS, bool BUCKET, int THREADS, bool ORDERED = true>
+template <int KG_ITEMS, bool BUCKET, int THREADS, bool ORDERED = true, bool BLOCKS = false>
 __global__ __launch_bounds__(THREADS, (THREADS == 1024 && ORDERED) ? 8 : 1) void keygen_kernel(FrameParams fp, const float4* __restrict__ pos,
                                                          uint2* __restrict__ entries,
                                                          uint2* __restrict__ culled, Control* ctl,
                                                          uint32_t* part_status, uint32_t places,
                                                          uint32_t ticket_slot, FrameParams* fp_out,
                                                          uint2* __restrict__ bucket_slots, uint32_t* bucket_status,
-                                                         SplitterTable split, uint32_t* zero_word) {
+                                                         SplitterTable split, uint32_t* zero_word,
+                                                         const float* __restrict__ block_bounds, BlockCullPlanes planes) {
+    static_assert(!BLOCKS || (BUCKET && !ORDERED && (THREADS * KG_ITEMS) % (int)KG_BLOCK == 0 && THREADS * KG_ITEMS <= 32 * (int)KG_BLOCK),
+                  "the block walk: chainless bucket tiles of whole blocks, a keep mask of 32 bits");
     constexpr int WAVES = THREADS / 64;
     constexpr int ROWS = KG_ITEMS * WAVES;
     static_assert((THREADS == 256 || THREADS == 512 || THREADS == 1024) && ROWS <= 128, "tile geometry");
@@ -77,10 +81,13 @@
     const uint32_t bucket_cap = (BUCKET && split.wide != 0u) ? BUCKET_CAP_WIDE : BUCKET_CAP;
     uint32_t p2 = 256u;
     while (p2 < nb) p2 <<= 1;
-    if constexpr (BUCKET) {
+    auto load_splitters = [&]() {
         const uint32_t* __restrict__ keys = nsub <= BUCKET_SUB_KERNARG ? split.key : split.device_keys;
         for (uint32_t t = (uint32_t)tid; t < p2; t += (uint32_t)THREADS)
             s_split[t] = t < nb - 1u ? keys[t] : 0xFFFFFFFFu;
+    };
+    if constexpr (BUCKET) {
+        if constexpr (!BLOCKS) load_splitters();
     } else if (tid < 256) {
 #pragma unroll
         for (int p = 0; p < 4; ++p) s_hist[p][tid] = 0u;
@@ -136,7 +143,25 @@
     };
     if constexpr (BUCKET && !ORDERED) {
         if (blockIdx.x == 0 && tid == 0) ctl->splat_count = fp.n;
+        bool have_splitters = !BLOCKS;
         for (uint32_t tile = blockIdx.x; tile < num_tiles; tile += gridDim.x) {
+            uint32_t keep = 0xFFFFFFFFu;
+            if constexpr (BLOCKS) {
+                constexpr uint32_t BPT = per_tile / KG_BLOCK;
+                const uint32_t blk = tile * BPT + (uint32_t)lane, nblk = (fp.n + KG_BLOCK - 1u) / KG_BLOCK;
+                bool walk = false;
+                if ((uint32_t)lane < BPT && blk < nblk) {
+                    const float* const bb = block_bounds + (size_t)blk * KG_BOUNDS_FLOATS;
+                    const float lo[3] = {bb[0], bb[1], bb[2]}, hi[3] = {bb[3], bb[4], bb[5]};
+                    walk = !block_certainly_culled(planes, lo, hi);
+                }
+                keep = (uint32_t)__ballot(walk);
+                if (keep == 0u) continue;
+                if (have_splitters) __syncthreads();
+                else load_splitters();
+                have_splitters = true;
+            }
+#define BGS_KG_KEPT(k) (!BLOCKS || ((keep >> (((uint32_t)((k) * THREADS) + (uint32_t)__builtin_amdgcn_readfirstlane(wave) * 64u) / KG_BLOCK)) & 1u) != 0u)
             for (uint32_t f = (uint32_t)tid; f < nb; f += (uint32_t)THREADS) s_bcnt[f] = 0u;
             if (tid == 0) s_total = 0u;
             __syncthreads();
@@ -145,7 +170,7 @@
 #pragma unroll
             for (int k = 0; k < KG_ITEMS; ++k) {
                 const uint32_t i = base + (uint32_t)(k * THREADS) + (uint32_t)tid;
-                pin[k] = i < fp.n ? pos[i] : make_float4(0.0f, 0.0f, 0.0f, 0.0f);
+                pin[k] = (i < fp.n && BGS_KG_KEPT(k)) ? pos[i] : make_float4(0.0f, 0.0f, 0.0f, 0.0f);
             }
             uint32_t key[KG_ITEMS], below[KG_ITEMS], rowoff[KG_ITEMS];
             const bool all_draw = fp.sort_mode != SORT_RADIX;
@@ -155,22 +180,26 @@
         uint32_t unsure_mask = 0u;                                                             \
         _Pragma("unroll") for (int k = k0; k < k0 + BGS_KG_GROUP; ++k) {                       \
             const uint32_t i = base + (uint32_t)(k * THREADS) + (uint32_t)tid;                 \
-            const float4 p = pin[k];                                                           \
-            bool unsure;                                                                       \
-            const uint32_t kf = sort_key_fast<KIND>(fp, V3{p.x, p.y, p.z}, unsure);            \
-            key[k] = i < fp.n ? kf : sentinel;                                                 \
-            unsure_mask |= (unsure && i < fp.n) ? (1u << (k - k0)) : 0u;                       \
+            key[k] = sentinel;                                                                 \
+            if (BGS_KG_KEPT(k)) {      \
+                const float4 p = pin[k];                                                       \
+                bool unsure;                                                                   \
+                const uint32_t kf = sort_key_fast<KIND>(fp, V3{p.x, p.y, p.z}, unsure);        \
+                key[k] = i < fp.n ? kf : sentinel;                                             \
+                unsure_mask |= (unsure && i < fp.n) ? (1u << (k - k0)) : 0u;                   \
+            }                                                                                  \
         }                                                                                      \
         if (unsure_mask) {                                                                     \
             _Pragma("unroll") for (int k = k0; k < k0 + BGS_KG_GROUP; ++k)                     \
                 if ((unsure_mask >> (k - k0)) & 1u) key[k] = sort_key_kind<KIND>(fp, V3{pin[k].x, pin[k].y, pin[k].z}); \
         }                                                                                      \
     }
-            if (fp.sort_mode == SORT_RADIX) { BGS_KG_KEYS(1) }
+            if (BLOCKS || fp.sort_mode == SORT_RADIX) { BGS_KG_KEYS(1) }
             else if (fp.sort_mode == SORT_NONE) { BGS_KG_KEYS(0) }
             else { BGS_KG_KEYS(2) }
 #undef BGS_KG_KEYS
-#define BGS_KG_DRAWN(k) (all_draw ? (base + (uint32_t)((k) * THREADS) + (uint32_t)tid < fp.n) : (key[k] != sentinel))
+#undef BGS_KG_KEPT
+#define BGS_KG_DRAWN(k) ((all_draw && !BLOCKS) ? (base + (uint32_t)((k) * THREADS) + (uint32_t)tid < fp.n) : (key[k] != sentinel))
             uint32_t run = 0u;
 #pragma unroll
             for (int k = 0; k < KG_ITEMS; ++k) {
@@ -187,7 +216,7 @@
                 if (BGS_KG_DRAWN(k)) {
                     const uint32_t j = wbase + rowoff[k] + below[k];
                     s_keys[j] = key[k];
-                    s_idx[j] = base + (uint32_t)(k * THREADS) + (uint32_t)tid;
+                    s_idx[j] = BLOCKS ? __float_as_uint(pin[k].w) : base + (uint32_t)(k * THREADS) + (uint32_t)tid;
                 }
 #undef BGS_KG_DRAWN
             __syncthreads();
@@ -382,12 +411,15 @@
     if (fp.n == 0) return false;
     const bool bucket = fp.sort_path == 1u;
     const bool unordered = bucket && culled == nullptr;
+    if (!(unordered && fp.sort_mode == SORT_RADIX)) block_bounds = nullptr;
+    const bool walk = block_bounds != nullptr;
 #ifndef BGS_KG_UNORDERED_TILE
 #define BGS_KG_UNORDERED_TILE 0
 #endif
     const uint32_t per_block = (unordered && BGS_KG_UNORDERED_TILE) ? (uint32_t)BGS_KG_UNORDERED_TILE : keygen_tile_splats(fp.n);
 #define BGS_KG_PICK(ITEMS, THR) \
-    (bucket ? (unordered ? reinterpret_cast<const void*>(&keygen_kernel<ITEMS, true, THR, false>)                       \
+    (bucket ? (unordered ? (walk ? reinterpret_cast<const void*>(&keygen_kernel<ITEMS, true, THR, false, true>)         \
+                                 : reinterpret_cast<const void*>(&keygen_kernel<ITEMS, true, THR, false>))              \
                          : reinterpret_cast<const void*>(&keygen_kernel<ITEMS, true, THR, true>))                       \
             : reinterpret_cast<const void*>(&keygen_kernel<ITEMS, false, THR, true>))
 #if BGS_KEYGEN_WIDE_THREADS == 256
@@ -399,7 +431,8 @@
 #endif
     if (bucket && wide && per_block == 4096u) {
         threads = 1024u;
-        func = unordered ? reinterpret_cast<const void*>(&keygen_kernel<4, true, 1024, false>)
+        func = unordered ? (walk ? reinterpret_cast<const void*>(&keygen_kernel<4, true, 1024, false, true>)
+                                 : reinterpret_cast<const void*>(&keygen_kernel<4, true, 1024, false>))
                          : reinterpret_cast<const void*>(&keygen_kernel<4, true, 1024, true>);
     }
 #undef BGS_KG_PICK
@@ -407,7 +440,7 @@
     if (!unordered && blocks > (uint32_t)max_blocks) blocks = (uint32_t)max_blocks;
     argv[0] = &fp; argv[1] = &pos; argv[2] = &entries; argv[3] = &culled; argv[4] = &ctl;
     argv[5] = &part_status; argv[6] = &places; argv[7] = &ticket_slot; argv[8] = &fp_out; argv[9] = &bucket_slots;
-    argv[10] = &bucket_status; argv[11] = &split; argv[12] = &zero_word;
+    argv[10] = &bucket_status; argv[11] = &split; argv[12] = &zero_word; argv[13] = &block_bounds; argv[14] = &planes;
     if (split.sub < 1u || split.sub > BUCKET_SUB_MAX) split.sub = 1u;
     {
         uint32_t nbk = BUCKET_COUNT * split.sub, pad2 = 256u;
diff --git a/bevy_gaussian_splatting_amd/plugin.py b/bevy_gaussian_splatting_amd/plugin.py
--- a/bevy_gaussian_splatting_amd/plugin.py
+++ b/bevy_gaussian_splatting_amd/plugin.py
@@ -680,6 +680,7 @@
             "algorithmic_bytes": int(st.algorithmic_bytes),
             "regrow_count": int(st.regrow_count),
             "sort_path": ("onesweep", "bucket", "kept")[int(st.sort_path)],
+            "block_walk": bool(st.block_walk),
             "list_capacity": int(st.list_capacity),
             "binning": "sort" if st.binning_mode else "scan",
             "frames_averaged": int(st.frames_averaged),
diff --git a/include/bgs.h b/include/bgs.h
--- a/include/bgs.h
+++ b/include/bgs.h
@@ -99,6 +99,7 @@
     uint32_t visible_count;
     uint32_t draw_count;
     uint32_t sort_path;
+    uint32_t block_walk;
     uint64_t instance_count;
     uint64_t instance_capacity;
     uint32_t tiles_x, tiles_y;
diff --git a/include/bgs_diag.h b/include/bgs_diag.h
--- a/include/bgs_diag.h
+++ b/include/bgs_diag.h
@@ -8,6 +8,7 @@
 #endif
 
 enum bgs_debug_flag {
+    BGS_DEBUG_NO_BLOCK_CULL = 0x80,
     BGS_DEBUG_BUCKETS_NARROW = 0x100,
     BGS_DEBUG_SPLIT_SUB_3 = 0x200,
     BGS_DEBUG_SPLIT_SUB_5 = 0x400,
```

New measurement: 23620 frames/s (median of 5 runs). 5.5% higher.
